# XuyangBai/PointDSC

Hardware: AMD Instinct MI355X
Metric: point-cloud pairs/sec @ N=5000 corr (higher is better)
Workload: dtype f32 (attention products as fp16x3 split (fp16 hi+lo operand pairs, three f16 MFMAs per product), f32 accumulate; fc_message / PointCN products as fp16 hi+lo split; spatial-consistency matrix stored as unorm16); 1 GPU; 3DMatch-like synthetic correspondences (BASELINE.json configs[2]): N=5000 corr, 32 pairs per step sharded over 1 GPU(s) = 32 per GPU, 12-layer PointDSC, seeded random weights; num_corr=5000, pairs_per_gpu=32, global_batch=32, compat_format=u16, layer_gemm=h3, att_leaves=canonical, latency_mode=False, range_guard=lazy (pipeline), collective=none (single process, no process group)

## Files before the change

include/pointdsc_hip.h:

```cpp
#ifndef POINTDSC_HIP_H
#define POINTDSC_HIP_H

#include <stddef.h>

#ifdef __cplusplus
extern "C" {
#endif

#define PDSC_VERSION 9
#define PDSC_CHANNELS 128
#define PDSC_MAX_K 64
#define PDSC_MAX_POWER_ITERS 32

enum pdsc_status {
    PDSC_OK = 0,
    PDSC_ERR_ARG = -1,
    PDSC_ERR_WORKSPACE = -2,
    PDSC_ERR_LAUNCH = -3
};

typedef struct pdsc_config {
    int in_dim;
    int num_layers;
    int num_channels;
// ... 79 lines not shown

int pdsc_layer0(const float* corr_pos, int in_dim, const float* W0, const float* b0, float* feat,
                int M, void* stream);

enum pdsc_layer_kernel {
    PDSC_LAYER_KERNEL_AUTO = 0,
    PDSC_LAYER_KERNEL_BLOCK,
    PDSC_LAYER_KERNEL_WAVE,
    PDSC_LAYER_KERNEL_H3,
    PDSC_LAYER_KERNEL_X3
};
typedef struct pdsc_layer_call {
    const float* msg;
    const float* part_o;
    const float* part_ml;
    int nsplit, Npad;
    const float* res;
    const float* feat_in;
    float* feat_out;
    float* featB_out;
    float* qkv_out;
    void* q_split;
    void* kv_tiles;
    const void* w1; const float* b1;
    const void* w2; const float* b2;
    const void* w3; const float* b3;
    const void* wp; const float* bp;
    const void* wq; const float* bq;
    const void* wq_split;
    const void* wfrag_tail;
    const void* wfrag_head;
    int gemm_format;
    int io_flags;
    int bs, N;
    int kernel;
} pdsc_layer_call;
int pdsc_layer_run(const pdsc_layer_call* call, void* stream);

size_t    pdsc_wsplit_bytes(const pdsc_config* cfg);
long long pdsc_wsplit_offset(const pdsc_config* cfg, int section, int layer);
int       pdsc_wsplit_build(const pdsc_config* cfg, const float* wpack, void* wsplit, void* stream);
#define PDSC_WS_FRAG_TAIL 100
#define PDSC_WS_FRAG_HEAD 101
#define PDSC_WS_FRAG_TAIL_H3 102
#define PDSC_WS_FRAG_HEAD_H3 103
#define PDSC_WS_FOLD_TAIL_H3 104
#define PDSC_WS_FOLD_HEAD_H3 105
#define PDSC_WS_FOLD_W 106
size_t pdsc_wfrag_fold_tail_bytes(void);
size_t pdsc_wfrag_fold_head_bytes(void);
int pdsc_layer_prefers_block(int bs, int N);
int pdsc_layer_h3_uses_coop(int bs, int N);
size_t pdsc_wfrag_tail_bytes(void);
size_t pdsc_wfrag_head_bytes(void);
int pdsc_wfrag_build_tail(const float* w1, const float* b1, const float* w2, const float* b2, const float* w3,
                          const float* b3, void* out, int gemm_format, void* stream);
int pdsc_wfrag_build_head(const float* wp, const float* bp, const float* wq, const float* bq, void* out,
                          int gemm_format, void* stream);

size_t pdsc_attention_scratch_bytes(int bs, int N, int nsplit);
int    pdsc_attention_default_split(int bs, int N);
int    pdsc_sc_attention(const float* qkv, const float* compat, long long ld, float* msg,
                         void* scratch, size_t scratch_bytes, int bs, int N, int nsplit, void* stream);

size_t pdsc_split_q_bytes(int bs, int N);
size_t pdsc_split_kv_bytes(int bs, int N);
int    pdsc_pack_qkv_split(const float* qkv, void* q_split, void* kv_tiles, int bs, int N, void* stream);
size_t pdsc_attention_split_scratch_bytes(int bs, int N, int nsplit);
int    pdsc_attention_split_default_split(int bs, int N);
int    pdsc_attention_leaf_count(int N);
int    pdsc_attention_leaf_plan(int bs, int N, int leaves_mode, int* nsplit, int* nleaf);
size_t pdsc_attention_leaf_scratch_bytes(int bs, int N, int leaves_mode);
int    pdsc_sc_attention_split(const void* q_split, const void* kv_tiles, const float* compat, long long ld,
                               float* msg, void* scratch, size_t scratch_bytes, int bs, int N, int nsplit,
                               void* stream);
int    pdsc_sc_attention_split_u16(const void* q_split, const void* kv_tiles, const unsigned short* compat_u16, long long ld,
                                   float* msg, void* scratch, size_t scratch_bytes, int bs, int N, int nsplit,
                                   void* stream);

int pdsc_attention_trace(long long* device_buffer);

int pdsc_attention_leaf_split_override(int d);

int pdsc_layer_trace(long long* device_buffer);

int pdsc_classifier_hidden(const float* feat, const float* W1, const float* b1, const float* W2, const float* b2, float* h2,
                           int M, void* stream);

int pdsc_normalize_confidence(const float* feat, const float* h2, const float* w3, const float* b3,
                              float* normed, float* conf, int M, void* stream);

int pdsc_nms_keys(const float* src_keypts, const float* conf, float radius, float* keys,
                  int bs, int N, void* stream);
size_t pdsc_nms_workspace_bytes(int bs, int N);
int pdsc_nms_keys_grid(const float* src_keypts, const float* conf, float radius, float* keys, void* workspace,
                       size_t workspace_bytes, int bs, int N, void* stream);
int pdsc_rank_select(const float* keys, int* seeds, int bs, int N, int num_seeds, void* stream);

int pdsc_knn_seeds(const float* normed, const int* seeds, float* dist_scratch, int* knn_idx,
                   int bs, int N, int S, int k, void* stream);
int pdsc_knn_seeds_form(const float* normed, const float* normed_pf, const int* seeds, float* dist_scratch, int* knn_idx,
                        int bs, int N, int S, int k, int form, void* stream);
int pdsc_normalize_confidence_pf(const float* feat, const float* h2, const float* w3, const float* b3, float* normed,
                                 float* normed_pf, float* conf, int bs, int N, void* stream);

int pdsc_seed_power_iteration(const float* normed, const float* src_keypts, const float* tgt_keypts,
                              const int* knn_idx, const float* sigma, const float* sigma_spat,
                              float* eig_iters, unsigned int* conv_mask, float* seed_M,
                              int bs, int N, int S, int k, int num_iterations, void* stream);

int pdsc_seed_transforms(const float* src_keypts, const float* tgt_keypts, const int* knn_idx,
                         const float* eig_iters, const unsigned int* conv_mask, float* seed_trans,
                         float* seed_weights ,
                         int bs, int N, int S, int k, int num_iterations, void* stream);

int pdsc_seed_solve(const float* normed, const float* src_keypts, const float* tgt_keypts, const int* knn_idx,
                    const float* sigma, const float* sigma_spat, float* eig_iters, unsigned int* conv_mask, float* seed_M,
                    float* seed_trans, float* seed_weights, int bs, int N, int S, int k, int num_iterations, void* stream);

int pdsc_rigid_transform_3d(const float* A, const float* B, const float* weights, float weight_threshold,
                            float* T, int bs, int n, void* stream);

int pdsc_score_hypotheses(const float* seed_trans, const float* src_keypts, const float* tgt_keypts,
                          float inlier_threshold, int* counts, int bs, int N, int S, void* stream);
int pdsc_select_best(const int* counts, const float* seed_trans, const float* src_keypts,
                     const float* tgt_keypts, float inlier_threshold, int* best, float* initial_trans,
                     float* labels, int bs, int N, int S, void* stream);

int pdsc_post_refinement(const float* initial_trans, const float* src_keypts, const float* tgt_keypts,
                         float threshold, int max_iters, float* final_trans, int* solves,
                         int bs, int N, void* stream);

int pdsc_forward_testing(const pdsc_config* cfg, const float* wpack, const void* wsplit ,
                         const float* corr_pos, const float* src_keypts, const float* tgt_keypts,
                         int bs, int N, int num_seeds,
                         float* final_trans, float* final_labels,
                         void* workspace, size_t workspace_bytes, void* stream);

int pdsc_forward_testing_ragged(const pdsc_config* cfg, const float* wpack, const void* wsplit,
                                const float* corr_pos, const float* src_keypts, const float* tgt_keypts,
                                int bs, int N, int num_seeds, const int* num_corr, const int* num_seeds_per_pair, int n_min,
                                float* final_trans, float* final_labels,
                                void* workspace, size_t workspace_bytes, void* stream);

int pdsc_forward_testing_streams(const pdsc_config* cfg, const float* wpack, const void* wsplit,
                                 const float* corr_pos, const float* src_keypts, const float* tgt_keypts,
                                 int bs, int N, int num_seeds, const int* num_corr ,
                                 const int* num_seeds_per_pair, int n_min,
                                 float* final_trans, float* final_labels,
                                 void* workspace, size_t workspace_bytes,
                                 void* stream, void* tail_stream, void* fork_event, void* join_event);

int pdsc_forward_validation(const pdsc_config* cfg, const float* wpack, const void* wsplit,
                            const float* corr_pos, const float* src_keypts, const float* tgt_keypts,
                            int bs, int N, int num_seeds, float* final_trans, float* logits,
                            float* M, long long ldM, void* workspace, size_t workspace_bytes, void* stream);

int pdsc_feature_compat(const float* normed, const float* sigma, float* M, long long ld, int bs, int N, void* stream);

int pdsc_conv_mask_all_pairs(unsigned int* conv_mask, int bs, void* stream);

size_t pdsc_match_scratch_bytes(int Ns, int Nt);
int pdsc_match_descriptors(const float* src_desc, const float* tgt_desc, int Ns, int Nt, int D, int* nn_idx,
                           float* nn_dist, void* scratch, size_t scratch_bytes, void* stream);
int pdsc_match_descriptors_ip(const float* src_desc, const float* tgt_desc, int Ns, int Nt, int D, int* nn_idx,
                              float* nn_dot, void* scratch, size_t scratch_bytes, void* stream);
// ... 135 lines not shown
```

pointdsc_amd/_lib.py:

```python
from __future__ import annotations

import ctypes as C
import os
from pathlib import Path

PKG = Path(__file__).resolve().parent
LIB_PATH = Path(os.environ.get("POINTDSC_HIP_LIB", PKG / "libpointdsc_hip.so"))


class PointDSCLibraryError(RuntimeError):
    pass


class PdscConfig(C.Structure):
    _fields_ = [
        ("in_dim", C.c_int), ("num_layers", C.c_int), ("num_channels", C.c_int),
        ("num_iterations", C.c_int), ("k", C.c_int), ("refine_iters", C.c_int),
        ("inlier_threshold", C.c_float), ("nms_radius", C.c_float), ("refine_threshold", C.c_float),
        ("attention_precision", C.c_int), ("compat_format", C.c_int), ("layer_gemm", C.c_int),
        ("att_leaves", C.c_int), ("value_fold", C.c_int),
    ]


W_SECTIONS = [
    "LAYER0_W", "LAYER0_B", "PCN_W", "PCN_B", "QKV_W", "QKV_B", "FC1_W", "FC1_B", "FC2_W", "FC2_B",
    "FC3_W", "FC3_B", "CLS1_W", "CLS1_B", "CLS2_W", "CLS2_B", "CLS3_W", "CLS3_B", "SIGMA", "SIGMA_SPAT",
]
W = {name: i for i, name in enumerate(W_SECTIONS)}

_vp, _i, _f, _ll, _sz = C.c_void_p, C.c_int, C.c_float, C.c_longlong, C.c_size_t
_cfgp = C.POINTER(PdscConfig)


class PdscLayerCall(C.Structure):
    _fields_ = (
        [(n, _vp) for n in ("msg", "part_o", "part_ml")] + [("nsplit", _i), ("Npad", _i)] +
        [(n, _vp) for n in ("res", "feat_in", "feat_out", "featB_out", "qkv_out", "q_split", "kv_tiles",
                            "w1", "b1", "w2", "b2", "w3", "b3", "wp", "bp", "wq", "bq", "wq_split", "wfrag_tail", "wfrag_head")] +
        [(n, _i) for n in ("gemm_format", "io_flags", "bs", "N", "kernel")])

SIGNATURES = {
    "pdsc_version": (_i, []),
    "pdsc_set_range_report": (_i, [_vp]),
    "pdsc_last_error": (C.c_char_p, []),
    "pdsc_experiments_enabled": (_i, []),
    "pdsc_wpack_floats": (_ll, [_cfgp]),
    "pdsc_wpack_offset": (_ll, [_cfgp, _i, _i]),
    "pdsc_compat_ld": (_ll, [_i]),
    "pdsc_workspace_bytes": (_sz, [_cfgp, _i, _i, _i]),
    "pdsc_workspace_offset": (_ll, [_cfgp, _i, _i, _i, C.c_char_p]),
    "pdsc_spatial_compat": (_i, [_vp, _vp, _vp, _vp, _vp, _ll, _i, _i, _vp]),
    "pdsc_spatial_compat_u16": (_i, [_vp, _vp, _vp, _vp, _ll, _i, _i, _vp]),
    "pdsc_selftest_exact_math": (_i, [_vp, _f, _vp, _vp, _ll, _vp]),
    "pdsc_selftest_mfma_valu_neighbour": (_i, [_vp, _i, _i, _vp]),
    "pdsc_classifier_hidden": (_i, [_vp, _vp, _vp, _vp, _vp, _vp, _i, _vp]),
    "pdsc_linear": (_i, [_vp, _ll, _vp, _vp, _vp, _ll, _vp, _ll, _i, _i, _i, _i, _vp]),
    "pdsc_layer0": (_i, [_vp, _i, _vp, _vp, _vp, _i, _vp]),
    "pdsc_layer_run": (_i, [C.POINTER(PdscLayerCall), _vp]),
    "pdsc_wsplit_bytes": (_sz, [_cfgp]),
    "pdsc_wsplit_offset": (_ll, [_cfgp, _i, _i]),
    "pdsc_wsplit_build": (_i, [_cfgp, _vp, _vp, _vp]),
    "pdsc_layer_prefers_block": (_i, [_i, _i]),
    "pdsc_layer_h3_uses_coop": (_i, [_i, _i]),
    "pdsc_wfrag_tail_bytes": (_sz, []),
    "pdsc_wfrag_head_bytes": (_sz, []),
    "pdsc_wfrag_fold_tail_bytes": (_sz, []),
    "pdsc_wfrag_fold_head_bytes": (_sz, []),
    "pdsc_wfrag_build_tail": (_i, [_vp] * 7 + [_i, _vp]),
    "pdsc_wfrag_build_head": (_i, [_vp] * 5 + [_i, _vp]),
    "pdsc_sc_attention_split_partials": (_i, [_vp, _vp, _vp, _i, _ll, _vp, _sz, _i, _i, _i, _i, _vp]),
    "pdsc_split_q_bytes": (_sz, [_i, _i]),
    "pdsc_split_kv_bytes": (_sz, [_i, _i]),
    "pdsc_pack_qkv_split": (_i, [_vp, _vp, _vp, _i, _i, _vp]),
    "pdsc_attention_split_scratch_bytes": (_sz, [_i, _i, _i]),
    "pdsc_attention_split_default_split": (_i, [_i, _i]),
    "pdsc_attention_leaf_count": (_i, [_i]),
    "pdsc_attention_leaf_plan": (_i, [_i, _i, _i, C.POINTER(C.c_int), C.POINTER(C.c_int)]),
    "pdsc_attention_leaf_scratch_bytes": (_sz, [_i, _i, _i]),
    "pdsc_attention_trace": (_i, [_vp]),
    "pdsc_attention_leaf_split_override": (_i, [_i]),
    "pdsc_layer_trace": (_i, [_vp]),
    "pdsc_sc_attention_split": (_i, [_vp, _vp, _vp, _ll, _vp, _vp, _sz, _i, _i, _i, _vp]),
    "pdsc_sc_attention_split_u16": (_i, [_vp, _vp, _vp, _ll, _vp, _vp, _sz, _i, _i, _i, _vp]),
    "pdsc_attention_scratch_bytes": (_sz, [_i, _i, _i]),
    "pdsc_attention_default_split": (_i, [_i, _i]),
    "pdsc_sc_attention": (_i, [_vp, _vp, _ll, _vp, _vp, _sz, _i, _i, _i, _vp]),
    "pdsc_normalize_confidence": (_i, [_vp, _vp, _vp, _vp, _vp, _vp, _i, _vp]),
    "pdsc_nms_keys": (_i, [_vp, _vp, _f, _vp, _i, _i, _vp]),
    "pdsc_nms_workspace_bytes": (_sz, [_i, _i]),
    "pdsc_nms_keys_grid": (_i, [_vp, _vp, _f, _vp, _vp, _sz, _i, _i, _vp]),
    "pdsc_rank_select": (_i, [_vp, _vp, _i, _i, _i, _vp]),
    "pdsc_knn_seeds": (_i, [_vp, _vp, _vp, _vp, _i, _i, _i, _i, _vp]),
    "pdsc_knn_seeds_form": (_i, [_vp, _vp, _vp, _vp, _vp, _i, _i, _i, _i, _i, _vp]),
    "pdsc_normalize_confidence_pf": (_i, [_vp, _vp, _vp, _vp, _vp, _vp, _vp, _i, _i, _vp]),
    "pdsc_seed_power_iteration": (_i, [_vp, _vp, _vp, _vp, _vp, _vp, _vp, _vp, _vp, _i, _i, _i, _i, _i, _vp]),
    "pdsc_seed_solve": (_i, [_vp] * 11 + [_i, _i, _i, _i, _i, _vp]),
    "pdsc_seed_transforms": (_i, [_vp, _vp, _vp, _vp, _vp, _vp, _vp, _i, _i, _i, _i, _i, _vp]),
    "pdsc_rigid_transform_3d": (_i, [_vp, _vp, _vp, _f, _vp, _i, _i, _vp]),
    "pdsc_score_hypotheses": (_i, [_vp, _vp, _vp, _f, _vp, _i, _i, _i, _vp]),
    "pdsc_select_best": (_i, [_vp, _vp, _vp, _vp, _f, _vp, _vp, _vp, _i, _i, _i, _vp]),
    "pdsc_post_refinement": (_i, [_vp, _vp, _vp, _f, _i, _vp, _vp, _i, _i, _vp]),
    "pdsc_profile_enable": (_i, [_i]),
    "pdsc_profile_reset": (_i, []),
    "pdsc_profile_set_stride": (_i, [_i, _i]),
    "pdsc_profile_read": (_i, [_i, C.POINTER(C.c_double), C.POINTER(C.c_int)]),
    "pdsc_match_scratch_bytes": (_sz, [_i, _i]),
    "pdsc_match_descriptors": (_i, [_vp, _vp, _i, _i, _i, _vp, _vp, _vp, _sz, _vp]),
    "pdsc_match_descriptors_ip": (_i, [_vp, _vp, _i, _i, _i, _vp, _vp, _vp, _sz, _vp]),
    "pdsc_select_correspondences": (_i, [_vp, _vp, _i, _vp, _vp, _vp]),
    "pdsc_build_corr_pos": (_i, [_vp, _vp, _vp, _vp, _vp, _vp, _vp, _vp]),
    "pdsc_sm_workspace_bytes": (_sz, [_i, _i]),
    "pdsc_sm_baseline": (_i, [_vp, _vp, _vp, _f, _i, _i, _vp, _vp, _vp, _vp, _sz, _i, _i, _vp]),
    "pdsc_sm_baseline_form": (_i, [_vp, _vp, _vp, _f, _i, _i, _vp, _vp, _vp, _vp, _sz, _i, _i, _i, _vp]),
    "pdsc_pmc_adjacency": (_i, [_vp, _f, _vp, _ll, _i, _i, _vp]),
    "pdsc_pmc_workspace_bytes": (_sz, [_i, _i]),
    "pdsc_pmc_baseline": (_i, [_vp, _vp, _vp, _f, _i, _vp, _vp, _vp, _vp, _vp, _sz, _i, _i, _vp]),
    "pdsc_pmc_baseline_ex": (_i, [_vp, _vp, _vp, _f, _i, _vp, _vp, _vp, _vp, _vp, _sz, _i, _i, _i, C.POINTER(C.c_float), _vp]),
    "pdsc_cal_confidence_workspace_bytes": (_sz, [_i, _i]),
    "pdsc_cal_confidence": (_i, [_vp, _ll, _vp, _i, _i, _vp, _vp, _sz, _i, _i, _vp]),
    "pdsc_eval_stats": (_i, [_vp, _vp, _vp, _vp, _f, _f, _vp, _i, _i, _vp]),
    "pdsc_loss_workspace_bytes": (_sz, [_i, _i]),
    "pdsc_classification_loss": (_i, [_vp, _vp, _vp, _i, _vp, _vp, _vp, _sz, _i, _i, _vp]),
    "pdsc_sm_loss_matrix": (_i, [_vp, _ll, _vp, _i, _vp, _vp, _vp, _sz, _i, _i, _vp]),
    "pdsc_sm_loss_features": (_i, [_vp, _vp, _vp, _i, _vp, _vp, _vp, _vp, _sz, _i, _i, _vp]),
    "pdsc_transformation_loss": (_i, [_vp, _vp, _vp, _vp, _vp, _f, _f, _vp, _vp, _sz, _i, _i, _vp]),
    "pdsc_sc_attention_lse": (_i, [_vp, _vp, _ll, _vp, _vp, _vp, _sz, _i, _i, _i, _vp]),
    "pdsc_attention_backward_workspace_bytes": (_sz, [_i, _i]),
    "pdsc_sc_attention_backward": (_i, [_vp, _vp, _ll, _vp, _vp, _vp, _vp, _vp, _sz, _i, _i, _vp]),
    "pdsc_attention_backward_default_split": (_i, [_i, _i]),
    "pdsc_attention_backward_split_workspace_bytes": (_sz, [_i, _i, _i]),
    "pdsc_sc_attention_backward_split": (_i, [_vp, _vp, _ll, _vp, _vp, _vp, _vp, _vp, _sz, _i, _i, _i, _vp]),
    "pdsc_feature_compat_backward_workspace_bytes": (_sz, [_i, _i]),
    "pdsc_feature_compat_backward": (_i, [_vp, _vp, _vp, _ll, _vp, _vp, _vp, _sz, _i, _i, _vp]),
    "pdsc_icp_workspace_bytes": (_sz, [_i, _i, _i]),
    "pdsc_icp_refine": (_i, [_vp, _vp, _vp, _vp, _vp, C.c_double, C.c_double, C.c_double, _i, _vp, _vp, _vp, _vp, _vp, _vp, _vp,
                             _sz, _i, _i, _i, _vp]),
    "pdsc_information_workspace_bytes": (_sz, [_i, _i, _i]),
    "pdsc_information_matrix": (_i, [_vp, _vp, _vp, _vp, _vp, C.c_double, _vp, _vp, _vp, _vp, _sz, _i, _i, _i, _vp]),
    "pdsc_voxel_keys": (_i, [_vp, _vp, C.c_double, _vp, _i, _i, _vp]),
    "pdsc_voxel_means": (_i, [_vp, _vp, _vp, _vp, _vp, _i, _i, _vp]),
    "pdsc_hybrid_neighbours_workspace_bytes": (_sz, [_i, _i]),
    "pdsc_hybrid_neighbours": (_i, [_vp, _vp, C.c_double, _i, _vp, _vp, _vp, _vp, _sz, _i, _i, _vp]),
    "pdsc_estimate_normals": (_i, [_vp, _vp, _vp, _vp, _i, C.POINTER(C.c_double), _vp, _i, _i, _vp]),
    "pdsc_spfh": (_i, [_vp, _vp, _vp, _vp, _vp, _i, _vp, _i, _i, _vp]),
    "pdsc_fpfh_from_spfh": (_i, [_vp, _vp, _vp, _vp, _vp, _i, _vp, _vp, _i, _i, _vp]),
    "pdsc_fpfh_workspace_bytes": (_sz, [_i, _i, _i, _i]),
    "pdsc_fpfh": (_i, [_vp, _vp, C.c_double, _i, C.c_double, _i, C.POINTER(C.c_double), _vp, _vp, _vp, _vp, _sz, _i, _i, _vp]),
    "pdsc_cloud_voxel_workspace_bytes": (_sz, [_i, _i]),
    "pdsc_cloud_voxel_keys": (_i, [_vp, _vp, C.c_double, _vp, _vp, _sz, _i, _i, _i, _vp]),
    "pdsc_cloud_voxel_means": (_i, [_vp, _vp, _vp, _vp, _vp, _vp, _vp, _i, _i, _vp, _sz, _i, _i, _i, _vp]),
    "pdsc_cloud_neighbours": (_i, [_vp, _vp, C.c_double, _i, _vp, _vp, _vp, _vp, _sz, _i, _i, _i, _vp]),
    "pdsc_posegraph_workspace_bytes": (_sz, [_i, _i, _i]),
    "pdsc_posegraph_nodes": (_i, [_vp] * 6 + [_i, _i, _i, _vp]),
    "pdsc_global_optimization": (_i, [_vp] * 9 + [C.c_double, C.c_double, C.c_double, _i, _vp, _vp, _vp, _vp, _vp, _vp, _sz, _i, _i, _i, _i,
                                      _i, _vp]),
    "pdsc_encoder_range_probe": (_i, [_cfgp, _vp, _vp, _vp, _vp, _vp, _i, _i, _i, _vp, _vp, _sz, _vp]),
    "pdsc_forward_validation": (_i, [_cfgp, _vp, _vp, _vp, _vp, _vp, _i, _i, _i, _vp, _vp, _vp, _ll, _vp, _sz, _vp]),
    "pdsc_feature_compat": (_i, [_vp, _vp, _vp, _ll, _i, _i, _vp]),
    "pdsc_conv_mask_all_pairs": (_i, [_vp, _i, _vp]),
    "pdsc_forward_testing": (_i, [_cfgp, _vp, _vp, _vp, _vp, _vp, _i, _i, _i, _vp, _vp, _vp, _sz, _vp]),
    "pdsc_forward_testing_ragged": (_i, [_cfgp, _vp, _vp, _vp, _vp, _vp, _i, _i, _i, _vp, _vp, _i, _vp, _vp, _vp, _sz, _vp]),
    "pdsc_forward_testing_streams": (_i, [_cfgp, _vp, _vp, _vp, _vp, _vp, _i, _i, _i, _vp, _vp, _i, _vp, _vp, _vp, _sz, _vp, _vp, _vp, _vp]),
}
# ... 37 lines not shown
```

pointdsc_amd/csrc/api.hip:

```cpp
#include <stdarg.h>
#include <stdlib.h>
#include <string.h>
#include <mutex>
#include "pdsc_common.h"
#include "ragged.h"
#include "attention_common.h"
#include "layer_args.h"

namespace pdsc {

static thread_local char g_err[512] = "";

static unsigned int*& range_report_slot() {
    static thread_local unsigned int* slot = nullptr;
    return slot;
}

void set_error(const char* fmt, ...) {
    va_list ap;
    va_start(ap, fmt);
    vsnprintf(g_err, sizeof(g_err), fmt, ap);
    va_end(ap);
}

int check_launch(const char* what) {
    const hipError_t e = hipGetLastError();
    if (e != hipSuccess) {
        set_error("%s: %s", what, hipGetErrorString(e));
        return PDSC_ERR_LAUNCH;
    }
    return PDSC_OK;
}

int ensure_dynamic_lds(const void* fn, size_t bytes, const char* what) {
    struct Entry { const void* fn; size_t granted[64]; };
    static Entry table[64];
    static int used = 0;
    static std::mutex mu;
    int dev = 0;
    if (hipGetDevice(&dev) != hipSuccess) return check_launch(what);
    std::lock_guard<std::mutex> lock(mu);
    Entry* e = nullptr;
    for (int i = 0; i < used; ++i)
        if (table[i].fn == fn) { e = &table[i]; break; }
    if (e && dev < 64 && e->granted[dev] >= bytes) return PDSC_OK;
    if (hipFuncSetAttribute(fn, hipFuncAttributeMaxDynamicSharedMemorySize, (int)bytes) != hipSuccess) return check_launch(what);
    if (!e && used < 64) { e = &table[used++]; e->fn = fn; memset(e->granted, 0, sizeof(e->granted)); }
    if (e && dev < 64) e->granted[dev] = bytes;
    return PDSC_OK;
}

__global__ void fill_u32_kernel(unsigned int* p, unsigned int value, size_t count) {
    const size_t i = (size_t)blockIdx.x * blockDim.x + threadIdx.x;
    if (i < count) p[i] = value;
}
__global__ void copy_u32_kernel(unsigned int* __restrict__ dst, const unsigned int* __restrict__ src, size_t count) {
    for (size_t i = (size_t)blockIdx.x * blockDim.x + threadIdx.x; i < count; i += (size_t)gridDim.x * blockDim.x) dst[i] = src[i];
}
__global__ void absmax_kernel(const float* __restrict__ x, size_t count, unsigned int* __restrict__ slot) {
    unsigned int m = 0u;
    for (size_t i = (size_t)blockIdx.x * blockDim.x + threadIdx.x; i < count; i += (size_t)gridDim.x * blockDim.x) {
        const unsigned int u = __float_as_uint(x[i]) & 0x7fffffffu;
        m = u > m ? u : m;
    }
#pragma unroll
    for (int off = 32; off > 0; off >>= 1) {
        const unsigned int o = __shfl_xor(m, off, 64);
        m = o > m ? o : m;
    }
    if ((threadIdx.x & 63) == 0 && m) atomicMax(slot, m);
}
static int launch_absmax(const float* x, size_t count, unsigned int* slot, hipStream_t st) {
    const size_t blocks = (count + 1023) / 1024;
    hipLaunchKernelGGL(absmax_kernel, dim3((unsigned)(blocks < 2048 ? blocks : 2048)), dim3(256), 0, st, x, count, slot);
    return check_launch("absmax");
}
int launch_copy_u32(unsigned int* dst, const unsigned int* src, size_t count, hipStream_t st) {
    if (count == 0) return PDSC_OK;
    const size_t blocks = (count + 255) / 256;
    hipLaunchKernelGGL(copy_u32_kernel, dim3((unsigned)(blocks < 4096 ? blocks : 4096)), dim3(256), 0, st, dst, src, count);
    return check_launch("copy");
}
int launch_fill_u32(unsigned int* p, unsigned int value, size_t count, hipStream_t st) {
    if (count == 0) return PDSC_OK;
    hipLaunchKernelGGL(fill_u32_kernel, dim3((unsigned)((count + 255) / 256)), dim3(256), 0, st, p, value, count);
    return check_launch("fill");
}

struct ProfKind { hipEvent_t* start = nullptr; hipEvent_t* stop = nullptr; int cap = 0, n = 0, stride = 1; long long calls = 0; bool open = false; };
static ProfKind g_prof[PDSC_PROF_NUM_KINDS];

void profile_mark_begin(int kind, hipStream_t st) {
    ProfKind& p = g_prof[kind];
    if (p.cap == 0 || p.n >= p.cap) return;
    if ((p.calls++ % p.stride) != 0) return;
    (void)hipEventRecord(p.start[p.n], st);
    p.open = true;
}
void profile_mark_end(int kind, hipStream_t st) {
// ... 99 lines not shown
    "compat", "featA", "featB", "featC", "qkv", "msg", "t64a", "t64b", "att_scratch", "q_split", "kv_tiles", "normed",
    "normed_pf", "h1", "h2", "conf", "keys", "nms_ws", "seeds", "knn_dist", "knn_idx", "eig_iters", "conv_mask",
    "seed_trans", "seed_w", "counts", "best", "initial_trans", "solves", "range_flag", "refine_trace",
#ifdef PDSC_EXPERIMENTS
    "score_dbg",
#endif
};
static_assert(sizeof(ws_names) / sizeof(ws_names[0]) == WS_NUM, "ws_names must name every WsId, in order");

struct WsLayout {
    size_t offset[WS_NUM], bytes[WS_NUM], total;
    template <class T> T* at(void* ws, WsId id) const { return (T*)((char*)ws + offset[id]); }
};

static WsLayout make_layout(const pdsc_config* c, int bs, int N, int S) {
    WsLayout L{};
    size_t* B = L.bytes;
    const size_t M = (size_t)bs * N, C = PDSC_CHANNELS, f = sizeof(float);
    const size_t ld = (size_t)pdsc_compat_ld(N);
    const int k = c->k < N - 1 ? c->k : N - 1;
    const int iters = c->num_iterations > 0 ? c->num_iterations : 1;
    const bool compat16 = c->attention_precision != PDSC_ATT_FP32 && c->compat_format == PDSC_COMPAT_U16;
    B[WS_COMPAT] = (size_t)bs * N * ld * (compat16 ? sizeof(unsigned short) : f);
    B[WS_FEATA] = M * C * f;
    const size_t Mpf = (size_t)bs * round_up(N, 32);
    B[WS_FEATB] = B[WS_FEATC] = Mpf * C * f;
    B[WS_QKV] = M * 3 * C * f;
    B[WS_MSG] = M * C * f;
    B[WS_T64A] = B[WS_T64B] = M * (C / 2) * f;
    {
        const size_t a32 = pdsc_attention_scratch_bytes(bs, N, 0), a16 = pdsc_attention_split_scratch_bytes(bs, N, 0);
        const size_t amg = c->att_leaves >= PDSC_LEAVES_CANONICAL ? pdsc_attention_leaf_scratch_bytes(bs, N, c->att_leaves) : 0;
        B[WS_ATT_SCRATCH] = c->attention_precision == PDSC_ATT_FP32 ? a32 : (a16 > amg ? a16 : amg);
    }
    B[WS_Q_SPLIT] = c->attention_precision != PDSC_ATT_FP32 ? pdsc_split_q_bytes(bs, N) : 0;
    B[WS_KV_TILES] = c->attention_precision != PDSC_ATT_FP32 ? pdsc_split_kv_bytes(bs, N) : 0;
    B[WS_NORMED] = M * C * f;
    B[WS_NORMED_PF] = knn_seeds_uses_fused(bs, N, S, k) ? Mpf * C * f : 0;
    B[WS_H1] = B[WS_H2] = M * 32 * f;
    B[WS_CONF] = B[WS_KEYS] = M * f;
    B[WS_NMS_WS] = pdsc_nms_workspace_bytes(bs, N);
    B[WS_SEEDS] = (size_t)bs * S * sizeof(int);
    B[WS_KNN_DIST] = (size_t)bs * S * ld * f;
    B[WS_KNN_IDX] = (size_t)bs * S * (k > 0 ? k : 1) * sizeof(int);
    B[WS_EIG_ITERS] = (size_t)bs * S * iters * PDSC_MAX_K * f;
    B[WS_CONV_MASK] = (size_t)bs * sizeof(unsigned int);
    B[WS_SEED_TRANS] = (size_t)bs * S * 16 * f;
    B[WS_SEED_W] = (size_t)bs * S * (k > 0 ? k : 1) * f;
    B[WS_COUNTS] = (size_t)bs * S * sizeof(int);
    B[WS_BEST] = (size_t)bs * sizeof(int);
    B[WS_INITIAL_TRANS] = (size_t)bs * 16 * f;
    B[WS_SOLVES] = (size_t)bs * sizeof(int);
    B[WS_RANGE_FLAG] = (size_t)bs * sizeof(unsigned int);
    B[WS_REFINE_TRACE] = (size_t)bs * PDSC_REFINE_TRACE * sizeof(int);
#ifdef PDSC_EXPERIMENTS
    B[WS_SCORE_DBG] = (size_t)bs * S * 16 * f;
#endif
    for (int i = 0; i < WS_NUM; ++i) {
        L.offset[i] = L.total;
        L.total += (size_t)round_up((long long)B[i], 256);
    }
    return L;
}

}

using namespace pdsc;

extern "C" int pdsc_version(void) { return PDSC_VERSION; }

extern "C" int pdsc_set_range_report(unsigned int* host_words) {
    if (host_words) {
        hipPointerAttribute_t at{};
        if (hipPointerGetAttributes(&at, host_words) != hipSuccess || at.type != hipMemoryTypeHost || at.devicePointer == nullptr) {
            (void)hipGetLastError();
            set_error("pdsc_set_range_report: %p is not pinned, device-mapped host memory", (void*)host_words);
            return PDSC_ERR_ARG;
        }
        host_words = (unsigned int*)at.devicePointer;
    }
    range_report_slot() = host_words;
    return PDSC_OK;
}
extern "C" int pdsc_experiments_enabled(void) {
#ifdef PDSC_EXPERIMENTS
    return 1;
#else
    return 0;
#endif
}
extern "C" const char* pdsc_last_error(void) { return g_err; }

extern "C" long long pdsc_wpack_floats(const pdsc_config* cfg) {
    if (!config_ok(cfg)) return -1;
    return wpack_offset(cfg, PDSC_W_SIGMA_SPAT, 0) + section_floats(PDSC_W_SIGMA_SPAT);
}
extern "C" long long pdsc_wpack_offset(const pdsc_config* cfg, int section, int layer) {
    if (!config_ok(cfg)) return -1;
    return wpack_offset(cfg, section, layer);
}

extern "C" size_t pdsc_workspace_bytes(const pdsc_config* cfg, int bs, int N, int num_seeds) {
    if (!config_ok(cfg) || bs <= 0 || N <= 1 || num_seeds <= 0) return 0;
    return make_layout(cfg, bs, N, num_seeds).total;
}
extern "C" long long pdsc_workspace_offset(const pdsc_config* cfg, int bs, int N, int num_seeds, const char* name) {
    if (!config_ok(cfg) || bs <= 0 || N <= 1 || num_seeds <= 0 || !name) return -1;
    const WsLayout L = make_layout(cfg, bs, N, num_seeds);
    for (int i = 0; i < WS_NUM; ++i)
        if (strcmp(ws_names[i], name) == 0) return (long long)L.offset[i];
    return -1;
}

extern "C" int pdsc_profile_enable(int max_records) {
    for (int k = 0; k < PDSC_PROF_NUM_KINDS; ++k) {
        ProfKind& p = g_prof[k];
        for (int i = 0; i < p.cap; ++i) { (void)hipEventDestroy(p.start[i]); (void)hipEventDestroy(p.stop[i]); }
        delete[] p.start; delete[] p.stop;
        const int keep_stride = p.stride;
        p = ProfKind();
        p.stride = keep_stride;
        if (max_records > 0) {
            p.start = new hipEvent_t[max_records];
            p.stop = new hipEvent_t[max_records];
            for (int i = 0; i < max_records; ++i) {
                if (hipEventCreate(&p.start[i]) != hipSuccess || hipEventCreate(&p.stop[i]) != hipSuccess)
                    return check_launch("pdsc_profile_enable");
            }
            p.cap = max_records;
        }
    }
    return PDSC_OK;
}
extern "C" int pdsc_profile_reset(void) {
    for (int k = 0; k < PDSC_PROF_NUM_KINDS; ++k) { g_prof[k].n = 0; g_prof[k].open = false; g_prof[k].calls = 0; }
    return PDSC_OK;
}
extern "C" int pdsc_profile_set_stride(int kind, int stride) {
    PDSC_REQUIRE(kind >= 0 && kind < PDSC_PROF_NUM_KINDS && stride >= 1, "pdsc_profile_set_stride: kind=%d stride=%d", kind, stride);
    g_prof[kind].stride = stride;
    g_prof[kind].calls = 0;
    return PDSC_OK;
}
extern "C" int pdsc_profile_read(int kind, double* total_ms, int* launches) {
    PDSC_REQUIRE(kind >= 0 && kind < PDSC_PROF_NUM_KINDS && total_ms && launches, "pdsc_profile_read: bad argument");
    ProfKind& p = g_prof[kind];
    double tot = 0.0;
    for (int i = 0; i < p.n; ++i) {
        if (hipEventSynchronize(p.stop[i]) != hipSuccess) return check_launch("pdsc_profile_read");
        float ms = 0.f;
        if (hipEventElapsedTime(&ms, p.start[i], p.stop[i]) != hipSuccess) return check_launch("pdsc_profile_read");
        tot += ms;
    }
    *total_ms = tot;
    *launches = p.n;
    return PDSC_OK;
}

#define PDSC_TRY(call)                 \
    do {                               \
        const int rc__ = (call);       \
        if (rc__ != PDSC_OK) return rc__; \
    } while (0)

struct EncoderPlan {
    bool fused;
    bool split;
    LayerKernel kernel;
    bool x3, frag;
    bool fuse_merge;
    bool pf, leaves, fold;
    int gemm;
    int ns, Npad;
    int nleaf, value_width;
    int leaf_ns;
    int ws_tail, ws_head;
};

static int plan_encoder(const pdsc_config* cfg, int bs, int N, const int* nvalid, int n_min, EncoderPlan* plan) {
    EncoderPlan& p = *plan = EncoderPlan{};
    p.split = cfg->attention_precision != PDSC_ATT_FP32;
    p.x3 = cfg->attention_precision == PDSC_ATT_FP16X3_ALL;
    p.fused = env_int("PDSC_FUSED_LAYERS", 1) != 0 && cfg->num_layers > 0;
    const bool canonical = cfg->att_leaves >= PDSC_LEAVES_CANONICAL;
    const int min_tiles = (n_min + 31) / 32;
    p.ns = p.split ? pdsc_attention_split_default_split(bs, N) : 0;
#define PDSC_REQUIRE_SHORTEST_PAIR(cond)                                                                                             \
    PDSC_REQUIRE(cond, "pdsc_forward_testing_ragged: the shortest pair (%d correspondences) has fewer 32-key tiles than the key split " \
                 "planned for bs=%d, N=%d (%d): batch pairs of more similar size", n_min, bs, N, p.ns)
    if (nvalid && p.split && !canonical) PDSC_REQUIRE_SHORTEST_PAIR(min_tiles >= p.ns);
    const char* var = env_str("PDSC_LAYER_VARIANT");
    const bool force_block = var && var[0] == 'b', force_wave = var && var[0] == 'w';
    auto by_size = [&](int pairs, int rows) {
        return force_block || (!force_wave && pdsc_layer_prefers_block(pairs, rows)) ? LayerKernel::Block : LayerKernel::Wave;
    };
    if (!p.fused || !p.split) {
        p.kernel = by_size(1, bs * N);
        return PDSC_OK;
    }
    p.Npad = (int)round_up(N, 256);
    p.gemm = env_int("PDSC_LAYER_GEMM", cfg->layer_gemm) == PDSC_LAYER_GEMM_H3 ? PDSC_LAYER_GEMM_H3 : PDSC_LAYER_GEMM_F32;
    const bool h3 = p.gemm == PDSC_LAYER_GEMM_H3;
    const LayerKernel natural = by_size(bs, N);
    p.frag = env_int("PDSC_LAYER_FRAG", 1) && !p.x3 && !force_block && (natural == LayerKernel::Wave || h3);
    p.kernel = p.x3     ? LayerKernel::X3
               : !p.frag ? natural
                         : h3 && env_int("PDSC_LAYER_H3_VARIANT", 1) != 0 ? LayerKernel::H3 : LayerKernel::Wave;
    p.fuse_merge = env_int("PDSC_FUSE_MERGE", 1) && p.ns > 1 && p.ns <= layer_merge_limit(p.kernel);
    const bool pf_ok = p.kernel == LayerKernel::H3 && env_int("PDSC_LAYER_PF", 1) != 0;
    int lf_ns = 0, lf_nw = 0;
    if (canonical) PDSC_TRY(leaf_plan(bs, N, cfg->att_leaves, &lf_nw, &lf_ns, &p.nleaf));
    p.leaf_ns = lf_ns;
    p.leaves = pf_ok && canonical && (!nvalid || min_tiles >= 2 * p.nleaf);
    if (nvalid && !p.leaves) PDSC_REQUIRE_SHORTEST_PAIR(min_tiles >= p.ns);
#undef PDSC_REQUIRE_SHORTEST_PAIR
    p.pf = p.leaves || (pf_ok && p.fuse_merge);
    p.fold = cfg->value_fold == PDSC_VALUE_FOLD_ON && p.pf && N <= PDSC_VALUE_FOLD_MAX_N;
    p.value_width = p.fold ? PDSC_CHANNELS / 2 : PDSC_CHANNELS;
    p.ws_tail = p.fold ? PDSC_WS_FOLD_TAIL_H3 : h3 ? PDSC_WS_FRAG_TAIL_H3 : PDSC_WS_FRAG_TAIL;
    p.ws_head = p.fold ? PDSC_WS_FOLD_HEAD_H3 : h3 ? PDSC_WS_FRAG_HEAD_H3 : PDSC_WS_FRAG_HEAD;
    return PDSC_OK;
}

enum class ForwardMode { Testing, Validation, Probe };

struct ForwardCall {
    ForwardMode mode;
    const pdsc_config* cfg;
    const float* wpack;
    const void* wsplit;
    const float *corr_pos, *src, *tgt;
    int bs, N, num_seeds;
    float *final_trans, *final_labels, *Mout;
    long long ldM;
    void* workspace;
    size_t workspace_bytes;
    void* stream;
    const int *nvalid, *svalid;
    int n_min;
    void *tail_stream, *ev_fork, *ev_join;
    unsigned int* probe;
};

struct ForwardCtx {
    const ForwardCall& c;
    EncoderPlan plan;
    WsLayout L;
    hipStream_t st;
    int M, S, k, cfmt;
    long long ld;
    bool split;
    float *compat, *featA, *featB, *featC, *qkv, *msg, *normed, *normed_pf, *conf, *keys, *seed_trans;
    int *seeds, *knn_idx, *counts;
    unsigned int *conv_mask, *range_flag;
    void *att_scratch, *q_split, *kv_tiles;
    const float* W(int section, int layer) const { return c.wpack + wpack_offset(c.cfg, section, layer); }
    const void* WS(int section, int layer) const { return (const unsigned short*)c.wsplit + pdsc_wsplit_offset(c.cfg, section, layer); }
};

static int validate_call(const ForwardCall& c) {
    if (!config_ok(c.cfg)) return PDSC_ERR_ARG;
    PDSC_REQUIRE(!c.tail_stream || (c.ev_fork && c.ev_join && c.tail_stream != c.stream),
                 "pdsc_forward_testing_streams: a tail stream (different from the main stream) needs the fork and join events");
    const int N = c.N, n_min = c.n_min, k = c.cfg->k < N - 1 ? c.cfg->k : N - 1;
    if (c.nvalid) {
        PDSC_REQUIRE(c.mode == ForwardMode::Testing && c.svalid, "pdsc_forward_testing_ragged: testing forward only, both count arrays needed");
        PDSC_REQUIRE(n_min >= 2 && n_min <= N, "pdsc_forward_testing_ragged: n_min=%d (N=%d)", n_min, N);
        PDSC_REQUIRE(n_min > k, "pdsc_forward_testing_ragged: the shortest pair (%d correspondences) has no "
                     "more than k=%d: the reference clamps k per pair (k = min(k, num_corr - 1)); run such a pair in its own call", n_min, k);
    }
    const bool outputs = c.mode == ForwardMode::Probe || (c.final_trans && c.final_labels);
    PDSC_REQUIRE(c.wpack && c.corr_pos && c.src && c.tgt && outputs && c.workspace, "pdsc_forward_testing: null pointer");
    PDSC_REQUIRE(c.bs > 0 && N > 1, "pdsc_forward_testing: bs=%d N=%d", c.bs, N);
    PDSC_REQUIRE(c.num_seeds >= 1 && c.num_seeds <= N,
                 "pdsc_forward_testing: num_seeds=%d (int(N*ratio) must be >= 1; the reference fails on an empty seed set)", c.num_seeds);
    return PDSC_OK;
}

static int bind_workspace(ForwardCtx& x) {
    const ForwardCall& c = x.c;
    const WsLayout& L = x.L = make_layout(c.cfg, c.bs, c.N, c.num_seeds);
    if (c.workspace_bytes < L.total) {
        set_error("pdsc_forward_testing: workspace %zu < %zu bytes", c.workspace_bytes, L.total);
        return PDSC_ERR_WORKSPACE;
    }
    void* ws = c.workspace;
    x.st = (hipStream_t)c.stream;
    x.M = c.bs * c.N; x.S = c.num_seeds; x.k = c.cfg->k < c.N - 1 ? c.cfg->k : c.N - 1;
    x.ld = pdsc_compat_ld(c.N);
    x.compat = L.at<float>(ws, WS_COMPAT); x.featA = L.at<float>(ws, WS_FEATA); x.featB = L.at<float>(ws, WS_FEATB);
    x.featC = L.at<float>(ws, WS_FEATC); x.qkv = L.at<float>(ws, WS_QKV); x.msg = L.at<float>(ws, WS_MSG);
    x.normed = L.at<float>(ws, WS_NORMED); x.conf = L.at<float>(ws, WS_CONF); x.keys = L.at<float>(ws, WS_KEYS);
    x.seed_trans = L.at<float>(ws, WS_SEED_TRANS); x.seeds = L.at<int>(ws, WS_SEEDS); x.knn_idx = L.at<int>(ws, WS_KNN_IDX);
    x.counts = L.at<int>(ws, WS_COUNTS); x.conv_mask = L.at<unsigned int>(ws, WS_CONV_MASK); x.att_scratch = L.at<void>(ws, WS_ATT_SCRATCH);
    const bool split = x.split = x.plan.split;
    PDSC_REQUIRE(!split || c.wsplit, "pdsc_forward_testing: the split-precision modes need the split-weight buffer (pdsc_wsplit_build)");
    x.q_split = split ? L.at<void>(ws, WS_Q_SPLIT) : nullptr;
    x.kv_tiles = split ? L.at<void>(ws, WS_KV_TILES) : nullptr;
    x.range_flag = split && c.mode != ForwardMode::Probe ? L.at<unsigned int>(ws, WS_RANGE_FLAG) : nullptr;
    x.cfmt = split && c.cfg->compat_format == PDSC_COMPAT_U16 ? PDSC_COMPAT_U16 : PDSC_COMPAT_F32;
    const bool knn_fused = c.mode == ForwardMode::Testing && knn_seeds_uses_fused(c.bs, c.N, x.S, x.k);
    x.normed_pf = knn_fused ? L.at<float>(ws, WS_NORMED_PF) : nullptr;
    return PDSC_OK;
}

static int probe_absmax(const ForwardCtx& x, int kind, const float* v, size_t count) {
    return x.c.probe ? launch_absmax(v, count, x.c.probe + kind, x.st) : PDSC_OK;
}

static int run_compat_layer0(const ForwardCtx& x) {
    const ForwardCall& c = x.c;
    if (x.cfmt == PDSC_COMPAT_U16)
        PDSC_TRY(pdsc_spatial_compat_u16(c.src, c.tgt, x.W(PDSC_W_SIGMA_SPAT, 0), (unsigned short*)x.compat, x.ld, c.bs, c.N, x.st));
    else
        PDSC_TRY(pdsc_spatial_compat(c.src, c.tgt, x.W(PDSC_W_SIGMA_SPAT, 0), x.compat, nullptr, x.ld, c.bs, c.N, x.st));
    PDSC_TRY(launch_layer0(c.corr_pos, c.cfg->in_dim, x.W(PDSC_W_LAYER0_W, 0), x.W(PDSC_W_LAYER0_B, 0), x.featA, x.M, x.range_flag, c.bs, x.st));
    return probe_absmax(x, PDSC_RANGE_LAYER0, x.featA, (size_t)x.M * PDSC_CHANNELS);
}

static int attention_split(const ForwardCtx& x, float* msg_out, int nsplit) {
    return launch_attention_split_ex(x.q_split, x.kv_tiles, x.compat, x.cfmt, x.ld, msg_out, x.att_scratch, x.L.bytes[WS_ATT_SCRATCH], x.c.bs,
                                     x.c.N, nsplit, PDSC_PARTIALS_ROWS, x.c.nvalid, x.st);
}

static int run_fused_layer(const ForwardCtx& x, int i, bool last, const float* cur, float* nxt) {
    const EncoderPlan& plan = x.plan;
    const bool tail = i >= 0, head = !last, split = x.split;
    const bool parts = plan.pf || plan.fuse_merge;
    const int slots = plan.leaves ? plan.nleaf : plan.ns;
    const int nparts = plan.leaves && plan.leaf_ns == 1 ? 1 : slots;
    const float* part_o = parts ? (const float*)x.att_scratch : nullptr;
    const float* part_ml = parts ? part_o + (size_t)x.c.bs * slots * plan.Npad * plan.value_width : nullptr;
    pdsc_layer_call c{};
    c.bs = split ? x.c.bs : 1; c.N = split ? x.c.N : x.M;
    if (tail) {
        c.msg = parts ? nullptr : x.msg;
        c.part_o = part_o; c.part_ml = part_ml; c.nsplit = nparts; c.Npad = plan.Npad;
        c.res = cur;
    } else
        c.feat_in = x.featA;
    if (last) c.feat_out = x.featA;
    if (head) {
        c.featB_out = nxt; c.qkv_out = split ? nullptr : x.qkv;
        c.q_split = x.q_split; c.kv_tiles = x.kv_tiles;
    }
    if (plan.frag) {
        if (tail) c.wfrag_tail = x.WS(plan.ws_tail, i);
        if (head) c.wfrag_head = x.WS(plan.ws_head, i + 1);
        c.gemm_format = plan.gemm;
    } else {
        auto mat = [&](int section, int l) { return plan.x3 ? x.WS(section, l) : (const void*)x.W(section, l); };
        if (tail) {
            c.w1 = mat(PDSC_W_FC1_W, i); c.b1 = x.W(PDSC_W_FC1_B, i); c.w2 = mat(PDSC_W_FC2_W, i); c.b2 = x.W(PDSC_W_FC2_B, i);
            c.w3 = mat(PDSC_W_FC3_W, i); c.b3 = x.W(PDSC_W_FC3_B, i);
        }
        if (head) {
            c.wp = mat(PDSC_W_PCN_W, i + 1); c.bp = x.W(PDSC_W_PCN_B, i + 1); c.wq = mat(PDSC_W_QKV_W, i + 1); c.bq = x.W(PDSC_W_QKV_B, i + 1);
            if (split) c.wq_split = x.WS(PDSC_W_QKV_W, i + 1);
        }
    }
    if (plan.pf) c.io_flags = (tail ? PDSC_IO_PARTIALS_PF | PDSC_IO_RES_PF : 0) | (head ? PDSC_IO_FEATB_PF : 0);
    LayerArgs a = layer_args_from_call(c);
    a.nvalid = split ? x.c.nvalid : nullptr;
    if (tail) a.part_slots = slots;
    if (plan.pf) {
        a.value_fold = plan.fold;
        a.range_flag = x.range_flag;
    } else
        a.trace = pdsc_layer_trace_buffer();
    PDSC_TRY(validate_layer_args(a, plan.kernel, "pdsc_forward_testing(layer)"));
    return dispatch_layer(a, plan.kernel, x.st);
}

static int run_encoder_fused(const ForwardCtx& x) {
    const ForwardCall& c = x.c;
    const EncoderPlan& plan = x.plan;
    const size_t att_bytes = x.L.bytes[WS_ATT_SCRATCH];
    PDSC_TRY(run_fused_layer(x, -1, false, nullptr, x.featB));
    float *cur = x.featB, *nxt = x.featC;
    for (int i = 0; i < c.cfg->num_layers; ++i) {
        if (!x.split)
            PDSC_TRY(launch_attention_fp32(x.qkv, x.compat, x.ld, x.msg, x.att_scratch, att_bytes, c.bs, c.N, 0, c.nvalid, x.st));
        else if (plan.leaves)
            PDSC_TRY(launch_attention_leaves(x.q_split, x.kv_tiles, x.compat, x.cfmt, x.ld, x.att_scratch, att_bytes, c.bs, c.N,
                                             c.cfg->att_leaves, c.nvalid, c.n_min, x.st, plan.value_width));
        else if (plan.pf)
            PDSC_TRY(launch_attention_split_ex(x.q_split, x.kv_tiles, x.compat, x.cfmt, x.ld, nullptr, x.att_scratch, att_bytes, c.bs, c.N,
                                               plan.ns, PDSC_PARTIALS_PF, c.nvalid, x.st, plan.value_width));
        else
            PDSC_TRY(attention_split(x, plan.fuse_merge ? nullptr : x.msg, plan.ns));
        PDSC_TRY(run_fused_layer(x, i, i + 1 == c.cfg->num_layers, cur, nxt));
        float* tmp = cur; cur = nxt; nxt = tmp;
    }
    return PDSC_OK;
}

static int run_encoder_per_conv(const ForwardCtx& x) {
    const int C = PDSC_CHANNELS, H = C / 2, M = x.M;
    float *t64a = x.L.at<float>(x.c.workspace, WS_T64A), *t64b = x.L.at<float>(x.c.workspace, WS_T64B);
    for (int i = 0; i < x.c.cfg->num_layers; ++i) {
        PDSC_TRY(pdsc_linear(x.featA, C, x.W(PDSC_W_PCN_W, i), x.W(PDSC_W_PCN_B, i), nullptr, 0, x.featB, C, M, C, C, 1, x.st));
        PDSC_TRY(probe_absmax(x, PDSC_RANGE_POINTCN, x.featB, (size_t)M * C));
        PDSC_TRY(pdsc_linear(x.featB, C, x.W(PDSC_W_QKV_W, i), x.W(PDSC_W_QKV_B, i), nullptr, 0, x.qkv, 3 * C, M, C, 3 * C, 0, x.st));
        PDSC_TRY(probe_absmax(x, PDSC_RANGE_QKV, x.qkv, (size_t)M * 3 * C));
        if (x.split) {
            PDSC_TRY(pdsc_pack_qkv_split(x.qkv, x.q_split, x.kv_tiles, x.c.bs, x.c.N, x.st));
            PDSC_TRY(attention_split(x, x.msg, 0));
        } else
            PDSC_TRY(pdsc_sc_attention(x.qkv, x.compat, x.ld, x.msg, x.att_scratch, x.L.bytes[WS_ATT_SCRATCH], x.c.bs, x.c.N, 0, x.st));
        PDSC_TRY(probe_absmax(x, PDSC_RANGE_MESSAGE, x.msg, (size_t)M * C));
        PDSC_TRY(pdsc_linear(x.msg, C, x.W(PDSC_W_FC1_W, i), x.W(PDSC_W_FC1_B, i), nullptr, 0, t64a, H, M, C, H, 1, x.st));
        PDSC_TRY(probe_absmax(x, PDSC_RANGE_FC1, t64a, (size_t)M * H));
        PDSC_TRY(pdsc_linear(t64a, H, x.W(PDSC_W_FC2_W, i), x.W(PDSC_W_FC2_B, i), nullptr, 0, t64b, H, M, H, H, 1, x.st));
        PDSC_TRY(probe_absmax(x, PDSC_RANGE_FC2, t64b, (size_t)M * H));
        PDSC_TRY(pdsc_linear(t64b, H, x.W(PDSC_W_FC3_W, i), x.W(PDSC_W_FC3_B, i), x.featB, C, x.featA, C, M, H, C, 0, x.st));
        PDSC_TRY(probe_absmax(x, PDSC_RANGE_FEATURE, x.featA, (size_t)M * C));
    }
    return PDSC_OK;
}

static int fork_tail(ForwardCtx& x) {
    if (!x.c.tail_stream) return PDSC_OK;
    if (hipEventRecord((hipEvent_t)x.c.ev_fork, (hipStream_t)x.c.stream) != hipSuccess ||
        hipStreamWaitEvent((hipStream_t)x.c.tail_stream, (hipEvent_t)x.c.ev_fork, 0) != hipSuccess)
        return check_launch("pdsc_forward_testing_streams(fork)");
    x.st = (hipStream_t)x.c.tail_stream;
    return PDSC_OK;
}
static int join_tail(const ForwardCtx& x) {
    if (!x.c.tail_stream) return PDSC_OK;
    if (hipEventRecord((hipEvent_t)x.c.ev_join, (hipStream_t)x.c.tail_stream) != hipSuccess ||
        hipStreamWaitEvent((hipStream_t)x.c.stream, (hipEvent_t)x.c.ev_join, 0) != hipSuccess)
        return check_launch("pdsc_forward_testing_streams(join)");
    return PDSC_OK;
}

static int run_seed_selection(const ForwardCtx& x) {
    const ForwardCall& c = x.c;
    const int C = PDSC_CHANNELS, M = x.M;
    float *h1 = x.L.at<float>(c.workspace, WS_H1), *h2 = x.L.at<float>(c.workspace, WS_H2);
    if (env_int("PDSC_CLS_FUSED", 1))
        PDSC_TRY(launch_classifier_hidden(x.featA, x.W(PDSC_W_CLS1_W, 0), x.W(PDSC_W_CLS1_B, 0), x.W(PDSC_W_CLS2_W, 0), x.W(PDSC_W_CLS2_B, 0), h2, M, x.st));
    else {
        PDSC_TRY(pdsc_linear(x.featA, C, x.W(PDSC_W_CLS1_W, 0), x.W(PDSC_W_CLS1_B, 0), nullptr, 0, h1, 32, M, C, 32, 1, x.st));
        PDSC_TRY(pdsc_linear(h1, 32, x.W(PDSC_W_CLS2_W, 0), x.W(PDSC_W_CLS2_B, 0), nullptr, 0, h2, 32, M, 32, 32, 1, x.st));
    }
    if (x.normed_pf)
        PDSC_TRY(launch_normalize_conf_pf(x.featA, h2, x.W(PDSC_W_CLS3_W, 0), x.W(PDSC_W_CLS3_B, 0), x.normed, x.normed_pf, x.conf, c.bs, c.N, x.st));
    else
        PDSC_TRY(pdsc_normalize_confidence(x.featA, h2, x.W(PDSC_W_CLS3_W, 0), x.W(PDSC_W_CLS3_B, 0), x.normed, x.conf, M, x.st));
    if (c.mode == ForwardMode::Testing) {
        PDSC_TRY(launch_nms_keys_grid(c.src, x.conf, c.cfg->nms_radius, x.keys, x.L.at<void>(c.workspace, WS_NMS_WS),
                                      pdsc_nms_workspace_bytes(c.bs, c.N), c.bs, c.N, c.nvalid, x.st));
        return launch_rank_select(x.keys, x.seeds, c.bs, c.N, x.S, c.nvalid, c.svalid, x.st, x.conv_mask);
    }
    PDSC_TRY(pdsc_feature_compat(x.normed, x.W(PDSC_W_SIGMA, 0), c.Mout, c.ldM, c.bs, c.N, x.st));
    return pdsc_rank_select(x.conf, x.seeds, c.bs, c.N, x.S, x.st);
}

static int run_hypotheses(const ForwardCtx& x) {
    const ForwardCall& c = x.c;
    const bool testing = c.mode == ForwardMode::Testing;
    const int iters = c.cfg->num_iterations;
    void* ws = c.workspace;
    float *knn_dist = x.L.at<float>(ws, WS_KNN_DIST), *eig = x.L.at<float>(ws, WS_EIG_ITERS), *seed_w = x.L.at<float>(ws, WS_SEED_W);
    PDSC_TRY(launch_knn_seeds_form(x.normed, x.normed_pf, x.seeds, knn_dist, x.knn_idx, c.bs, c.N, x.S, x.k, c.nvalid, x.normed_pf ? 2 : 1, x.st));
    if (!testing && c.bs > 1) {
        PDSC_TRY(pdsc_seed_power_iteration(x.normed, c.src, c.tgt, x.knn_idx, x.W(PDSC_W_SIGMA, 0), x.W(PDSC_W_SIGMA_SPAT, 0), eig, x.conv_mask,
                                           nullptr, c.bs, c.N, x.S, x.k, iters, x.st));
        PDSC_TRY(pdsc_conv_mask_all_pairs(x.conv_mask, c.bs, x.st));
        PDSC_TRY(pdsc_seed_transforms(c.src, c.tgt, x.knn_idx, eig, x.conv_mask, x.seed_trans, seed_w, c.bs, c.N, x.S, x.k, iters, x.st));
    } else
        PDSC_TRY(launch_seed_solve_forward(x.normed, c.src, c.tgt, x.knn_idx, x.W(PDSC_W_SIGMA, 0), x.W(PDSC_W_SIGMA_SPAT, 0), eig, x.conv_mask,
                                           x.seed_trans, seed_w, c.bs, c.N, x.S, x.k, iters, testing, x.st));
#ifdef PDSC_EXPERIMENTS
    score_debug_slot() = env_int("PDSC_SCORE_DEBUG", 0) ? x.L.at<float>(ws, WS_SCORE_DBG) : nullptr;
#endif
    PDSC_TRY(launch_score_hypotheses(x.seed_trans, c.src, c.tgt, c.cfg->inlier_threshold, x.counts, c.bs, c.N, x.S, c.nvalid, x.st));
#ifdef PDSC_EXPERIMENTS
    score_debug_slot() = nullptr;
#endif
    return PDSC_OK;
}

static int finish_testing(const ForwardCtx& x) {
    const ForwardCall& c = x.c;
    const WsLayout& L = x.L;
    void* ws = c.workspace;
    return launch_select_and_refine(x.counts, x.seed_trans, c.src, c.tgt, c.cfg->inlier_threshold, c.cfg->refine_threshold, c.cfg->refine_iters,
                                    L.at<int>(ws, WS_BEST), L.at<float>(ws, WS_INITIAL_TRANS), c.final_labels, c.final_trans,
                                    L.at<int>(ws, WS_SOLVES), c.bs, c.N, x.S, c.nvalid, x.st, L.at<int>(ws, WS_REFINE_TRACE), x.range_flag,
                                    range_report_slot());
}
static int finish_validation(const ForwardCtx& x) {
    const ForwardCall& c = x.c;
    PDSC_TRY(pdsc_select_best(x.counts, x.seed_trans, c.src, c.tgt, c.cfg->inlier_threshold, x.L.at<int>(c.workspace, WS_BEST), c.final_trans,
                              x.keys , c.bs, c.N, x.S, x.st));
    return launch_copy_u32((unsigned int*)c.final_labels, (const unsigned int*)x.conf, (size_t)x.M, x.st);
}

static int run_forward(const ForwardCall& call) {
    const bool probe = call.mode == ForwardMode::Probe, testing = call.mode == ForwardMode::Testing;
    ForwardCtx x{call};
    PDSC_TRY(validate_call(call));
    PDSC_TRY(plan_encoder(call.cfg, call.bs, call.N, call.nvalid, call.n_min, &x.plan));
    PDSC_TRY(bind_workspace(x));
    PDSC_TRY(run_compat_layer0(x));
    PDSC_TRY(x.plan.fused && !probe ? run_encoder_fused(x) : run_encoder_per_conv(x));
    if (probe) return PDSC_OK;
    PDSC_TRY(fork_tail(x));
    PDSC_TRY(run_seed_selection(x));
    PDSC_TRY(run_hypotheses(x));
    PDSC_TRY(testing ? finish_testing(x) : finish_validation(x));
    return join_tail(x);
}

extern "C" int pdsc_forward_testing(const pdsc_config* cfg, const float* wpack, const void* wsplit, const float* corr_pos,
                                    const float* src, const float* tgt, int bs, int N, int num_seeds,
                                    float* final_trans, float* final_labels, void* workspace, size_t workspace_bytes,
                                    void* stream) {
    return run_forward({.mode = ForwardMode::Testing, .cfg = cfg, .wpack = wpack, .wsplit = wsplit, .corr_pos = corr_pos, .src = src,
                        .tgt = tgt, .bs = bs, .N = N, .num_seeds = num_seeds, .final_trans = final_trans, .final_labels = final_labels,
                        .workspace = workspace, .workspace_bytes = workspace_bytes, .stream = stream});
}

extern "C" int pdsc_forward_testing_ragged(const pdsc_config* cfg, const float* wpack, const void* wsplit, const float* corr_pos,
                                           const float* src, const float* tgt, int bs, int N, int num_seeds, const int* num_corr,
                                           const int* num_seeds_per_pair, int n_min, float* final_trans, float* final_labels,
                                           void* workspace, size_t workspace_bytes, void* stream) {
    PDSC_REQUIRE(num_corr && num_seeds_per_pair, "pdsc_forward_testing_ragged: the per-pair count arrays (device, [bs] int32) are required");
    return run_forward({.mode = ForwardMode::Testing, .cfg = cfg, .wpack = wpack, .wsplit = wsplit, .corr_pos = corr_pos, .src = src,
                        .tgt = tgt, .bs = bs, .N = N, .num_seeds = num_seeds, .final_trans = final_trans, .final_labels = final_labels,
                        .workspace = workspace, .workspace_bytes = workspace_bytes, .stream = stream, .nvalid = num_corr,
                        .svalid = num_seeds_per_pair, .n_min = n_min});
}

extern "C" int pdsc_forward_testing_streams(const pdsc_config* cfg, const float* wpack, const void* wsplit, const float* corr_pos,
                                            const float* src, const float* tgt, int bs, int N, int num_seeds, const int* num_corr,
                                            const int* num_seeds_per_pair, int n_min, float* final_trans, float* final_labels,
                                            void* workspace, size_t workspace_bytes, void* stream, void* tail_stream, void* fork_event,
                                            void* join_event) {
    PDSC_REQUIRE((num_corr == nullptr) == (num_seeds_per_pair == nullptr), "pdsc_forward_testing_streams: both count arrays or neither");
    PDSC_REQUIRE(tail_stream && fork_event && join_event, "pdsc_forward_testing_streams: tail stream and both events are required");
    return run_forward({.mode = ForwardMode::Testing, .cfg = cfg, .wpack = wpack, .wsplit = wsplit, .corr_pos = corr_pos, .src = src,
                        .tgt = tgt, .bs = bs, .N = N, .num_seeds = num_seeds, .final_trans = final_trans, .final_labels = final_labels,
                        .workspace = workspace, .workspace_bytes = workspace_bytes, .stream = stream, .nvalid = num_corr,
                        .svalid = num_seeds_per_pair, .n_min = n_min, .tail_stream = tail_stream, .ev_fork = fork_event, .ev_join = join_event});
}

extern "C" int pdsc_encoder_range_probe(const pdsc_config* cfg, const float* wpack, const void* wsplit, const float* corr_pos,
                                        const float* src, const float* tgt, int bs, int N, int num_seeds, float* absmax,
                                        void* workspace, size_t workspace_bytes, void* stream) {
    PDSC_REQUIRE(absmax, "pdsc_encoder_range_probe: absmax [PDSC_RANGE_NUM_KINDS] (device) required");
    PDSC_TRY(launch_fill_u32((unsigned int*)absmax, 0u, PDSC_RANGE_NUM_KINDS, (hipStream_t)stream));
    return run_forward({.mode = ForwardMode::Probe, .cfg = cfg, .wpack = wpack, .wsplit = wsplit, .corr_pos = corr_pos, .src = src, .tgt = tgt,
                        .bs = bs, .N = N, .num_seeds = num_seeds, .workspace = workspace, .workspace_bytes = workspace_bytes, .stream = stream,
                        .probe = (unsigned int*)absmax});
}

extern "C" int pdsc_forward_validation(const pdsc_config* cfg, const float* wpack, const void* wsplit, const float* corr_pos,
                                       const float* src, const float* tgt, int bs, int N, int num_seeds,
                                       float* final_trans, float* logits, float* Mout, long long ldM, void* workspace,
                                       size_t workspace_bytes, void* stream) {
    PDSC_REQUIRE(Mout && ldM >= N, "pdsc_forward_validation: M matrix [bs][N][ldM >= N] required");
    return run_forward({.mode = ForwardMode::Validation, .cfg = cfg, .wpack = wpack, .wsplit = wsplit, .corr_pos = corr_pos, .src = src,
                        .tgt = tgt, .bs = bs, .N = N, .num_seeds = num_seeds, .final_trans = final_trans, .final_labels = logits, .Mout = Mout,
                        .ldM = ldM, .workspace = workspace, .workspace_bytes = workspace_bytes, .stream = stream});
}
```

pointdsc_amd/csrc/compat.hip:

```cpp
#include <stdlib.h>
#include "pdsc_common.h"

#define PDSC_COMPAT_DEFAULT_VARIANT 3

namespace pdsc {

struct InvariantDivisor {
    float b, y;
    __device__ __forceinline__ explicit InvariantDivisor(float b_) : b(b_) {
        const float y0 = __builtin_amdgcn_rcpf(b_);
        const float e = fmaf(-b_, y0, 1.0f);
        y = fmaf(e, y0, y0);
    }
    __device__ __forceinline__ float div(float a) const {
        const float q0 = a * y;
        const float r0 = fmaf(-b, q0, a);
        const float q1 = fmaf(r0, y, q0);
        const float r1 = fmaf(-b, q1, a);
        return fmaf(r1, y, q1);
    }
};

template <bool FASTMATH>
__device__ __forceinline__ float dist3(float x, float y, float z) {
    const float ss = fmaf(z, z, fmaf(y, y, x * x));
    return FASTMATH ? sqrt_rn(ss) : sqrtf(ss);
}
template <bool FASTMATH>
__device__ __forceinline__ float compat_from_dists(float ds, float dt, float s2, const InvariantDivisor& inv) {
    const float df = ds - dt;
    const float q = FASTMATH ? inv.div(df * df) : (df * df) / s2;
    return fmaxf(1.0f - q, 0.0f);
}

constexpr int CT_ROWS = 64;
constexpr int CT_COLS = 256;

template <bool WRITE_DIST, bool FASTMATH>
__global__ __launch_bounds__(256) void compat_kernel(const float* __restrict__ src, const float* __restrict__ tgt,
                                                     const float* __restrict__ sigma_spat,
                                                     float* __restrict__ compat, float* __restrict__ src_dist,
                                                     long long ld, int N) {
    __shared__ __attribute__((aligned(16))) float rows_s[CT_ROWS][8];
    const int b = blockIdx.z;
    const int i0 = blockIdx.y * CT_ROWS;
    const int j0 = blockIdx.x * CT_COLS;
    const float* srcb = src + (size_t)b * N * 3;
    const float* tgtb = tgt + (size_t)b * N * 3;
    const int t = threadIdx.x;
    if (t < CT_ROWS) {
        const int i = min(i0 + t, N - 1);
        rows_s[t][0] = srcb[i * 3 + 0]; rows_s[t][1] = srcb[i * 3 + 1]; rows_s[t][2] = srcb[i * 3 + 2];
        rows_s[t][4] = tgtb[i * 3 + 0]; rows_s[t][5] = tgtb[i * 3 + 1]; rows_s[t][6] = tgtb[i * 3 + 2];
    }
    const int lane = t & 63, wave = t >> 6;
    const int jc = j0 + lane * 4;
    float sx[4], sy[4], sz[4], tx[4], ty[4], tz[4];
#pragma unroll
    for (int c = 0; c < 4; ++c) {
        const int j = min(jc + c, N - 1);
        sx[c] = srcb[j * 3 + 0]; sy[c] = srcb[j * 3 + 1]; sz[c] = srcb[j * 3 + 2];
        tx[c] = tgtb[j * 3 + 0]; ty[c] = tgtb[j * 3 + 1]; tz[c] = tgtb[j * 3 + 2];
    }
    const float sg = sigma_spat[0];
    const float s2 = sg * sg;
    const InvariantDivisor inv(s2);
    __syncthreads();
    if (jc >= ld) return;
    float* outb = compat + (size_t)b * N * ld;
    float* distb = WRITE_DIST ? src_dist + (size_t)b * N * ld : nullptr;
#pragma unroll 4
    for (int r = 0; r < 16; ++r) {
        const int il = wave * 16 + r;
        const int i = i0 + il;
        if (i >= N) break;
        const f32x4 ps = *reinterpret_cast<const f32x4*>(&rows_s[il][0]);
        const f32x4 pt = *reinterpret_cast<const f32x4*>(&rows_s[il][4]);
        f32x4 o, dd;
#pragma unroll
        for (int c = 0; c < 4; ++c) {
            const float ds = dist3<FASTMATH>(ps[0] - sx[c], ps[1] - sy[c], ps[2] - sz[c]);
            const float dt = dist3<FASTMATH>(pt[0] - tx[c], pt[1] - ty[c], pt[2] - tz[c]);
            const float v = compat_from_dists<FASTMATH>(ds, dt, s2, inv);
            const bool valid = (jc + c) < N;
            o[c] = valid ? v : 0.0f;
            dd[c] = valid ? ds : 0.0f;
        }
        *reinterpret_cast<f32x4*>(outb + (size_t)i * ld + jc) = o;
        if (WRITE_DIST) *reinterpret_cast<f32x4*>(distb + (size_t)i * ld + jc) = dd;
    }
}

constexpr int CS_T = 128;
constexpr int CS_STRIP = 32;
constexpr int CS_LD = CS_T + 4;

template <bool FASTMATH>
__global__ __launch_bounds__(256) void compat_sym_kernel(const float* __restrict__ src, const float* __restrict__ tgt,
                                                         const float* __restrict__ sigma_spat, float* __restrict__ compat,
                                                         long long ld, int N) {
    const int I = blockIdx.y, J = blockIdx.x, b = blockIdx.z;
    if (I > J) return;
    __shared__ __attribute__((aligned(16))) float Ts[CS_STRIP * CS_LD];
    __shared__ __attribute__((aligned(16))) float rows_s[CS_T * 8];
    const int i0 = I * CS_T, j0 = J * CS_T;
    const float* srcb = src + (size_t)b * N * 3;
    const float* tgtb = tgt + (size_t)b * N * 3;
    const int t = threadIdx.x;
    if (t < CS_T) {
        const int i = min(i0 + t, N - 1);
        rows_s[t * 8 + 0] = srcb[i * 3 + 0]; rows_s[t * 8 + 1] = srcb[i * 3 + 1]; rows_s[t * 8 + 2] = srcb[i * 3 + 2];
        rows_s[t * 8 + 4] = tgtb[i * 3 + 0]; rows_s[t * 8 + 5] = tgtb[i * 3 + 1]; rows_s[t * 8 + 6] = tgtb[i * 3 + 2];
    }
    const int l32 = t & 31, rg = t >> 5;
    const int jc = j0 + l32 * 4;
    float sx[4], sy[4], sz[4], tx[4], ty[4], tz[4];
#pragma unroll
    for (int c = 0; c < 4; ++c) {
        const int j = min(jc + c, N - 1);
        sx[c] = srcb[j * 3 + 0]; sy[c] = srcb[j * 3 + 1]; sz[c] = srcb[j * 3 + 2];
        tx[c] = tgtb[j * 3 + 0]; ty[c] = tgtb[j * 3 + 1]; tz[c] = tgtb[j * 3 + 2];
    }
    const float sg = sigma_spat[0];
    const float s2 = sg * sg;
    const InvariantDivisor inv(s2);
    float* outb = compat + (size_t)b * N * ld;
    const bool offdiag = I != J;
    __syncthreads();
    for (int strip = 0; strip < CS_T / CS_STRIP; ++strip) {
#pragma unroll
        for (int r = 0; r < 4; ++r) {
            const int sl = rg + 8 * r;
            const int il = strip * CS_STRIP + sl;
            const int i = i0 + il;
            const f32x4 ps = *reinterpret_cast<const f32x4*>(rows_s + il * 8);
            const f32x4 pt = *reinterpret_cast<const f32x4*>(rows_s + il * 8 + 4);
            f32x4 o;
#pragma unroll
            for (int c = 0; c < 4; ++c) {
                const float ds = dist3<FASTMATH>(ps[0] - sx[c], ps[1] - sy[c], ps[2] - sz[c]);
                const float dt = dist3<FASTMATH>(pt[0] - tx[c], pt[1] - ty[c], pt[2] - tz[c]);
                const float v = compat_from_dists<FASTMATH>(ds, dt, s2, inv);
                o[c] = (jc + c) < N ? v : 0.0f;
            }
            if (i < N && jc < ld) *reinterpret_cast<f32x4*>(outb + (size_t)i * ld + jc) = o;
            if (offdiag) *reinterpret_cast<f32x4*>(Ts + sl * CS_LD + 4 * l32) = o;
        }
        if (offdiag) {
            __syncthreads();
            const int sl = t & 31, jq0 = t >> 5;
            const int i = i0 + strip * CS_STRIP + sl;
#pragma unroll
            for (int p = 0; p < 4; ++p) {
                const int jq = jq0 + 8 * p;
                const f32x4 v = *reinterpret_cast<const f32x4*>(Ts + sl * CS_LD + 4 * jq);
#pragma unroll
                for (int c = 0; c < 4; ++c) {
                    const int j = j0 + 4 * jq + c;
                    if (j < N && i < N) outb[(size_t)j * ld + i] = v[c];
                }
            }
            __syncthreads();
        }
    }
}

typedef unsigned short u16x2 __attribute__((ext_vector_type(2)));
typedef float f32x2 __attribute__((ext_vector_type(2)));
__host__ __device__ __forceinline__ int c16_pos(int r) { return 16 * ((r >> 2) & 1) + 4 * (r >> 3) + (r & 3); }
__host__ __device__ __forceinline__ int c16_chunk_base(int q) { return 16 * (q & 1) + 4 * (q >> 1); }

constexpr int CF_T = 128;
__device__ __forceinline__ int cf_point_slot(int r) { return (r + (r >> 4)) * 8; }

template <bool EDGE, bool CLAMP>
__device__ __forceinline__ void compat_fast_tile(const float* __restrict__ pts, unsigned short* __restrict__ outb, long long ld,
                                                 int N, int i0, int j0, bool offdiag, float ninv) {
    const int t = threadIdx.x, lane = t & 63, w = t >> 6;
    const int ri = (w >> 1) * 8 + (lane >> 3), cj = (w & 1) * 8 + (lane & 7);
    const int rbase = 32 * (ri >> 2) + c16_chunk_base(ri & 3);
    const int cbase = 32 * (cj >> 2) + c16_chunk_base(cj & 3);
    f32x2 sx[4], sy[4], sz[4], tx[4], ty[4], tz[4];
#pragma unroll
    for (int cp = 0; cp < 4; ++cp) {
        const int m0 = 2 * cp, c0 = cbase + (m0 & 3) + 8 * (m0 >> 2);
        const f32x4 a0 = *reinterpret_cast<const f32x4*>(pts + cf_point_slot(CF_T + c0));
        const f32x4 b0 = *reinterpret_cast<const f32x4*>(pts + cf_point_slot(CF_T + c0) + 4);
        const f32x4 a1 = *reinterpret_cast<const f32x4*>(pts + cf_point_slot(CF_T + c0 + 1));
        const f32x4 b1 = *reinterpret_cast<const f32x4*>(pts + cf_point_slot(CF_T + c0 + 1) + 4);
        sx[cp] = f32x2{a0[0], a1[0]}; sy[cp] = f32x2{a0[1], a1[1]}; sz[cp] = f32x2{a0[2], a1[2]};
        tx[cp] = f32x2{b0[0], b1[0]}; ty[cp] = f32x2{b0[1], b1[1]}; tz[cp] = f32x2{b0[2], b1[2]};
    }
    unsigned tr[8][4];
    f32x2 one2 = {1.0f, 1.0f}, ninv2 = {ninv, ninv}, zero2 = {0.f, 0.f};
    asm volatile("" : "+v"(one2), "+v"(ninv2), "+v"(zero2));
    const int colpos = j0 + 32 * (cj >> 2) + 8 * (cj & 3);
    const int rowpos = i0 + 32 * (ri >> 2) + 8 * (ri & 3);
#pragma unroll
    for (int rp = 0; rp < 4; ++rp) {
        const int m0 = 2 * rp, r0 = rbase + (m0 & 3) + 8 * (m0 >> 2);
        const f32x4 ps0 = *reinterpret_cast<const f32x4*>(pts + cf_point_slot(r0));
        const f32x4 pt0 = *reinterpret_cast<const f32x4*>(pts + cf_point_slot(r0) + 4);
        const f32x4 ps1 = *reinterpret_cast<const f32x4*>(pts + cf_point_slot(r0 + 1));
        const f32x4 pt1 = *reinterpret_cast<const f32x4*>(pts + cf_point_slot(r0 + 1) + 4);
        unsigned d0[4], d1[4];
        f32x2 bs[2][3], bt[2][3];
#pragma unroll
        for (int rr = 0; rr < 2; ++rr)
#pragma unroll
            for (int e = 0; e < 3; ++e) {
                bs[rr][e] = f32x2{(rr ? ps1 : ps0)[e], (rr ? ps1 : ps0)[e]};
                bt[rr][e] = f32x2{(rr ? pt1 : pt0)[e], (rr ? pt1 : pt0)[e]};
                asm volatile("" : "+v"(bs[rr][e]), "+v"(bt[rr][e]));
            }
#pragma unroll
        for (int cp = 0; cp < 4; ++cp) {
            f32x2 o[2];
#pragma unroll
            for (int rr = 0; rr < 2; ++rr) {
                const f32x2 dx = bs[rr][0] - sx[cp], dy = bs[rr][1] - sy[cp], dz = bs[rr][2] - sz[cp];
                const f32x2 ex = bt[rr][0] - tx[cp], ey = bt[rr][1] - ty[cp], ez = bt[rr][2] - tz[cp];
                const f32x2 a = __builtin_elementwise_fma(dz, dz, __builtin_elementwise_fma(dy, dy, dx * dx));
                const f32x2 b = __builtin_elementwise_fma(ez, ez, __builtin_elementwise_fma(ey, ey, ex * ex));
                const f32x2 ds = {__builtin_amdgcn_sqrtf(a[0]), __builtin_amdgcn_sqrtf(a[1])};
                const f32x2 dt = {__builtin_amdgcn_sqrtf(b[0]), __builtin_amdgcn_sqrtf(b[1])};
                const f32x2 df = ds - dt;
                f32x2 v = __builtin_elementwise_fma(df * df, ninv2, one2);
                if (CLAMP) v = __builtin_elementwise_max(v, zero2);
                o[rr] = v;
            }
            if (EDGE) {
                const int mc = 2 * cp, jc = j0 + cbase + (mc & 3) + 8 * (mc >> 2);
                const int ir = i0 + r0;
                const bool vj0 = jc < N, vj1 = jc + 1 < N, vi0 = ir < N, vi1 = ir + 1 < N;
                o[0][0] = (vi0 && vj0) ? o[0][0] : 0.f; o[0][1] = (vi0 && vj1) ? o[0][1] : 0.f;
                o[1][0] = (vi1 && vj0) ? o[1][0] : 0.f; o[1][1] = (vi1 && vj1) ? o[1][1] : 0.f;
            }
            d0[cp] = __builtin_bit_cast(unsigned, __builtin_amdgcn_cvt_pknorm_u16(o[0][0], o[0][1]));
            d1[cp] = __builtin_bit_cast(unsigned, __builtin_amdgcn_cvt_pknorm_u16(o[1][0], o[1][1]));
            tr[2 * cp][rp] = __builtin_bit_cast(unsigned, __builtin_amdgcn_cvt_pknorm_u16(o[0][0], o[1][0]));
            tr[2 * cp + 1][rp] = __builtin_bit_cast(unsigned, __builtin_amdgcn_cvt_pknorm_u16(o[0][1], o[1][1]));
        }
        const int i = i0 + r0;
        if (!EDGE || (i < N && colpos < ld)) *reinterpret_cast<u32x4*>(outb + (size_t)i * ld + colpos) = u32x4{d0[0], d0[1], d0[2], d0[3]};
        if (!EDGE || (i + 1 < N && colpos < ld)) *reinterpret_cast<u32x4*>(outb + (size_t)(i + 1) * ld + colpos) = u32x4{d1[0], d1[1], d1[2], d1[3]};
    }
    if (offdiag) {
#pragma unroll
        for (int m = 0; m < 8; ++m) {
            const int j = j0 + cbase + (m & 3) + 8 * (m >> 2);
            if (!EDGE || (j < N && rowpos < ld)) *reinterpret_cast<u32x4*>(outb + (size_t)j * ld + rowpos) = u32x4{tr[m][0], tr[m][1], tr[m][2], tr[m][3]};
        }
    }
}

template <bool CLAMP>
__global__ __launch_bounds__(256) void compat_sym_u16_kernel(const float* __restrict__ src, const float* __restrict__ tgt,
                                                             const float* __restrict__ sigma_spat,
                                                             unsigned short* __restrict__ compat, long long ld, int N, int nt) {
    const int idx = blockIdx.x, b = blockIdx.y;
    int I = (int)(((float)(2 * nt + 1) - __builtin_sqrtf((float)((2 * nt + 1) * (2 * nt + 1) - 8 * idx))) * 0.5f);
    I = max(0, min(I, nt - 1));
    while (I > 0 && I * nt - I * (I - 1) / 2 > idx) --I;
    while ((I + 1) * nt - (I + 1) * I / 2 <= idx) ++I;
    const int J = I + idx - (I * nt - I * (I - 1) / 2);
    __shared__ __attribute__((aligned(16))) float pts[(2 * CF_T + 2 * CF_T / 16) * 8];
    const int i0 = I * CF_T, j0 = J * CF_T;
    const float* srcb = src + (size_t)b * N * 3;
    const float* tgtb = tgt + (size_t)b * N * 3;
    const int t = threadIdx.x;
    {
        const int p = min((t < CF_T ? i0 : j0 - CF_T) + t, N - 1);
        float* d = pts + cf_point_slot(t);
        *reinterpret_cast<f32x4*>(d) = f32x4{srcb[p * 3 + 0], srcb[p * 3 + 1], srcb[p * 3 + 2], 0.f};
        *reinterpret_cast<f32x4*>(d + 4) = f32x4{tgtb[p * 3 + 0], tgtb[p * 3 + 1], tgtb[p * 3 + 2], 0.f};
    }
    const float sg = sigma_spat[0];
    const float s2 = sg * sg;
    const float y0 = __builtin_amdgcn_rcpf(s2);
    const float ninv = -fmaf(fmaf(-s2, y0, 1.0f), y0, y0);
    unsigned short* outb = compat + (size_t)b * N * ld;
    __syncthreads();
    if (i0 + CF_T > N || j0 + CF_T > N)
        compat_fast_tile<true, CLAMP>(pts, outb, ld, N, i0, j0, I != J, ninv);
    else
        compat_fast_tile<false, CLAMP>(pts, outb, ld, N, i0, j0, I != J, ninv);
}

#ifdef PDSC_EXPERIMENTS
constexpr int C16_PITCH = 2 * CS_T + 8;

__global__ __launch_bounds__(256) void compat_sym_u16_exact_kernel(const float* __restrict__ src, const float* __restrict__ tgt,
                                                                   const float* __restrict__ sigma_spat,
                                                                   unsigned short* __restrict__ compat, long long ld, int N) {
    const int I = blockIdx.y, J = blockIdx.x, b = blockIdx.z;
    if (I > J) return;
    __shared__ __attribute__((aligned(16))) unsigned char Ts[CS_STRIP * C16_PITCH];
    __shared__ __attribute__((aligned(16))) float rows_s[CS_T * 8];
    const int i0 = I * CS_T, j0 = J * CS_T;
    const float* srcb = src + (size_t)b * N * 3;
    const float* tgtb = tgt + (size_t)b * N * 3;
    const int t = threadIdx.x;
    if (t < CS_T) {
        const int i = min(i0 + t, N - 1);
        rows_s[t * 8 + 0] = srcb[i * 3 + 0]; rows_s[t * 8 + 1] = srcb[i * 3 + 1]; rows_s[t * 8 + 2] = srcb[i * 3 + 2];
        rows_s[t * 8 + 4] = tgtb[i * 3 + 0]; rows_s[t * 8 + 5] = tgtb[i * 3 + 1]; rows_s[t * 8 + 6] = tgtb[i * 3 + 2];
    }
    const int l32 = t & 31, rg = t >> 5;
    const int jc = j0 + l32 * 4;
    float sx[4], sy[4], sz[4], tx[4], ty[4], tz[4];
#pragma unroll
    for (int c = 0; c < 4; ++c) {
        const int j = min(jc + c, N - 1);
        sx[c] = srcb[j * 3 + 0]; sy[c] = srcb[j * 3 + 1]; sz[c] = srcb[j * 3 + 2];
        tx[c] = tgtb[j * 3 + 0]; ty[c] = tgtb[j * 3 + 1]; tz[c] = tgtb[j * 3 + 2];
    }
    const float sg = sigma_spat[0];
    const float s2 = sg * sg;
    const InvariantDivisor inv(s2);
    unsigned short* outb = compat + (size_t)b * N * ld;
    const bool offdiag = I != J;
    const int jpos = (jc & ~31) + c16_pos(jc & 31);
    __syncthreads();
    for (int strip = 0; strip < CS_T / CS_STRIP; ++strip) {
#pragma unroll
        for (int r = 0; r < 4; ++r) {
            const int sl = rg + 8 * r;
            const int il = strip * CS_STRIP + sl;
            const int i = i0 + il;
            const f32x4 ps = *reinterpret_cast<const f32x4*>(rows_s + il * 8);
            const f32x4 pt = *reinterpret_cast<const f32x4*>(rows_s + il * 8 + 4);
            float o[4];
#pragma unroll
            for (int c = 0; c < 4; ++c) {
                const float ds = dist3<true>(ps[0] - sx[c], ps[1] - sy[c], ps[2] - sz[c]);
                const float dt = dist3<true>(pt[0] - tx[c], pt[1] - ty[c], pt[2] - tz[c]);
                const float v = compat_from_dists<true>(ds, dt, s2, inv);
                o[c] = ((jc + c) < N && i < N) ? v : 0.0f;
            }
            uint2 q;
            q.x = __builtin_bit_cast(unsigned, __builtin_amdgcn_cvt_pknorm_u16(o[0], o[1]));
            q.y = __builtin_bit_cast(unsigned, __builtin_amdgcn_cvt_pknorm_u16(o[2], o[3]));
            if (i < N && jc < ld) *reinterpret_cast<uint2*>(outb + (size_t)i * ld + jpos) = q;
            if (offdiag) *reinterpret_cast<uint2*>(Ts + sl * C16_PITCH + 8 * l32) = q;
        }
        if (offdiag) {
            __syncthreads();
#pragma unroll
            for (int p2 = 0; p2 < 2; ++p2) {
                const int idx = t + 256 * p2, jl = idx >> 2, q = idx & 3;
                unsigned w[4];
#pragma unroll
                for (int m = 0; m < 8; ++m) {
                    const int p = 8 * q + m;
                    const int sl = 8 * ((p >> 2) & 3) + 4 * (p >> 4) + (p & 3);
                    const unsigned v = *reinterpret_cast<const unsigned short*>(Ts + sl * C16_PITCH + 2 * jl);
                    if (m & 1) w[m >> 1] |= v << 16; else w[m >> 1] = v;
                }
                const int j = j0 + jl;
                if (j < N) *reinterpret_cast<u32x4*>(outb + (size_t)j * ld + i0 + strip * CS_STRIP + 8 * q) = u32x4{w[0], w[1], w[2], w[3]};
            }
            __syncthreads();
        }
    }
}
#endif

__global__ void exact_math_selftest_kernel(const float* __restrict__ x, float b, float* __restrict__ sq, float* __restrict__ dv,
                                           long long n) {
    const long long i = (long long)blockIdx.x * 256 + threadIdx.x;
    if (i >= n) return;
    const InvariantDivisor inv(b);
    sq[i] = sqrt_rn(x[i]);
    dv[i] = inv.div(x[i]);
}

}

extern "C" int pdsc_selftest_exact_math(const float* x, float divisor, float* sqrt_out, float* div_out, long long n,
                                        void* stream) {
    PDSC_REQUIRE(x && sqrt_out && div_out && n > 0, "pdsc_selftest_exact_math: bad argument");
    hipLaunchKernelGGL(pdsc::exact_math_selftest_kernel, dim3((unsigned)((n + 255) / 256)), dim3(256), 0, (hipStream_t)stream,
                       x, divisor, sqrt_out, div_out, n);
    return pdsc::check_launch("pdsc_selftest_exact_math");
}

extern "C" long long pdsc_compat_ld(int N) { return N <= 0 ? -1 : pdsc::round_up(N, 64); }

extern "C" int pdsc_spatial_compat(const float* src, const float* tgt, const float* sigma_spat, float* compat,
                                   float* src_dist, long long ld, int bs, int N, void* stream) {
    PDSC_REQUIRE(src && tgt && sigma_spat && compat, "pdsc_spatial_compat: null pointer");
    PDSC_REQUIRE(bs > 0 && N > 0, "pdsc_spatial_compat: bs=%d N=%d", bs, N);
    PDSC_REQUIRE(ld >= N && ld % 4 == 0, "pdsc_spatial_compat: ld=%lld must be >= N and a multiple of 4", ld);
    hipStream_t st = (hipStream_t)stream;
    const dim3 full_grid(pdsc::ceil_div((int)ld, pdsc::CT_COLS), pdsc::ceil_div(N, pdsc::CT_ROWS), bs);
    const int nt = pdsc::ceil_div(N, pdsc::CS_T);
    const dim3 sym_grid(nt, nt, bs);
    pdsc::profile_mark_begin(PDSC_PROF_COMPAT, st);
    if (src_dist)
        hipLaunchKernelGGL((pdsc::compat_kernel<true, true>), full_grid, dim3(256), 0, st, src, tgt, sigma_spat, compat, src_dist, ld, N);
    else {
#ifdef PDSC_EXPERIMENTS
        const int variant = pdsc::env_int("PDSC_COMPAT_VARIANT", PDSC_COMPAT_DEFAULT_VARIANT);
        if (variant == 0)
            hipLaunchKernelGGL((pdsc::compat_kernel<false, false>), full_grid, dim3(256), 0, st, src, tgt, sigma_spat, compat, nullptr, ld, N);
        else if (variant == 1)
            hipLaunchKernelGGL((pdsc::compat_kernel<false, true>), full_grid, dim3(256), 0, st, src, tgt, sigma_spat, compat, nullptr, ld, N);
        else if (variant == 2)
            hipLaunchKernelGGL((pdsc::compat_sym_kernel<false>), sym_grid, dim3(256), 0, st, src, tgt, sigma_spat, compat, ld, N);
        else
#endif
        hipLaunchKernelGGL((pdsc::compat_sym_kernel<true>), sym_grid, dim3(256), 0, st, src, tgt, sigma_spat, compat, ld, N);
    }
    pdsc::profile_mark_end(PDSC_PROF_COMPAT, st);
    return pdsc::check_launch("pdsc_spatial_compat");
}

extern "C" int pdsc_spatial_compat_u16(const float* src, const float* tgt, const float* sigma_spat, unsigned short* compat_u16,
                                       long long ld, int bs, int N, void* stream) {
    PDSC_REQUIRE(src && tgt && sigma_spat && compat_u16, "pdsc_spatial_compat_u16: null pointer");
    PDSC_REQUIRE(bs > 0 && N > 0, "pdsc_spatial_compat_u16: bs=%d N=%d", bs, N);
    PDSC_REQUIRE(ld >= pdsc::round_up(N, 32) && ld % 32 == 0, "pdsc_spatial_compat_u16: ld=%lld must be a multiple of 32 and >= N", ld);
    hipStream_t st = (hipStream_t)stream;
    const int nt = pdsc::ceil_div(N, pdsc::CF_T);
    PDSC_REQUIRE(nt <= 1024, "pdsc_spatial_compat_u16: N=%d too large", N);
    const dim3 grid((unsigned)(nt * (nt + 1) / 2), bs);
    pdsc::profile_mark_begin(PDSC_PROF_COMPAT, st);
#ifdef PDSC_EXPERIMENTS
    const int variant = pdsc::env_int("PDSC_COMPAT16_VARIANT", 2);
    if (variant == 0)
        hipLaunchKernelGGL(pdsc::compat_sym_u16_exact_kernel, dim3(nt, nt, bs), dim3(256), 0, st, src, tgt, sigma_spat, compat_u16, ld, N);
    else if (variant == 1)
        hipLaunchKernelGGL(pdsc::compat_sym_u16_kernel<true>, grid, dim3(256), 0, st, src, tgt, sigma_spat, compat_u16, ld, N, nt);
    else
#endif
    hipLaunchKernelGGL(pdsc::compat_sym_u16_kernel<false>, grid, dim3(256), 0, st, src, tgt, sigma_spat, compat_u16, ld, N, nt);
    pdsc::profile_mark_end(PDSC_PROF_COMPAT, st);
    return pdsc::check_launch("pdsc_spatial_compat_u16");
}
```

pointdsc_amd/csrc/layer.hip:

```cpp
#include <stdlib.h>
#include <type_traits>
#include "pdsc_common.h"
#include "split_layout.h"
#include "merge_partials.h"
#include "layer_args.h"
#include "layer_block.h"

namespace pdsc {

constexpr int LF_ROWS = 32;
constexpr int LF_LD = PDSC_CHANNELS + 4;
constexpr int LF_TILE = LF_ROWS * LF_LD;


#define LF_STAMP(k)                                                                                   \
    if (a.trace && lane == 0) a.trace[(((size_t)blockIdx.y * gridDim.x + blockIdx.x) * 4 + wave) * 16 + (k)] = __builtin_readcyclecounter();

template <int K>
__device__ __forceinline__ void load_w(const float* __restrict__ W, int n0, int l31, int h, f32x4 (&w)[K / 8]) {
    const float* p = W + (size_t)(n0 + l31) * K + 4 * h;
#pragma unroll
    for (int q = 0; q < K / 8; ++q) w[q] = *reinterpret_cast<const f32x4*>(p + 8 * q);
}

// ... 213 lines not shown
            const int n0 = 128 * c + 32 * wave;
            const f32x16 zero = {0.f, 0.f, 0.f, 0.f, 0.f, 0.f, 0.f, 0.f, 0.f, 0.f, 0.f, 0.f, 0.f, 0.f, 0.f, 0.f};
            f32x16 acc = zero;
#pragma unroll
            for (int kk = 0; kk < 8; ++kk) {
                const sp16x8 xh = *reinterpret_cast<const sp16x8*>(Xh + xo + 16 * kk);
                const sp16x8 xl = *reinterpret_cast<const sp16x8*>(Xl + xo + 16 * kk);
                acc = PDSC_MFMA_X3(wl[kk], xh, acc, 0, 0, 0);
                acc = PDSC_MFMA_X3(wh[kk], xl, acc, 0, 0, 0);
                acc = PDSC_MFMA_X3(wh[kk], xh, acc, 0, 0, 0);
            }
            if (c < 2) {
                const sp16* p = a.wq_split + (size_t)(n0 + 128 + l31) * PDSC_CHANNELS + 8 * h;
#pragma unroll
                for (int kk = 0; kk < 8; ++kk) {
                    wh[kk] = *reinterpret_cast<const sp16x8*>(p + 16 * kk);
                    wl[kk] = *reinterpret_cast<const sp16x8*>(p + (size_t)3 * PDSC_CHANNELS * PDSC_CHANNELS + 16 * kk);
                }
            }
            if (c == 0) { LF_STAMP(10) }
            __syncthreads();
            store_tile<false, false>(acc, a.bq, n0, Xa, 32 * wave, l31, h, nullptr);
            __syncthreads();
            if (c == 0) { LF_STAMP(11) }
            if (a.qkv_out) tile_to_global<LF_LD>(Xa, a.qkv_out + 128 * c, 3 * PDSC_CHANNELS, m0, M, t);
            if (a.qs) {
                if (c == 0) tile_to_split<0, LF_LD>(Xa, a.qs + (size_t)m0 * SPL_Q_LD, img, valid, t);
                else if (c == 1) tile_to_split<1, LF_LD>(Xa, nullptr, img, valid, t);
                else tile_to_split<2, LF_LD>(Xa, nullptr, img, valid, t);
            }
            if (c == 0) { LF_STAMP(12) }
        }
        LF_STAMP(13)
    }
}

template <bool T, bool H>
static int launch_layer(const LayerArgs& a, hipStream_t st) {
    if (H && a.wq_split)
        hipLaunchKernelGGL((layer_fused_kernel<T, H, H>), dim3(ceil_div(a.N, LF_ROWS), a.bs), dim3(256), 0, st, a);
    else
        hipLaunchKernelGGL((layer_fused_kernel<T, H, false>), dim3(ceil_div(a.N, LF_ROWS), a.bs), dim3(256), 0, st, a);
    return check_launch("pdsc_layer_run(block)");
}

}

static long long* g_layer_trace = nullptr;
long long* pdsc_layer_trace_buffer(void) { return g_layer_trace; }
extern "C" int pdsc_layer_trace(long long* device_buffer) {
    g_layer_trace = device_buffer;
    return PDSC_OK;
}

extern "C" int pdsc_layer_prefers_block(int bs, int N) {
    return (long long)bs * pdsc::ceil_div(N, pdsc::LF_ROWS) <= 288;
}

namespace pdsc {

int validate_layer_args(const LayerArgs& a, LayerKernel kernel, const char* who) {
    const bool tail = a.msg != nullptr || a.part_o != nullptr, head = a.featB_out != nullptr;
    const bool h3 = kernel == LayerKernel::H3;
    const bool frag = h3 || (kernel == LayerKernel::Wave && (a.wf_tail || a.wf_head));
    const int io = a.io_flags;
    PDSC_REQUIRE(tail || head, "%s: neither tail (msg / partials) nor head (featB_out) requested", who);
    PDSC_REQUIRE(a.bs > 0 && a.N > 0, "%s: bs=%d N=%d", who, a.bs, a.N);
    PDSC_REQUIRE(a.gemm_format == PDSC_LAYER_GEMM_F32 || a.gemm_format == PDSC_LAYER_GEMM_H3, "%s: gemm_format=%d", who, a.gemm_format);
    PDSC_REQUIRE((io & ~(PDSC_IO_PARTIALS_PF | PDSC_IO_RES_PF | PDSC_IO_FEATB_PF)) == 0, "%s: io_flags=%d", who, io);
    PDSC_REQUIRE(h3 || (io == 0 && !a.value_fold), "%s: point-fragment hand-offs and the folded layer exist in the H3 kernel only", who);
    PDSC_REQUIRE(!h3 || a.gemm_format == PDSC_LAYER_GEMM_H3, "%s: point-fragment hand-offs need gemm_format = PDSC_LAYER_GEMM_H3", who);
    PDSC_REQUIRE(!a.value_fold || (io & PDSC_IO_PARTIALS_PF) || !tail, "%s: the folded layer merges point-fragment partials", who);
    if (tail) {
        PDSC_REQUIRE(a.res && (frag ? a.wf_tail != nullptr : a.w1 && a.b1 && a.w2 && a.b2 && a.w3 && a.b3),
                     "%s: tail needs res and fc1..fc3 (natural layout or the tail stream)", who);
        if (!a.msg) PDSC_REQUIRE(a.part_ml && a.nsplit >= 1 && a.nsplit <= layer_merge_limit(kernel) && a.Npad >= a.N,
                                 "%s: partials need part_ml, 1 <= nsplit <= %d (what this launch's kernel merges), Npad >= N", who,
                                 layer_merge_limit(kernel));
        if (!a.msg) PDSC_REQUIRE(a.part_slots == a.nsplit || (h3 && a.part_slots > a.nsplit),
                                 "%s: part_slots=%d (partials per pair in the layout) must be nsplit=%d, or more in the H3 kernels", who,
                                 a.part_slots, a.nsplit);
        PDSC_REQUIRE(!(io & PDSC_IO_PARTIALS_PF) || (!a.msg && a.Npad % 32 == 0), "%s: PF partials come un-merged (msg NULL), Npad a multiple of 32", who);
    } else {
        PDSC_REQUIRE(a.feat_in, "%s: head-only needs feat_in", who);
        PDSC_REQUIRE(!(io & (PDSC_IO_PARTIALS_PF | PDSC_IO_RES_PF)), "%s: head-only takes feat_in in row order", who);
    }
    if (head) PDSC_REQUIRE((a.qkv_out || a.qs) && (frag ? a.wf_head != nullptr : a.wp && a.bp && a.wq && a.bq),
                           "%s: head needs qkv_out or the split streams, and pcn, qkv weights (natural layout or the head stream)", who);
    else PDSC_REQUIRE(a.feat_out && !(io & PDSC_IO_FEATB_PF), "%s: tail-only needs feat_out (row order)", who);
    PDSC_REQUIRE((a.qs == nullptr) == (a.kv == nullptr), "%s: q_split and kv_tiles go together", who);
    PDSC_REQUIRE(!h3 || launch_layer_h3_fits(a, tail, head), "%s: output set not served by the H3 kernel (head: the split streams "
                 "only; tail + head: no feat_out; tail only: feat_out)", who);
    return PDSC_OK;
}

int dispatch_layer(const LayerArgs& a, LayerKernel kernel, hipStream_t st) {
    const bool tail = a.msg != nullptr || a.part_o != nullptr, head = a.featB_out != nullptr;
    if (kernel == LayerKernel::H3) {
        LayerArgs h = a;
        h.stagger_cycles = env_int("PDSC_LAYER_STAGGER", 0);
        h.stagger_mode = env_int("PDSC_LAYER_STAGGER_MODE", 1);
        return launch_layer_h3(h, tail, head, st);
    }
    if (kernel == LayerKernel::Wave) return launch_layer_wave(a, tail, head, st);
    if (kernel == LayerKernel::X3) return launch_layer_x3(a, tail, head, st);
    if (tail && head) {
        profile_mark_begin(PDSC_PROF_LAYER, st);
        const int rc = launch_layer<true, true>(a, st);
        profile_mark_end(PDSC_PROF_LAYER, st);
        return rc;
    }
    if (tail) return launch_layer<true, false>(a, st);
    return launch_layer<false, true>(a, st);
}

}

static bool choose_layer_kernel(const pdsc_layer_call& c, const pdsc::LayerArgs& a, pdsc::LayerKernel* kernel) {
    using pdsc::LayerKernel;
    switch (c.kernel) {
        case PDSC_LAYER_KERNEL_BLOCK: *kernel = LayerKernel::Block; return true;
        case PDSC_LAYER_KERNEL_WAVE: *kernel = LayerKernel::Wave; return true;
        case PDSC_LAYER_KERNEL_H3: *kernel = LayerKernel::H3; return true;
        case PDSC_LAYER_KERNEL_X3: *kernel = LayerKernel::X3; return true;
        case PDSC_LAYER_KERNEL_AUTO: break;
        default: return false;
    }
    if (!a.wf_tail && !a.wf_head) {
        const char* ev = pdsc::env_str("PDSC_LAYER_VARIANT");
        const bool block = ev && (ev[0] == 'b' || ev[0] == 'w') ? ev[0] == 'b' : pdsc_layer_prefers_block(c.bs, c.N) != 0;
        *kernel = block ? LayerKernel::Block : LayerKernel::Wave;
    } else if (c.io_flags != 0) {
        *kernel = LayerKernel::H3;
    } else {
        const bool h3 = c.gemm_format == PDSC_LAYER_GEMM_H3 && pdsc::env_int("PDSC_LAYER_H3_VARIANT", 1) != 0 &&
                        pdsc::launch_layer_h3_fits(a, a.msg != nullptr || a.part_o != nullptr, a.featB_out != nullptr);
        *kernel = h3 ? LayerKernel::H3 : LayerKernel::Wave;
    }
    return true;
}

extern "C" int pdsc_layer_run(const pdsc_layer_call* call, void* stream) {
    PDSC_REQUIRE(call, "pdsc_layer_run: null call");
    const pdsc_layer_call& c = *call;
    const bool natural = c.w1 || c.b1 || c.w2 || c.b2 || c.w3 || c.b3 || c.wp || c.bp || c.wq || c.bq || c.wq_split;
    PDSC_REQUIRE(!natural || (!c.wfrag_tail && !c.wfrag_head), "pdsc_layer_run: weights given in natural layout AND as fragment streams");
    if (c.featB_out && !c.q_split && !c.kv_tiles) PDSC_REQUIRE(c.qkv_out, "pdsc_layer_run: head needs qkv_out when no split streams are given");
    pdsc::LayerArgs a = pdsc::layer_args_from_call(c);
    a.trace = c.io_flags ? nullptr : g_layer_trace;
    pdsc::LayerKernel kernel;
    PDSC_REQUIRE(choose_layer_kernel(c, a, &kernel), "pdsc_layer_run: kernel=%d", c.kernel);
    const int rc = pdsc::validate_layer_args(a, kernel, "pdsc_layer_run");
    return rc != PDSC_OK ? rc : pdsc::dispatch_layer(a, kernel, (hipStream_t)stream);
}
```

pointdsc_amd/csrc/layer_args.h:

```cpp
#pragma once
#include "pdsc_common.h"
#include "merge_partials.h"

namespace pdsc {

struct LayerArgs {
    const float* msg;
    const float* part_o;
    const float* part_ml;
    int nsplit, Npad;
    int part_slots;
    const float* res;
    const float* feat_in;
    float* feat_out;
    float* featB_out;
    float* qkv_out;
    const float *w1, *b1, *w2, *b2, *w3, *b3;
    const float *wp, *bp, *wq, *bq;
    const sp16* wq_split;
    sp16* qs;
    unsigned char* kv;
    int N, bs;
    const unsigned char* wf_tail;
    const unsigned char* wf_head;
    int gemm_format;
    int io_flags;
    int stagger_cycles, stagger_mode;
    long long* trace;
    unsigned int* range_flag;
    int value_fold;
    const int* nvalid;
};

enum class LayerKernel { Block, Wave, H3, X3 };
constexpr int layer_merge_limit(LayerKernel k) {
    return k == LayerKernel::Block ? MERGE_MAX_SPLIT_BLOCK : k == LayerKernel::H3 ? MERGE_MAX_SPLIT_H3 : MERGE_MAX_SPLIT;
}

inline LayerArgs layer_args_from_call(const pdsc_layer_call& c) {
    LayerArgs a{};
    a.msg = c.msg; a.part_o = c.part_o; a.part_ml = c.part_ml; a.nsplit = c.nsplit; a.part_slots = c.nsplit; a.Npad = c.Npad;
    a.res = c.res; a.feat_in = c.feat_in; a.feat_out = c.feat_out; a.featB_out = c.featB_out; a.qkv_out = c.qkv_out;
    a.qs = (sp16*)c.q_split; a.kv = (unsigned char*)c.kv_tiles;
    a.w1 = (const float*)c.w1; a.b1 = c.b1; a.w2 = (const float*)c.w2; a.b2 = c.b2; a.w3 = (const float*)c.w3; a.b3 = c.b3;
    a.wp = (const float*)c.wp; a.bp = c.bp; a.wq = (const float*)c.wq; a.bq = c.bq; a.wq_split = (const sp16*)c.wq_split;
    a.wf_tail = (const unsigned char*)c.wfrag_tail; a.wf_head = (const unsigned char*)c.wfrag_head;
    a.gemm_format = c.gemm_format; a.io_flags = c.io_flags;
    a.N = c.N; a.bs = c.bs;
    return a;
}

int validate_layer_args(const LayerArgs& a, LayerKernel kernel, const char* who);
int dispatch_layer(const LayerArgs& a, LayerKernel kernel, hipStream_t st);

int launch_layer_wave(const LayerArgs& a, bool tail, bool head, hipStream_t st);
int launch_layer_h3(const LayerArgs& a, bool tail, bool head, hipStream_t st);
int launch_layer_h3_coop(const LayerArgs& a, bool tail, bool head, hipStream_t st);
int launch_layer_x3(const LayerArgs& a, bool tail, bool head, hipStream_t st);
bool launch_layer_h3_fits(const LayerArgs& a, bool tail, bool head);
enum class H3Form { TailHeadPF, HeadPF, TailHead, Tail, Head, FoldTailHeadPF, FoldHeadPF, FoldTail, Unserved };
H3Form layer_h3_form(const LayerArgs& a, bool tail, bool head);
int build_value_fold(const float* w1, const float* b1, const float* wqkv, const float* bqkv, const float* w2, const float* b2,
                     const float* w3, const float* b3, const float* wp, const float* bp, float* wfold, void* tail_out, void* head_out,
                     hipStream_t st);

}

long long* pdsc_layer_trace_buffer(void);
```

pointdsc_amd/csrc/layer_coop.hip:

```cpp
#include <type_traits>
#include "pdsc_common.h"
#include "split_layout.h"
#include "merge_partials.h"
#include "layer_args.h"
#include "layer_wave.h"
#include "ragged.h"

namespace pdsc {

constexpr int LC_WAVES = 4;

struct CoopOps { u32x4 v[2][8][2][64]; };

template <bool QKV>
__device__ __forceinline__ void coop_finish(const f32x16& acc, const f32x16& cross, f32x4 (&v)[4]) {
#pragma unroll
    for (int g = 0; g < 4; ++g)
#pragma unroll
        for (int e = 0; e < 4; ++e) v[g][e] = QKV ? acc[4 * g + e] : fmaf(cross[4 * g + e], H3_INV, acc[4 * g + e]);
}

template <bool T, bool H, bool FB_PF, int NB, bool F = false>
__global__ __launch_bounds__(64 * LC_WAVES, NB <= 4 ? 2 : 1) void layer_h3_coop_kernel(LayerArgs a) {
    __shared__ __attribute__((aligned(16))) CoopOps ops;
    __shared__ __attribute__((aligned(16))) float Vs_all[LC_WAVES][32 * LW_VLD];
    const int lane = threadIdx.x & 63;
    const int w = __builtin_amdgcn_readfirstlane(threadIdx.x >> 6);
    const int l31 = lane & 31, h = lane >> 5;
    const int gw = blockIdx.x;
    const TileDesc td = tile_desc(a, gw, l31);
    if (td.valid <= 0) return;
    const int b = td.b, m0 = td.m0, valid = td.valid;
    const bool live = td.live;
    const size_t row = td.row;
    float* Vs = Vs_all[w];
    unsigned char* patch = reinterpret_cast<unsigned char*>(Vs);
    float rmax = 0.f;

    constexpr int K0 = T ? (F ? 2 : 0) : 4, K1 = H ? 12 : 4;
    constexpr int TC = tail_chunks<F>(), HC = head_chunks<F>(), TO = F ? 2 : 0;
    constexpr int VW = F ? LW_FOLD_VW : PDSC_CHANNELS;
    WChunk W[NB];
    const bool low = w < 2;
    auto issue = [&](auto kc) {
        constexpr int k = decltype(kc)::value;
        if constexpr (k >= K0 && k < K1) {
            WChunk& dst = W[k % NB];
            if constexpr (k < 2) { if (low) load_chunk_frag(dst, a.wf_tail, 2 * w + k, TC, k == 0 ? w : -1, lane); }
            else if constexpr (k == 2) { if (low) load_chunk_frag(dst, a.wf_tail, 4 - 2 * TO + w, TC, 2 - TO + w, lane); }
            else if constexpr (k == 3) load_chunk_frag(dst, a.wf_tail, 6 - 2 * TO + w, TC, 4 - TO + w, lane);
            else if constexpr (k < 6) load_chunk_frag(dst, a.wf_head, 2 * w + (k - 4), HC, k == 4 ? w : -1, lane);
            else {
                const int t = w + 4 * ((k - 6) >> 1);
                if (!F || k < 10 || low) load_chunk_frag(dst, a.wf_head, 8 + 2 * t + (k & 1), HC, (k & 1) ? -1 : 4 + t, lane);
            }
        }
    };
    static_for<K0, K0 + NB>([&](auto kc) { issue(kc); });
    f32x16 acc, cross;
    auto run_chunk = [&](auto kc, int set, int c, bool first, auto qkv_c) {
        constexpr int k = decltype(kc)::value;
        u32x4 oh[4], ol[4];
#pragma unroll
        for (int g = 0; g < 4; ++g) { oh[g] = ops.v[set][4 * c + g][0][lane]; ol[g] = ops.v[set][4 * c + g][1][lane]; }
        if (first) acc = bias_step(W[k % NB]);
        if constexpr (decltype(qkv_c)::value) mma_x3(acc, W[k % NB], oh, ol);
        else mma_h3(acc, cross, W[k % NB], oh, ol, first);
        issue(std::integral_constant<int, k + NB>{});
    };
    using std::false_type; using std::true_type;
    auto put = [&](int set, int kk, const u32x4& oh, const u32x4& ol) { ops.v[set][kk][0][lane] = oh; ops.v[set][kk][1][lane] = ol; };
    f32x4 y3[4];
    f32x4 v[4];

    if constexpr (T) {
        f32x4 x0[4];
        if (F && !low) {
        } else if (a.msg) {
#pragma unroll
            for (int q = 0; q < 4; ++q) x0[q] = *reinterpret_cast<const f32x4*>(a.msg + row * VW + 8 * (4 * w + q) + 4 * h);
        } else {
            with_split_count<MERGE_MAX_SPLIT_H3>(a.nsplit, [&](auto ns_tag) {
                constexpr int NS = decltype(ns_tag)::value;
                const size_t slot0 = (size_t)b * a.part_slots * a.Npad + (row - (size_t)b * a.N);
                const MergeWeights<NS> mw = merge_row_weights<NS>(a.part_ml, slot0, (size_t)a.Npad);
                const bool pf = a.io_flags & PDSC_IO_PARTIALS_PF;
                const size_t e0 = pf ? ((size_t)b * a.part_slots * a.Npad + (size_t)td.tile * 32) * VW + lane * 4 : slot0 * VW + 4 * h;
                const int eq = pf ? 256 : 8;
                constexpr int GQ = NB > 4 ? 4 : NS <= 2 ? 4 : NS <= 4 ? 2 : 1;
#pragma unroll
                for (int q0 = 0; q0 < 4; q0 += GQ) {
                    f32x4 pv[GQ][NS];
#pragma unroll
                    for (int q = 0; q < GQ; ++q)
#pragma unroll
                        for (int sp = 0; sp < NS; ++sp) pv[q][sp] = *reinterpret_cast<const f32x4*>(a.part_o + e0 + (size_t)sp * a.Npad * VW + (size_t)eq * (4 * w + q0 + q));
#pragma unroll
                    for (int q = 0; q < GQ; ++q) {
#pragma unroll
                        for (int e = 0; e < 4; ++e) {
                            x0[q0 + q][e] = merge_apply<NS>(pv[q], mw, e);
                            if constexpr (GQ < 4) asm volatile("" : "+v"(x0[q0 + q][e]));
                        }
                    }
                    if constexpr (GQ < 4) __builtin_amdgcn_sched_barrier(0);
                }
            });
        }
        if constexpr (F) {
            if (low) {
                const float* bpr = reinterpret_cast<const float*>(a.wf_tail + LW_FOLD_BPRIME_BYTES);
#pragma unroll
                for (int q = 0; q < 4; ++q) {
                    const f32x4 bv = *reinterpret_cast<const f32x4*>(bpr + 8 * (4 * w + q) + 4 * h);
#pragma unroll
                    for (int e = 0; e < 4; ++e) x0[q][e] = fmaxf(x0[q][e] + bv[e], 0.f);
                }
                u32x4 ph, pl;
                make_kstep<true>(x0[0], x0[1], ph, pl, rmax); put(1, 2 * w, ph, pl);
                make_kstep<true>(x0[2], x0[3], ph, pl, rmax); put(1, 2 * w + 1, ph, pl);
            }
        } else {
            u32x4 ph, pl;
            make_kstep<true>(x0[0], x0[1], ph, pl, rmax); put(0, 2 * w, ph, pl);
            make_kstep<true>(x0[2], x0[3], ph, pl, rmax); put(0, 2 * w + 1, ph, pl);
        }
        {
            const bool pf = a.io_flags & PDSC_IO_RES_PF;
            const float* r0 = a.res + (pf ? (size_t)gw * PF_TILE_FLOATS + lane * 4 : row * PDSC_CHANNELS + 4 * h);
            const int eq = pf ? 256 : 8;
#pragma unroll
            for (int s = 0; s < 4; ++s) y3[s] = *reinterpret_cast<const f32x4*>(r0 + eq * (4 * w + s));
        }
        __syncthreads();

        if constexpr (F) {
        } else if (low) {
            run_chunk(std::integral_constant<int, 0>{}, 0, 0, true, false_type{});
            run_chunk(std::integral_constant<int, 1>{}, 0, 1, false, false_type{});
            coop_finish<false>(acc, cross, v);
#pragma unroll
            for (int s = 0; s < 4; ++s)
#pragma unroll
                for (int e = 0; e < 4; ++e) v[s][e] = fmaxf(v[s][e], 0.f);
            u32x4 ph, pl;
            make_kstep<true>(v[0], v[1], ph, pl, rmax); put(1, 2 * w, ph, pl);
            make_kstep<true>(v[2], v[3], ph, pl, rmax); put(1, 2 * w + 1, ph, pl);
        } else {
            issue(std::integral_constant<int, NB>{});
            issue(std::integral_constant<int, NB + 1>{});
        }
        if constexpr (!F) __syncthreads();

        if (low) {
            run_chunk(std::integral_constant<int, 2>{}, 1, 0, true, false_type{});
            coop_finish<false>(acc, cross, v);
#pragma unroll
            for (int s = 0; s < 4; ++s)
#pragma unroll
                for (int e = 0; e < 4; ++e) v[s][e] = fmaxf(v[s][e], 0.f);
            u32x4 ph, pl;
            make_kstep<true>(v[0], v[1], ph, pl, rmax); put(0, 2 * w, ph, pl);
            make_kstep<true>(v[2], v[3], ph, pl, rmax); put(0, 2 * w + 1, ph, pl);
        } else {
            issue(std::integral_constant<int, NB + 2>{});
        }
        __syncthreads();

        run_chunk(std::integral_constant<int, 3>{}, 0, 0, true, false_type{});
        coop_finish<false>(acc, cross, v);
#pragma unroll
        for (int s = 0; s < 4; ++s) {
#pragma unroll
            for (int e = 0; e < 4; ++e) y3[s][e] = y3[s][e] + v[s][e];
            if constexpr (!H) *reinterpret_cast<f32x4*>(a.feat_out + row * PDSC_CHANNELS + 32 * w + 8 * s + 4 * h) = y3[s];
        }
    } else {
#pragma unroll
        for (int s = 0; s < 4; ++s) y3[s] = *reinterpret_cast<const f32x4*>(a.feat_in + row * PDSC_CHANNELS + 32 * w + 8 * s + 4 * h);
    }

    if constexpr (H) {
        {
            u32x4 ph, pl;
            make_kstep<true>(y3[0], y3[1], ph, pl, rmax); put(1, 2 * w, ph, pl);
            make_kstep<true>(y3[2], y3[3], ph, pl, rmax); put(1, 2 * w + 1, ph, pl);
        }
        __syncthreads();

        run_chunk(std::integral_constant<int, 4>{}, 1, 0, true, false_type{});
        run_chunk(std::integral_constant<int, 5>{}, 1, 1, false, false_type{});
        coop_finish<false>(acc, cross, v);
#pragma unroll
        for (int s = 0; s < 4; ++s) {
#pragma unroll
            for (int e = 0; e < 4; ++e) v[s][e] = fmaxf(v[s][e], 0.f);
            if constexpr (FB_PF) *reinterpret_cast<f32x4*>(a.featB_out + (size_t)gw * PF_TILE_FLOATS + pf_offset_floats(4 * w + s) + lane * 4) = v[s];
            else *reinterpret_cast<f32x4*>(patch + l31 * LW_PROW + 32 * s + 16 * h) = v[s];
        }
        if constexpr (!FB_PF) {
            wave_lds_sync();
#pragma unroll
            for (int it = 0; it < 4; ++it) {
                const int pt = 8 * it + (lane >> 3), piece = lane & 7;
                const u32x4 ev = *reinterpret_cast<const u32x4*>(patch + pt * LW_PROW + 16 * piece);
                *reinterpret_cast<u32x4*>(a.featB_out + ((size_t)m0 + min(pt, valid - 1)) * PDSC_CHANNELS + 32 * w + 4 * piece) = ev;
            }
            wave_lds_sync();
        }
        {
            u32x4 ph, pl;
            make_kstep<false>(v[0], v[1], ph, pl, rmax); put(0, 2 * w, ph, pl);
            make_kstep<false>(v[2], v[3], ph, pl, rmax); put(0, 2 * w + 1, ph, pl);
        }
        __syncthreads();

        unsigned char* img = a.kv + (size_t)gw * SPL_TILE_STRIDE;
        const int n0 = 32 * w;

        run_chunk(std::integral_constant<int, 6>{}, 0, 0, true, true_type{});
        run_chunk(std::integral_constant<int, 7>{}, 0, 1, false, true_type{});
        coop_finish<true>(acc, cross, v);
#pragma unroll
        for (int s = 0; s < 4; ++s) range_note(rmax, v[s]);
#pragma unroll
        for (int s = 0; s < 4; ++s) {
            unsigned hi[2], lo[2];
            split4(v[s], hi, lo);
            *reinterpret_cast<u32x4*>(patch + l31 * LW_PROW + 64 * h + 16 * s) = chunk_for_store(hi, lo);
        }
        wave_lds_sync();
#pragma unroll
        for (int it = 0; it < 4; ++it) {
            const int pt = 8 * it + (lane >> 3), piece = lane & 7;
            const u32x4 ev = *reinterpret_cast<const u32x4*>(patch + pt * LW_PROW + 16 * piece);
            sp16* dst = a.qs + ((size_t)m0 + min(pt, valid - 1)) * SPL_Q_LD + (piece >> 2) * PDSC_CHANNELS + n0 + 8 * (piece & 3);
            *reinterpret_cast<u32x4*>(dst) = ev;
        }

        run_chunk(std::integral_constant<int, 8>{}, 0, 0, true, true_type{});
        run_chunk(std::integral_constant<int, 9>{}, 0, 1, false, true_type{});
        coop_finish<true>(acc, cross, v);
#pragma unroll
        for (int s = 0; s < 4; ++s) range_note(rmax, v[s]);
#pragma unroll
        for (int s = 0; s < 4; ++s) {
            f32x4 z = v[s];
#pragma unroll
            for (int e = 0; e < 4; ++e) z[e] = live ? z[e] : 0.f;
            unsigned hi[2], lo[2];
            split4(z, hi, lo);
            *reinterpret_cast<u32x4*>(img + (h ? SPL_KL : SPL_KH) + spl_k_offset(l31, 4 * w + s)) = chunk_for_store(hi, lo);
        }

        if (F && !low) { range_report(a.range_flag, b, rmax); return; }
        run_chunk(std::integral_constant<int, 10>{}, 0, 0, true, true_type{});
        run_chunk(std::integral_constant<int, 11>{}, 0, 1, false, true_type{});
        coop_finish<true>(acc, cross, v);
#pragma unroll
        for (int s = 0; s < 4; ++s) range_note(rmax, v[s]);
        wave_lds_sync();
#pragma unroll
        for (int s = 0; s < 4; ++s) {
            f32x4 z = v[s];
#pragma unroll
            for (int e = 0; e < 4; ++e) z[e] = live ? z[e] : 0.f;
            *reinterpret_cast<f32x4*>(Vs + l31 * LW_VLD + 8 * s + 4 * h) = z;
        }
        wave_lds_sync();
#pragma unroll
        for (int it = 0; it < 2; ++it) {
            const int cl = 16 * it + (lane >> 2), jh = lane & 3;
            float vt[8];
#pragma unroll
            for (int e = 0; e < 8; ++e) vt[e] = Vs[spl_v_key(jh, e) * LW_VLD + cl];
            unsigned chi[4], clo[4];
#pragma unroll
            for (int e = 0; e < 8; e += 2) split2(vt[e], vt[e + 1], chi[e / 2], clo[e / 2]);
            const int off = spl_v_offset_w<VW>(n0 + cl, jh);
            *reinterpret_cast<u32x4*>(img + SPL_VH + off) = u32x4{chi[0], chi[1], chi[2], chi[3]};
            *reinterpret_cast<u32x4*>(img + (F ? spl_v_lo<LW_FOLD_VW>() : SPL_VL) + off) = u32x4{clo[0], clo[1], clo[2], clo[3]};
        }
    }
    range_report(a.range_flag, b, rmax);
}

int launch_layer_h3_coop(const LayerArgs& a, bool tail, bool head, hipStream_t st) {
    const dim3 grid(a.bs * ceil_div(a.N, 32)), block(64 * LC_WAVES);
    switch (layer_h3_form(a, tail, head)) {
        case H3Form::FoldTailHeadPF: hipLaunchKernelGGL((layer_h3_coop_kernel<true, true, true, 4, true>), grid, block, 0, st, a); break;
        case H3Form::FoldHeadPF: hipLaunchKernelGGL((layer_h3_coop_kernel<false, true, true, 4, true>), grid, block, 0, st, a); break;
        case H3Form::FoldTail: hipLaunchKernelGGL((layer_h3_coop_kernel<true, false, false, 4, true>), grid, block, 0, st, a); break;
        case H3Form::TailHeadPF: hipLaunchKernelGGL((layer_h3_coop_kernel<true, true, true, 4>), grid, block, 0, st, a); break;
        case H3Form::HeadPF: hipLaunchKernelGGL((layer_h3_coop_kernel<false, true, true, 4>), grid, block, 0, st, a); break;
        case H3Form::TailHead: hipLaunchKernelGGL((layer_h3_coop_kernel<true, true, false, 4>), grid, block, 0, st, a); break;
        case H3Form::Tail: hipLaunchKernelGGL((layer_h3_coop_kernel<true, false, false, 4>), grid, block, 0, st, a); break;
        case H3Form::Head: hipLaunchKernelGGL((layer_h3_coop_kernel<false, true, false, 4>), grid, block, 0, st, a); break;
        case H3Form::Unserved: return PDSC_ERR_ARG;
    }
    return check_launch("pdsc_layer_run(h3, four wavefronts per tile)");
}

}
```

pointdsc_amd/csrc/layer_h3.hip:

```cpp
#include <stdlib.h>
#include <type_traits>
#include "pdsc_common.h"
#include "split_layout.h"
#include "merge_partials.h"
#include "layer_args.h"
#include "layer_wave.h"

namespace pdsc {

constexpr int PDSC_H3_COOP_TILES = 2560;

#define LH_STAMP(k) \
    if (TRACE && lane == 0) a.trace[(size_t)gw * 64 + (k)] = __builtin_readcyclecounter();

template <bool F = false>
constexpr int stage_tiles(int stage) { return stage == ST_FC1 || stage == ST_FC2 ? 2 : stage == ST_FC3 || stage == ST_PCN ? 4 : F ? 10 : 12; }

template <bool T, bool H, bool TRACE = false, int PIPE = 6, int EXP = 0, bool FB_PF = false, int NWV = LW_WAVES, int NBUF = 2, bool F = false>
__global__ __launch_bounds__(64 * NWV, NBUF > 2 ? 1 : 2) void layer_h3_kernel(LayerArgs a) {
    __shared__ __attribute__((aligned(16))) float Vs_all[NWV][32 * LW_VLD];
    const int lane = threadIdx.x & 63;
    const int wave = __builtin_amdgcn_readfirstlane(threadIdx.x >> 6);
    const int l31 = lane & 31, h = lane >> 5;
    const int tpp = ceil_div_dev(a.N, 32);
    const int gw = blockIdx.x * NWV + wave;
    if (gw >= a.bs * tpp) return;
    const int b = gw / tpp, tile = gw - b * tpp;
    const int m0 = b * a.N + tile * 32;
    const int valid = min(32, (a.nvalid ? a.nvalid[b] : a.N) - tile * 32);
    if (valid <= 0) return;
    const bool live = l31 < valid;
    const size_t row = (size_t)m0 + min(l31, valid - 1);
    float* Vs = Vs_all[wave];
    unsigned char* patch = reinterpret_cast<unsigned char*>(Vs);

    if (a.stagger_cycles > 0 && blockIdx.x < 512) {
        unsigned hwid;
        asm volatile("s_getreg_b32 %0, hwreg(HW_REG_HW_ID)" : "=s"(hwid));
        const bool late = a.stagger_mode == 1 ? (hwid & 1u) : a.stagger_mode == 2 ? (blockIdx.x & 1) : ((blockIdx.x >> 8) & 1);
        if (late) {
            const long long t0 = __builtin_readcyclecounter();
            while (__builtin_readcyclecounter() - t0 < a.stagger_cycles) __builtin_amdgcn_s_sleep(32);
        }
    }
    LH_STAMP(0)
    float rmax = 0.f;
    constexpr int NCH = num_chunks<T, H, F>();
    constexpr int VW = F ? LW_FOLD_VW : PDSC_CHANNELS;
    constexpr int NQ = VW / 8;
    WChunk w[NBUF];
    static_for<0, NBUF - 1>([&](auto jc) {
        constexpr int j = decltype(jc)::value;
        if constexpr (j < NCH) load_chunk<T, true, true, F>(w[j], a, j, lane);
    });

    u32x4 a0h[8], a0l[8], a1h[4], a1l[4], a2h[4], a2l[4], ayh[8], ayl[8], xqh[8], xql[8];
    f32x4 y3[16];
    if (T) {
        f32x4 x0[16];
        auto first_operand = [&](int kk) __attribute__((always_inline)) {
            if constexpr (F) {
                const float* bpr = reinterpret_cast<const float*>(a.wf_tail + LW_FOLD_BPRIME_BYTES);
#pragma unroll
                for (int u = 0; u < 2; ++u) {
                    const f32x4 bv = *reinterpret_cast<const f32x4*>(bpr + 8 * (2 * kk + u) + 4 * h);
#pragma unroll
                    for (int e = 0; e < 4; ++e) x0[2 * kk + u][e] = fmaxf(x0[2 * kk + u][e] + bv[e], 0.f);
                }
                make_kstep<true>(x0[2 * kk], x0[2 * kk + 1], a1h[kk], a1l[kk], rmax);
            } else {
                make_kstep<true>(x0[2 * kk], x0[2 * kk + 1], a0h[kk], a0l[kk], rmax);
            }
        };
        if (a.msg) {
#pragma unroll
            for (int q = 0; q < NQ; ++q) x0[q] = *reinterpret_cast<const f32x4*>(a.msg + row * VW + 8 * q + 4 * h);
#pragma unroll
            for (int kk = 0; kk < NQ / 2; ++kk) first_operand(kk);
        } else {
            with_split_count<MERGE_MAX_SPLIT_H3>(a.nsplit, [&](auto ns_tag) {
                constexpr int NS = decltype(ns_tag)::value;
                constexpr int GQ = (NS <= 2 ? 16 : NS <= 4 ? 8 : 4) < NQ ? (NS <= 2 ? 16 : NS <= 4 ? 8 : 4) : NQ;
                const size_t slot0 = (size_t)b * a.part_slots * a.Npad + (row - (size_t)b * a.N);
                const bool pf = a.io_flags & PDSC_IO_PARTIALS_PF;
                const size_t e0 = pf ? ((size_t)b * a.part_slots * a.Npad + (size_t)tile * 32) * VW + lane * 4 : slot0 * VW + 4 * h;
                const int eq = pf ? 256 : 8;
                const MergeWeights<NS> mw = merge_row_weights<NS>(a.part_ml, slot0, (size_t)a.Npad);
#pragma unroll
                for (int q0 = 0; q0 < NQ; q0 += GQ) {
                    f32x4 pv[GQ][NS];
#pragma unroll
                    for (int q = 0; q < GQ; ++q)
#pragma unroll
                        for (int sp = 0; sp < NS; ++sp)
                            pv[q][sp] = (EXP & 4) ? f32x4{1.f, 2.f, 3.f, (float)lane}
                                                  : *reinterpret_cast<const f32x4*>(a.part_o + e0 + (size_t)sp * a.Npad * VW + eq * (q0 + q));
#pragma unroll
                    for (int q = 0; q < GQ; ++q) {
#pragma unroll
                        for (int e = 0; e < 4; ++e) {
                            x0[q0 + q][e] = merge_apply<NS>(pv[q], mw, e);
                            asm volatile("" : "+v"(x0[q0 + q][e]));
                        }
                    }
#pragma unroll
                    for (int kk = q0 / 2; kk < (q0 + GQ) / 2; ++kk) first_operand(kk);
                    __builtin_amdgcn_sched_barrier(0);
                }
            });
        }
    } else {
#pragma unroll
        for (int q = 0; q < 16; ++q) y3[q] = *reinterpret_cast<const f32x4*>(a.feat_in + row * PDSC_CHANNELS + 8 * q + 4 * h);
#pragma unroll
        for (int kk = 0; kk < 8; ++kk) make_kstep<true>(y3[2 * kk], y3[2 * kk + 1], ayh[kk], ayl[kk], rmax);
    }
    LH_STAMP(1)

    unsigned char* img = H ? a.kv + (size_t)gw * SPL_TILE_STRIDE : nullptr;
    f32x16 acc, cross;
    f32x4 vp[4];
    u32x4 ev = {0u, 0u, 0u, 0u};
    float vt[8];

    auto epi = [&](auto stage_c, auto tile_c, auto sc, f32x4 (&v)[4]) {
        constexpr ChunkDesc d = {decltype(stage_c)::value, decltype(tile_c)::value, 0, 0};
        constexpr int s = decltype(sc)::value;
        constexpr int n0 = 32 * d.tile;
        if constexpr (d.stage == ST_FC1 || d.stage == ST_FC2) {
            if constexpr (s < 4) {
#pragma unroll
                for (int e = 0; e < 4; ++e) v[s][e] = fmaxf(v[s][e], 0.f);
                if constexpr (s & 1)
                    make_kstep<true>(v[s - 1], v[s], (d.stage == ST_FC1 ? a1h : a2h)[2 * d.tile + (s >> 1)],
                                     (d.stage == ST_FC1 ? a1l : a2l)[2 * d.tile + (s >> 1)], rmax);
            }
        } else if constexpr (d.stage == ST_FC3) {
            if constexpr (s < 4) {
#pragma unroll
                for (int e = 0; e < 4; ++e) y3[4 * d.tile + s][e] = y3[4 * d.tile + s][e] + v[s][e];
                if constexpr (!H && !(EXP & 2)) *reinterpret_cast<f32x4*>(a.feat_out + row * PDSC_CHANNELS + n0 + 8 * s + 4 * h) = y3[4 * d.tile + s];
                if constexpr (H && (s & 1))
                    make_kstep<true>(y3[4 * d.tile + s - 1], y3[4 * d.tile + s], ayh[2 * d.tile + (s >> 1)], ayl[2 * d.tile + (s >> 1)], rmax);
            }
        } else if constexpr (d.stage == ST_PCN) {
            if constexpr (s < 4) {
#pragma unroll
                for (int e = 0; e < 4; ++e) v[s][e] = fmaxf(v[s][e], 0.f);
                if constexpr (FB_PF) {
                    if constexpr (!(EXP & (2 | 64))) *reinterpret_cast<f32x4*>(a.featB_out + (size_t)gw * PF_TILE_FLOATS + pf_offset_floats(4 * d.tile + s) + lane * 4) = v[s];
                } else
                    patch_put_featB(patch, lane, s, v[s]);
            }
            if constexpr (!FB_PF) {
                if constexpr (s == 3) wave_lds_sync();
                if constexpr (s >= 4) {
                    const int pt = min(patch_line_row(lane, s - 4), valid - 1);
                    if constexpr (!(EXP & 2)) *reinterpret_cast<u32x4*>(featB_line(a.featB_out, (size_t)m0 + pt, n0, lane)) = ev;
                    else asm volatile("" :: "v"(ev));
                }
                if constexpr (s >= 3 && s < 7) ev = patch_line(patch, lane, s - 3);
            }
            if constexpr (s == 4 || s == 5)
                make_kstep<false>(v[2 * (s - 4)], v[2 * (s - 4) + 1], xqh[2 * d.tile + (s - 4)], xql[2 * d.tile + (s - 4)], rmax);
        } else {
            if constexpr (s < 4) range_note(rmax, v[s]);
            {
                if constexpr (d.tile >= 4 && d.tile < 8) {
                    if constexpr (s < 4) {
                        const u32x4 ck = k_chunk(v[s], live);
                        if constexpr (!(EXP & (2 | 16))) k_chunk_store(img, lane, 4 * (d.tile - 4) + s, ck);
                        else asm volatile("" :: "v"(ck));
                    }
                } else if constexpr (d.tile < 4) {
                    if constexpr (s < 4) {
                        unsigned hi[2], lo[2];
                        split4(v[s], hi, lo);
                        *reinterpret_cast<u32x4*>(patch + l31 * LW_PROW + 64 * h + 16 * s) = chunk_for_store(hi, lo);
                    }
                    if constexpr (s == 3) wave_lds_sync();
                    if constexpr (s >= 4) {
                        const int pt = 8 * (s - 4) + (lane >> 3), piece = lane & 7;
                        sp16* dst = a.qs + ((size_t)m0 + min(pt, valid - 1)) * SPL_Q_LD + (piece >> 2) * PDSC_CHANNELS + n0 + 8 * (piece & 3);
                        if constexpr (!(EXP & (2 | 8))) *reinterpret_cast<u32x4*>(dst) = ev;
                        else asm volatile("" :: "v"(ev), "v"(dst));
                    }
                    if constexpr (s >= 3 && s < 7) ev = patch_line(patch, lane, s - 3);
                } else {
                    if constexpr (s < 4) vt_put(Vs, lane, s, zero_unless(live, v[s]));
                    if constexpr (s == 3) wave_lds_sync();
                    if constexpr (s == 4 || s == 6) vt_gather(Vs, lane, (s - 4) >> 1, vt);
                    if constexpr (s == 5 || s == 7) {
                        u32x4 ch, cl;
                        vt_split(vt, ch, cl);
                        const int off = vt_offset<VW>(lane, (s - 5) >> 1, 32 * (d.tile - 8));
                        if constexpr (!(EXP & (2 | 32))) vt_store<VW>(img, off, ch, cl);
                        else asm volatile("" :: "v"(ch), "v"(cl), "v"(off));
                    }
                }
            }
        }
    };

    static_for<0, NCH>([&](auto ic) {
        constexpr int i = decltype(ic)::value;
        constexpr ChunkDesc d = chunk_desc<T, F>(i);
        if constexpr (i + NBUF - 1 < NCH && !((EXP & 1) && i >= 1)) load_chunk<T, true, true, F>(w[(i + NBUF - 1) % NBUF], a, i + NBUF - 1, lane);
        if constexpr (T && d.stage == ST_FC2 && d.tile == 0 && !(EXP & 4)) {
            const bool pf = a.io_flags & PDSC_IO_RES_PF;
            const float* r0 = a.res + (pf ? (size_t)gw * PF_TILE_FLOATS + lane * 4 : row * PDSC_CHANNELS + 4 * h);
            const int eq = pf ? 256 : 8;
#pragma unroll
            for (int q = 0; q < 16; ++q) y3[q] = *reinterpret_cast<const f32x4*>(r0 + eq * q);
        }
        const WChunk& wc = w[i % NBUF];
        if constexpr (d.chunk == 0) acc = bias_step(wc);
        constexpr bool pending = d.tile > 0;
        using StageC = std::integral_constant<int, d.stage>;
        using PrevC = std::integral_constant<int, d.tile - 1>;
        static_for<0, 4>([&](auto gc) {
            constexpr int g = decltype(gc)::value;
            if constexpr (d.stage == ST_QKV) {
                const sp16x8 wh = __builtin_bit_cast(sp16x8, wc.v[2 * g]), wl = __builtin_bit_cast(sp16x8, wc.v[2 * g + 1]);
                const sp16x8 bh = __builtin_bit_cast(sp16x8, xqh[4 * d.chunk + g]), bl = __builtin_bit_cast(sp16x8, xql[4 * d.chunk + g]);
                acc = PDSC_MFMA_X3(wl, bh, acc, 0, 0, 0);
                acc = PDSC_MFMA_X3(wh, bl, acc, 0, 0, 0);
                acc = PDSC_MFMA_X3(wh, bh, acc, 0, 0, 0);
            } else {
                const u32x4* oh = d.stage == ST_FC1 ? a0h : d.stage == ST_FC2 ? a1h : d.stage == ST_FC3 ? a2h : ayh;
                const u32x4* ol = d.stage == ST_FC1 ? a0l : d.stage == ST_FC2 ? a1l : d.stage == ST_FC3 ? a2l : ayl;
                const f32x16 zero = {0.f, 0.f, 0.f, 0.f, 0.f, 0.f, 0.f, 0.f, 0.f, 0.f, 0.f, 0.f, 0.f, 0.f, 0.f, 0.f};
                const f16x8 wh = __builtin_bit_cast(f16x8, wc.v[2 * g]), wl = __builtin_bit_cast(f16x8, wc.v[2 * g + 1]);
                const f16x8 bh = __builtin_bit_cast(f16x8, oh[4 * d.chunk + g]), bl = __builtin_bit_cast(f16x8, ol[4 * d.chunk + g]);
                cross = __builtin_amdgcn_mfma_f32_32x32x16_f16(wl, bh, (d.chunk == 0 && g == 0) ? zero : cross, 0, 0, 0);
                acc = __builtin_amdgcn_mfma_f32_32x32x16_f16(wh, bh, acc, 0, 0, 0);
                cross = __builtin_amdgcn_mfma_f32_32x32x16_f16(wh, bl, cross, 0, 0, 0);
            }
            if constexpr (pending) {
                if constexpr (d.nchunks == 2) {
                    epi(StageC{}, PrevC{}, std::integral_constant<int, 4 * d.chunk + g>{}, vp);
                } else {
                    epi(StageC{}, PrevC{}, std::integral_constant<int, 2 * g>{}, vp);
                    epi(StageC{}, PrevC{}, std::integral_constant<int, 2 * g + 1>{}, vp);
                }
            }
        });
        if constexpr (d.chunk == d.nchunks - 1) {
#pragma unroll
            for (int g = 0; g < 4; ++g)
#pragma unroll
                for (int e = 0; e < 4; ++e) vp[g][e] = d.stage != ST_QKV ? fmaf(cross[4 * g + e], H3_INV, acc[4 * g + e]) : acc[4 * g + e];
            if constexpr (d.tile == stage_tiles<F>(d.stage) - 1) {
                static_for<0, 8>([&](auto sc) { epi(StageC{}, std::integral_constant<int, d.tile>{}, sc, vp); });
            }
        }
        if constexpr (PIPE > 0) {
#pragma unroll
            for (int k = 0; k < 13; ++k) {
                __builtin_amdgcn_sched_group_barrier(0x008, 1, 0);
                __builtin_amdgcn_sched_group_barrier(0x002, PIPE, 0);
            }
        }
        LH_STAMP(2 + i)
        __builtin_amdgcn_sched_barrier(0);
    });

    LH_STAMP(63)
    range_report(a.range_flag, b, rmax);
}

bool launch_layer_h3_fits(const LayerArgs& a, bool tail, bool head) {
    if (a.gemm_format != PDSC_LAYER_GEMM_H3) return false;
    if (head && (!a.qs || !a.kv || a.qkv_out)) return false;
    if (tail && head && a.feat_out) return false;
    if (tail && !head && !a.feat_out) return false;
    return a.wf_tail || !tail;
}

H3Form layer_h3_form(const LayerArgs& a, bool tail, bool head) {
    const bool fb_pf = a.io_flags & PDSC_IO_FEATB_PF;
    if (a.value_fold) {
        if (tail && head && fb_pf) return H3Form::FoldTailHeadPF;
        if (head && !tail && fb_pf) return H3Form::FoldHeadPF;
        if (tail && !head) return H3Form::FoldTail;
        set_error("pdsc_layer_run(h3): the folded layer exists with point-fragment featB only");
        return H3Form::Unserved;
    }
    if (head && fb_pf) return tail ? H3Form::TailHeadPF : H3Form::HeadPF;
    return tail && head ? H3Form::TailHead : tail ? H3Form::Tail : H3Form::Head;
}

static void h3_launch_shape(int tiles, int* nwv, int* nbuf) {
    *nwv = LW_WAVES; *nbuf = 2;
    (void)tiles;
#ifdef PDSC_EXPERIMENTS
    const int force = env_int("PDSC_LAYER_H3_SHAPE", 0);
    if (force == 42 || force == 23 || force == 13 || force == 24 || force == 14 || force == 22) { *nwv = force / 10; *nbuf = force % 10; }
#endif
}

int launch_layer_h3(const LayerArgs& a, bool tail, bool head, hipStream_t st) {
    const int waves = a.bs * ceil_div(a.N, 32);
    int nwv, nbuf;
    h3_launch_shape(waves, &nwv, &nbuf);
    if (a.value_fold) { nwv = LW_WAVES; nbuf = 2; }
    const dim3 grid(ceil_div(waves, nwv)), block(64 * nwv);
    const H3Form form = layer_h3_form(a, tail, head);
    if (form == H3Form::Unserved) return PDSC_ERR_ARG;
    const bool timed = tail && head;
    int coop_tiles = PDSC_H3_COOP_TILES;
#ifdef PDSC_EXPERIMENTS
    coop_tiles = env_int("PDSC_LAYER_H3_COOP", coop_tiles);
#endif
    if (waves <= coop_tiles && !a.trace) {
        if (timed) profile_mark_begin(PDSC_PROF_LAYER, st);
        const int rc = launch_layer_h3_coop(a, tail, head, st);
        if (timed) profile_mark_end(PDSC_PROF_LAYER, st);
        return rc;
    }
    if (timed) profile_mark_begin(PDSC_PROF_LAYER, st);
#ifdef PDSC_EXPERIMENTS
#define PDSC_H3_LAUNCH_EXTRA(TT, HH, PF)                                                                                            \
        if (nwv == 1 && nbuf == 4) hipLaunchKernelGGL((layer_h3_kernel<TT, HH, false, 6, 0, PF, 1, 4>), grid, block, 0, st, a);      \
        else if (nwv == 2 && nbuf == 3) hipLaunchKernelGGL((layer_h3_kernel<TT, HH, false, 6, 0, PF, 2, 3>), grid, block, 0, st, a); \
        else if (nwv == 1 && nbuf == 3) hipLaunchKernelGGL((layer_h3_kernel<TT, HH, false, 6, 0, PF, 1, 3>), grid, block, 0, st, a); \
        else if (nwv == 2 && nbuf == 4) hipLaunchKernelGGL((layer_h3_kernel<TT, HH, false, 6, 0, PF, 2, 4>), grid, block, 0, st, a); \
        else if (nwv == 2 && nbuf == 2) hipLaunchKernelGGL((layer_h3_kernel<TT, HH, false, 6, 0, PF, 2, 2>), grid, block, 0, st, a); \
        else
#else
#define PDSC_H3_LAUNCH_EXTRA(TT, HH, PF)
#endif
#define PDSC_H3_LAUNCH(TT, HH, PF)                                                                                                  \
    do {                                                                                                                            \
        PDSC_H3_LAUNCH_EXTRA(TT, HH, PF)                                                                                            \
        hipLaunchKernelGGL((layer_h3_kernel<TT, HH, false, 6, 0, PF>), grid, block, 0, st, a);                                       \
    } while (0)
    switch (form) {
        case H3Form::FoldTailHeadPF: hipLaunchKernelGGL((layer_h3_kernel<true, true, false, 6, 0, true, LW_WAVES, 2, true>), grid, block, 0, st, a); break;
        case H3Form::FoldHeadPF: hipLaunchKernelGGL((layer_h3_kernel<false, true, false, 6, 0, true, LW_WAVES, 2, true>), grid, block, 0, st, a); break;
        case H3Form::FoldTail: hipLaunchKernelGGL((layer_h3_kernel<true, false, false, 6, 0, false, LW_WAVES, 2, true>), grid, block, 0, st, a); break;
        case H3Form::TailHeadPF: {
#ifdef PDSC_LAYER_DIAG
            const int ex = env_int("PDSC_LAYER_H3_EXP", 0);
            if (ex == 1) hipLaunchKernelGGL((layer_h3_kernel<true, true, false, 6, 1, true>), grid, block, 0, st, a);
            else if (ex == 2) hipLaunchKernelGGL((layer_h3_kernel<true, true, false, 6, 2, true>), grid, block, 0, st, a);
            else if (ex == 4) hipLaunchKernelGGL((layer_h3_kernel<true, true, false, 6, 4, true>), grid, block, 0, st, a);
            else if (ex == 7) hipLaunchKernelGGL((layer_h3_kernel<true, true, false, 6, 7, true>), grid, block, 0, st, a);
            else if (ex == 8) hipLaunchKernelGGL((layer_h3_kernel<true, true, false, 6, 8, true>), grid, block, 0, st, a);
            else if (ex == 16) hipLaunchKernelGGL((layer_h3_kernel<true, true, false, 6, 16, true>), grid, block, 0, st, a);
            else if (ex == 32) hipLaunchKernelGGL((layer_h3_kernel<true, true, false, 6, 32, true>), grid, block, 0, st, a);
            else if (ex == 64) hipLaunchKernelGGL((layer_h3_kernel<true, true, false, 6, 64, true>), grid, block, 0, st, a);
            else
#endif
            PDSC_H3_LAUNCH(true, true, true);
            break;
        }
        case H3Form::HeadPF: PDSC_H3_LAUNCH(false, true, true); break;
        case H3Form::TailHead:
#ifdef PDSC_EXPERIMENTS
            if (a.trace) hipLaunchKernelGGL((layer_h3_kernel<true, true, true>), dim3(ceil_div(waves, LW_WAVES)), dim3(64 * LW_WAVES), 0, st, a);
            else
#endif
            PDSC_H3_LAUNCH(true, true, false);
            break;
        case H3Form::Tail: PDSC_H3_LAUNCH(true, false, false); break;
        case H3Form::Head: PDSC_H3_LAUNCH(false, true, false); break;
        case H3Form::Unserved: break;
    }
#undef PDSC_H3_LAUNCH
#undef PDSC_H3_LAUNCH_EXTRA
    if (timed) profile_mark_end(PDSC_PROF_LAYER, st);
    return check_launch("pdsc_layer_run(h3)");
}

}

using namespace pdsc;

extern "C" int pdsc_layer_h3_uses_coop(int bs, int N) {
    if (bs <= 0 || N <= 0) return 0;
    int coop_tiles = PDSC_H3_COOP_TILES;
#ifdef PDSC_EXPERIMENTS
    coop_tiles = env_int("PDSC_LAYER_H3_COOP", coop_tiles);
#endif
    return (long long)bs * ceil_div(N, 32) <= coop_tiles ? 1 : 0;
}
```

pointdsc_amd/csrc/linear.hip:

```cpp
#include "pdsc_common.h"
#include "gram_tile.h"
#include "ragged.h"

namespace pdsc {

constexpr int LIN_BM = 64;

struct LinearArgs {
    const float* X; long long ldx; long long x_batch;
    const int* row_idx; long long idx_batch;
    const float* W; long long w_batch;
    const float* bias;
    const float* R; long long ldr;
    float* Y; long long ldy; long long y_batch;
    int M, K, Nout, relu;
    const float* sigma;
};

template <int NT, int MODE>
__global__ __launch_bounds__(256) void linear_kernel(LinearArgs a) {
    extern __shared__ __attribute__((aligned(16))) float lds[];
    const int K = a.K, KP = K + 4, K4 = K >> 2;
    float* Xs = lds;
    float* Ws = lds + LIN_BM * KP;
    const int t = threadIdx.x, lane = t & 63, wave = t >> 6;
    const int b = blockIdx.z;
    const int m0 = blockIdx.y * LIN_BM;
    const int n0 = blockIdx.x * (64 * NT);
    const float* X = a.X + (size_t)b * a.x_batch;
    const float* W = a.W + (size_t)b * a.w_batch;
    const int* ridx = a.row_idx ? a.row_idx + (size_t)b * a.idx_batch : nullptr;

    for (int idx = t; idx < LIN_BM * K4; idx += 256) {
        const int row = idx / K4, c = idx - row * K4;
        int m = m0 + row;
        f32x4 v = {0.f, 0.f, 0.f, 0.f};
        if (m < a.M) {
            if (ridx) m = ridx[m];
            v = *reinterpret_cast<const f32x4*>(X + (size_t)m * a.ldx + c * 4);
        }
        *reinterpret_cast<f32x4*>(Xs + row * KP + c * 4) = v;
    }
    for (int idx = t; idx < 64 * NT * K4; idx += 256) {
        const int row = idx / K4, c = idx - row * K4;
        const int n = n0 + row;
        f32x4 v = {0.f, 0.f, 0.f, 0.f};
        if (n < a.Nout) v = *reinterpret_cast<const f32x4*>(W + (size_t)n * K + c * 4);
        *reinterpret_cast<f32x4*>(Ws + row * KP + c * 4) = v;
    }
    __syncthreads();

    const int wm = wave & 1, wn = wave >> 1;
    const int l31 = lane & 31, h = lane >> 5;
    f32x16 acc[NT];
#pragma unroll
    for (int nt = 0; nt < NT; ++nt)
#pragma unroll
        for (int r = 0; r < 16; ++r) acc[nt][r] = 0.f;

    const float* xa = Xs + (wm * 32 + l31) * KP + 4 * h;
    const float* wb = Ws + ((wn * NT) * 32 + l31) * KP + 4 * h;
    const int nq = K >> 3;
    for (int q = 0; q < nq; ++q) {
        const f32x4 av = *reinterpret_cast<const f32x4*>(xa + 8 * q);
        f32x4 bv[NT];
#pragma unroll
        for (int nt = 0; nt < NT; ++nt) bv[nt] = *reinterpret_cast<const f32x4*>(wb + nt * 32 * KP + 8 * q);
#pragma unroll
        for (int e = 0; e < 4; ++e)
#pragma unroll
            for (int nt = 0; nt < NT; ++nt)
                acc[nt] = __builtin_amdgcn_mfma_f32_32x32x2f32(av[e], bv[nt][e], acc[nt], 0, 0, 0);
    }

    float* Y = a.Y + (size_t)b * a.y_batch;
#pragma unroll
    for (int nt = 0; nt < NT; ++nt) {
        const int n = n0 + (wn * NT + nt) * 32 + l31;
        if (n >= a.Nout) continue;
        const float bval = (MODE == 0 && a.bias) ? a.bias[n] : 0.f;
        float sig2 = 1.f;
        if (MODE == 2) { const float sg = a.sigma[0]; sig2 = sg * sg; }
#pragma unroll
        for (int r = 0; r < 16; ++r) {
            const int i = (r & 3) + 8 * (r >> 2) + 4 * h;
            const int m = m0 + wm * 32 + i;
            if (m >= a.M) continue;
            float v = acc[nt][r];
            if (MODE == 0) {
                v = v + bval;
                if (a.relu) v = fmaxf(v, 0.f);
                if (a.R) v = a.R[(size_t)m * a.ldr + n] + v;
            } else if (MODE == 1) {
                v = 2.0f - 2.0f * v;
            } else {
                v = fminf(fmaxf(1.0f - (1.0f - v) / sig2, 0.0f), 1.0f);
                if (m == n) v = 0.0f;
            }
            Y[(size_t)m * a.ldy + n] = v;
        }
    }
}

constexpr int L0_MAX_BLOCKS = 2048;
constexpr int L0_LD = 16;
template <int KD>
__global__ __launch_bounds__(256) void layer0_kernel(const float* __restrict__ corr, int in_dim,
                                                     const float* __restrict__ W0, const float* __restrict__ b0,
                                                     float* __restrict__ feat, int M, unsigned int* __restrict__ range_flag, int bs) {
    if (range_flag && blockIdx.x == 0)
        for (int i = threadIdx.x; i < bs; i += 256) range_flag[i] = 0u;
    const int c4 = (threadIdx.x & 31) * 4, rl = threadIdx.x >> 5;
    float w[4][KD], bias[4];
#pragma unroll
    for (int c = 0; c < 4; ++c) {
#pragma unroll
        for (int d4 = 0; d4 < KD; d4 += 4) {
            const f32x4 v = *reinterpret_cast<const f32x4*>(W0 + (c4 + c) * L0_LD + d4);
#pragma unroll
            for (int d = 0; d < 4; ++d) w[c][d4 + d] = v[d];
        }
        bias[c] = b0[c4 + c];
    }
    for (long long row = (long long)blockIdx.x * 8 + rl; row < M; row += (long long)gridDim.x * 8) {
        float x[KD];
#pragma unroll
        for (int d = 0; d < KD; ++d) x[d] = d < in_dim ? corr[row * in_dim + d] : 0.f;
        f32x4 o;
#pragma unroll
        for (int c = 0; c < 4; ++c) {
            float s = 0.f;
#pragma unroll
            for (int d = 0; d < KD; ++d) s = fmaf(x[d], w[c][d], s);
            o[c] = s + bias[c];
        }
        *reinterpret_cast<f32x4*>(feat + row * PDSC_CHANNELS + c4) = o;
    }
}

constexpr int CH_ROWS = 128, CH_K = PDSC_CHANNELS, CH_H = 32;
constexpr int CH_XLD = CH_K + 4, CH_W2LD = CH_H + 4;
struct ClassifierLds {
    float W1[CH_H * CH_XLD];
    float W2[CH_H * CH_W2LD];
    float b1[CH_H], b2[CH_H];
    float X[CH_ROWS * CH_XLD];
};

__global__ __launch_bounds__(256) void classifier_hidden_kernel(const float* __restrict__ X, const float* __restrict__ W1,
                                                               const float* __restrict__ b1, const float* __restrict__ W2,
                                                               const float* __restrict__ b2, float* __restrict__ H2, int M) {
    extern __shared__ __attribute__((aligned(16))) unsigned char lds_raw[];
    ClassifierLds& sh = *reinterpret_cast<ClassifierLds*>(lds_raw);
    const int t = threadIdx.x, lane = t & 63, wave = t >> 6, l31 = lane & 31, h = lane >> 5;
    const int num_tiles = ceil_div_dev(M, CH_ROWS);
    for (int idx = t; idx < CH_H * (CH_K / 4); idx += 256) {
        const int row = idx / (CH_K / 4), c = idx - row * (CH_K / 4);
        *reinterpret_cast<f32x4*>(sh.W1 + row * CH_XLD + 4 * c) = *reinterpret_cast<const f32x4*>(W1 + (size_t)row * CH_K + 4 * c);
    }
    for (int idx = t; idx < CH_H * (CH_H / 4); idx += 256) {
        const int row = idx / (CH_H / 4), c = idx - row * (CH_H / 4);
        *reinterpret_cast<f32x4*>(sh.W2 + row * CH_W2LD + 4 * c) = *reinterpret_cast<const f32x4*>(W2 + (size_t)row * CH_H + 4 * c);
    }
    if (t < CH_H) { sh.b1[t] = b1[t]; sh.b2[t] = b2[t]; }
    f32x4 stage[16];
    auto load_tile = [&](int tile) {
#pragma unroll
        for (int i = 0; i < 16; ++i) {
            const int m = tile * CH_ROWS + (t >> 5) + 8 * i;
            stage[i] = m < M ? *reinterpret_cast<const f32x4*>(X + (size_t)m * CH_K + 4 * (t & 31)) : f32x4{0.f, 0.f, 0.f, 0.f};
        }
    };
    int tile = blockIdx.x;
    if (tile < num_tiles) load_tile(tile);
    for (; tile < num_tiles; tile += gridDim.x) {
        __syncthreads();
#pragma unroll
        for (int i = 0; i < 16; ++i) *reinterpret_cast<f32x4*>(sh.X + ((t >> 5) + 8 * i) * CH_XLD + 4 * (t & 31)) = stage[i];
        __syncthreads();
        if (tile + gridDim.x < num_tiles) load_tile(tile + gridDim.x);
        f32x16 acc;
#pragma unroll
        for (int r = 0; r < 16; ++r) acc[r] = 0.f;
        const float* wa = sh.W1 + l31 * CH_XLD + 4 * h;
        const float* xb = sh.X + (wave * 32 + l31) * CH_XLD + 4 * h;
#pragma unroll
        for (int q = 0; q < CH_K / 8; ++q) {
            const f32x4 av = *reinterpret_cast<const f32x4*>(wa + 8 * q);
            const f32x4 bv = *reinterpret_cast<const f32x4*>(xb + 8 * q);
#pragma unroll
            for (int e = 0; e < 4; ++e) acc = __builtin_amdgcn_mfma_f32_32x32x2f32(av[e], bv[e], acc, 0, 0, 0);
        }
        f32x4 h1[4];
#pragma unroll
        for (int q = 0; q < 4; ++q)
#pragma unroll
            for (int e = 0; e < 4; ++e) h1[q][e] = fmaxf(acc[4 * q + e] + sh.b1[e + 8 * q + 4 * h], 0.f);
        f32x16 acc2;
#pragma unroll
        for (int r = 0; r < 16; ++r) acc2[r] = 0.f;
        const float* wa2 = sh.W2 + l31 * CH_W2LD + 4 * h;
#pragma unroll
        for (int q = 0; q < CH_H / 8; ++q) {
            const f32x4 av = *reinterpret_cast<const f32x4*>(wa2 + 8 * q);
#pragma unroll
            for (int e = 0; e < 4; ++e) acc2 = __builtin_amdgcn_mfma_f32_32x32x2f32(av[e], h1[q][e], acc2, 0, 0, 0);
        }
        const int m = tile * CH_ROWS + wave * 32 + l31;
        if (m < M) {
#pragma unroll
            for (int g = 0; g < 4; ++g) {
                f32x4 o;
#pragma unroll
                for (int e = 0; e < 4; ++e) o[e] = fmaxf(acc2[4 * g + e] + sh.b2[e + 8 * g + 4 * h], 0.f);
                *reinterpret_cast<f32x4*>(H2 + (size_t)m * CH_H + 8 * g + 4 * h) = o;
            }
        }
    }
// ... 83 lines not shown
            const int col = tile * GR_COLS + 32 * sub + l31;
            if (col < a.N) {
#pragma unroll
                for (int r = 0; r < 16; ++r) {
                    const int row = r0 + (r & 3) + 8 * (r >> 2) + 4 * h;
                    if (row < a.R) {
                        float v;
                        if (MODE == 1) v = 2.0f - 2.0f * acc[r];
                        else {
                            v = feature_compat_clamp(feature_compat_raw(acc[r], sig2));
                            if (row == col) v = 0.0f;
                        }
                        Yb[(size_t)row * a.ldy + col] = v;
                    }
                }
            }
        }
        if (tile + 1 < t1) {
            store_tile(lds + ((tile + 1 - t0) & 1) * GR_COLS * GR_LD);
            __syncthreads();
        }
    }
}

template <int MODE, int GR_COLS>
static int launch_gram_cols(GramArgs a, int bs, hipStream_t st) {
    const size_t lds_bytes = 2 * (size_t)GR_COLS * GR_LD * sizeof(float);
    const int rc_lds = ensure_dynamic_lds(reinterpret_cast<const void*>(&gram_rows_kernel<MODE, GR_COLS>), lds_bytes, "gram_rows(dynamic LDS)");
    if (rc_lds != PDSC_OK) return rc_lds;
    const int row_blocks = ceil_div(a.R, GR_ROWS), tiles = ceil_div(a.N, GR_COLS);
    int splits = ceil_div(GR_COLS == 32 ? 1536 : 768, row_blocks * bs);
    if (splits > tiles) splits = tiles;
    if (splits < 1) splits = 1;
    a.tiles_per_split = ceil_div(tiles, splits);
    splits = ceil_div(tiles, a.tiles_per_split);
    hipLaunchKernelGGL((gram_rows_kernel<MODE, GR_COLS>), dim3(splits, row_blocks, bs), dim3(256), lds_bytes, st, a);
    return check_launch("gram_rows_kernel");
}
template <int MODE>
static int launch_gram(GramArgs a, int bs, hipStream_t st) {
    return env_int("PDSC_GRAM_COLS", 64) == 32 ? launch_gram_cols<MODE, 32>(a, bs, st) : launch_gram_cols<MODE, 64>(a, bs, st);
}

int knn_dist_rows(const float* normed, const int* seeds, float* dist, long long ldd, int bs, int N, int S,
                  hipStream_t st) {
    GramArgs a{};
    a.X = normed; a.row_idx = seeds; a.Y = dist; a.ldy = ldd; a.R = S; a.N = N;
    return launch_gram<1>(a, bs, st);
}

}

extern "C" int pdsc_feature_compat(const float* normed, const float* sigma, float* Mout, long long ld, int bs, int N,
                                   void* stream) {
    PDSC_REQUIRE(normed && sigma && Mout, "pdsc_feature_compat: null pointer");
    PDSC_REQUIRE(bs > 0 && N > 0 && ld >= N, "pdsc_feature_compat: bs=%d N=%d ld=%lld", bs, N, ld);
    pdsc::GramArgs a{};
    a.X = normed; a.sigma = sigma; a.Y = Mout; a.ldy = ld; a.R = N; a.N = N;
    return pdsc::launch_gram<2>(a, bs, (hipStream_t)stream);
}

extern "C" int pdsc_linear(const float* X, long long ldx, const float* W, const float* bias, const float* residual,
                           long long ldr, float* Y, long long ldy, int M, int K, int Nout, int relu, void* stream) {
    PDSC_REQUIRE(X && W && Y, "pdsc_linear: null pointer");
    PDSC_REQUIRE(M > 0 && Nout > 0, "pdsc_linear: M=%d Nout=%d", M, Nout);
    PDSC_REQUIRE(K >= 8 && K <= 128 && K % 8 == 0, "pdsc_linear: K=%d must be a multiple of 8 in [8,128]", K);
    PDSC_REQUIRE(ldx >= K && ldx % 4 == 0, "pdsc_linear: ldx=%lld", ldx);
    PDSC_REQUIRE(ldy >= Nout, "pdsc_linear: ldy=%lld < Nout", ldy);
    PDSC_REQUIRE(!residual || ldr >= Nout, "pdsc_linear: ldr=%lld < Nout", ldr);
    pdsc::LinearArgs a{};
    a.X = X; a.ldx = ldx; a.W = W; a.bias = bias; a.R = residual; a.ldr = ldr; a.Y = Y; a.ldy = ldy;
    a.M = M; a.K = K; a.Nout = Nout; a.relu = relu;
    hipStream_t st = (hipStream_t)stream;
    if (Nout > 64) return pdsc::launch_linear<2, 0>(a, 1, st);
    return pdsc::launch_linear<1, 0>(a, 1, st);
}

namespace pdsc {
int launch_layer0(const float* corr_pos, int in_dim, const float* W0, const float* b0, float* feat, int M, unsigned int* range_flag, int bs,
                  hipStream_t st) {
    PDSC_REQUIRE(corr_pos && W0 && b0 && feat, "pdsc_layer0: null pointer");
    PDSC_REQUIRE(in_dim >= 1 && in_dim <= 16 && M > 0, "pdsc_layer0: in_dim=%d (1..16) M=%d", in_dim, M);
    const int blocks = ceil_div(M, 8) < L0_MAX_BLOCKS ? ceil_div(M, 8) : L0_MAX_BLOCKS;
    if (in_dim <= 8)
        hipLaunchKernelGGL(layer0_kernel<8>, dim3((unsigned)blocks), dim3(256), 0, st, corr_pos, in_dim, W0, b0, feat, M, range_flag, bs);
    else
        hipLaunchKernelGGL(layer0_kernel<16>, dim3((unsigned)blocks), dim3(256), 0, st, corr_pos, in_dim, W0, b0, feat, M, range_flag, bs);
    return check_launch("pdsc_layer0");
}
}

extern "C" int pdsc_layer0(const float* corr_pos, int in_dim, const float* W0, const float* b0, float* feat, int M,
                           void* stream) {
    return pdsc::launch_layer0(corr_pos, in_dim, W0, b0, feat, M, nullptr, 0, (hipStream_t)stream);
}

extern "C" int pdsc_classifier_hidden(const float* feat, const float* W1, const float* b1, const float* W2, const float* b2, float* h2,
                                      int M, void* stream) {
    PDSC_REQUIRE(feat && W1 && b1 && W2 && b2 && h2 && M > 0, "pdsc_classifier_hidden: bad argument");
    return pdsc::launch_classifier_hidden(feat, W1, b1, W2, b2, h2, M, (hipStream_t)stream);
}
```

pointdsc_amd/csrc/ragged.h:

```cpp
#pragma once
#include "pdsc_common.h"

namespace pdsc {

int launch_nms_keys_grid(const float* src, const float* conf, float radius, float* keys, void* workspace, size_t workspace_bytes,
                         int bs, int N, const int* nvalid, hipStream_t st);
int launch_rank_select(const float* keys, int* seeds, int bs, int N, int num_seeds, const int* nvalid, const int* svalid, hipStream_t st,
                       unsigned int* conv_mask_init = nullptr);
int launch_seed_solve_forward(const float* normed, const float* src, const float* tgt, const int* knn_idx, const float* sigma,
                              const float* sigma_spat, float* eig_iters, unsigned int* conv_mask, float* seed_trans, float* seed_weights,
                              int bs, int N, int S, int k, int num_iterations, bool mask_ready, hipStream_t st);
int launch_select_and_refine(const int* counts, const float* seed_trans, const float* src, const float* tgt, float inlier_threshold,
                             float refine_threshold, int max_iters, int* best, float* initial_trans, float* labels, float* final_trans,
                             int* solves, int bs, int N, int S, const int* nvalid, hipStream_t st, int* trace, const unsigned int* range_flag,
                             unsigned int* range_report = nullptr);
int launch_knn_seeds(const float* normed, const int* seeds, float* dist_scratch, int* knn_idx, int bs, int N, int S, int k,
                     const int* nvalid, hipStream_t st);
bool knn_seeds_uses_fused(int bs, int N, int S, int k);
int launch_knn_seeds_form(const float* normed, const float* normed_pf, const int* seeds, float* dist_scratch, int* knn_idx, int bs, int N,
                          int S, int k, const int* nvalid, int form, hipStream_t st);
int launch_normalize_conf_pf(const float* feat, const float* h2, const float* w3, const float* b3, float* normed, float* normed_pf,
                             float* conf, int bs, int N, hipStream_t st);
int launch_score_hypotheses_slp(const float* seed_trans, const float* src, const float* tgt, float thr2, int* counts, int bs, int N, int S,
                                const int* nvalid, hipStream_t st);
float*& score_debug_slot();
int launch_score_hypotheses(const float* seed_trans, const float* src, const float* tgt, float inlier_threshold, int* counts, int bs,
                            int N, int S, const int* nvalid, hipStream_t st);
int launch_select_best(const int* counts, const float* seed_trans, const float* src, const float* tgt, float inlier_threshold, int* best,
                       float* best_trans, float* labels, int bs, int N, int S, const int* nvalid, hipStream_t st);
int launch_post_refinement(const float* initial_trans, const float* src, const float* tgt, float threshold, int max_iters,
                           float* final_trans, int* solves, int bs, int N, const int* nvalid, hipStream_t st, int* trace = nullptr,
                           const unsigned int* range_flag = nullptr);
int launch_layer0(const float* corr_pos, int in_dim, const float* W0, const float* b0, float* feat, int M, unsigned int* range_flag, int bs,
                  hipStream_t st);
constexpr int PDSC_REFINE_TRACE = 24;
int launch_attention_split_ex(const void* q_split, const void* kv_tiles, const void* compat, int compat_format, long long ld,
                              float* msg, void* scratch, size_t scratch_bytes, int bs, int N, int nsplit, int partial_layout,
                              const int* nvalid, hipStream_t st, int value_width = PDSC_CHANNELS);

constexpr int PDSC_ATT_MAX_LEAVES = 8;
int attention_leaf_count(int N);
int leaf_plan(int bs, int N, int leaves_mode, int* nw_out, int* nsplit_out, int* nleaf_out);
int launch_attention_leaves(const void* q_split, const void* kv_tiles, const void* compat, int compat_format, long long ld,
                            void* scratch, size_t scratch_bytes, int bs, int N, int leaves_mode, const int* nvalid, int n_min,
                            hipStream_t st, int value_width = PDSC_CHANNELS);

}
```

Baseline: 2558 pairs/s.

## Fuse layer0 into first head kernel and classifier into last tail kernel

On the point-fragment fused encoder route, the first layer's head kernel now computes the layer0 linear projection from corr_pos in registers instead of reading a layer0 feature buffer. The final tail kernel also runs the classifier MLP, normalization and confidence output directly from its registers. The range-flag clearing that the layer0 kernel used to do is moved into the compat kernel's first block. This removes the separate layer0, classifier-hidden and normalize launches and their feature round-trips through memory. The cost is heavier kernel variants with possibly more register pressure, and an override knob that selects which ends are fused.

After: 2568 pairs/s (median of 6 runs). About the same (+0.4%).

```diff
diff --git a/include/pointdsc_hip.h b/include/pointdsc_hip.h
--- a/include/pointdsc_hip.h
+++ b/include/pointdsc_hip.h
@@ -185,6 +185,8 @@
 
 int pdsc_attention_leaf_split_override(int d);
 
+int pdsc_encoder_ends_override(int mode);
+
 int pdsc_layer_trace(long long* device_buffer);
 
 int pdsc_classifier_hidden(const float* feat, const float* W1, const float* b1, const float* W2, const float* b2, float* h2,
diff --git a/pointdsc_amd/_lib.py b/pointdsc_amd/_lib.py
--- a/pointdsc_amd/_lib.py
+++ b/pointdsc_amd/_lib.py
@@ -79,6 +79,7 @@
     "pdsc_attention_leaf_scratch_bytes": (_sz, [_i, _i, _i]),
     "pdsc_attention_trace": (_i, [_vp]),
     "pdsc_attention_leaf_split_override": (_i, [_i]),
+    "pdsc_encoder_ends_override": (_i, [_i]),
     "pdsc_layer_trace": (_i, [_vp]),
     "pdsc_sc_attention_split": (_i, [_vp, _vp, _vp, _ll, _vp, _vp, _sz, _i, _i, _i, _vp]),
     "pdsc_sc_attention_split_u16": (_i, [_vp, _vp, _vp, _ll, _vp, _vp, _sz, _i, _i, _i, _vp]),
diff --git a/pointdsc_amd/csrc/api.hip b/pointdsc_amd/csrc/api.hip
--- a/pointdsc_amd/csrc/api.hip
+++ b/pointdsc_amd/csrc/api.hip
@@ -15,6 +15,8 @@
     static thread_local unsigned int* slot = nullptr;
     return slot;
 }
+
+static int g_encoder_ends_override = 0;
 
 void set_error(const char* fmt, ...) {
     va_list ap;
@@ -280,6 +282,12 @@
     range_report_slot() = host_words;
     return PDSC_OK;
 }
+extern "C" int pdsc_encoder_ends_override(int mode) {
+    PDSC_REQUIRE(mode >= 0 && mode <= 4, "pdsc_encoder_ends_override: mode=%d (0 = the planner decides, 1 = separate launches, 2 = fused, "
+                 "3 / 4 = the head / the tail alone fused)", mode);
+    g_encoder_ends_override = mode;
+    return PDSC_OK;
+}
 extern "C" int pdsc_experiments_enabled(void) {
 #ifdef PDSC_EXPERIMENTS
     return 1;
@@ -373,6 +381,8 @@
     int nleaf, value_width;
     int leaf_ns;
     int ws_tail, ws_head;
+    bool head_layer0;
+    bool tail_finish;
 };
 
 static int plan_encoder(const pdsc_config* cfg, int bs, int N, const int* nvalid, int n_min, EncoderPlan* plan) {
@@ -417,6 +427,8 @@
     p.value_width = p.fold ? PDSC_CHANNELS / 2 : PDSC_CHANNELS;
     p.ws_tail = p.fold ? PDSC_WS_FOLD_TAIL_H3 : h3 ? PDSC_WS_FRAG_TAIL_H3 : PDSC_WS_FRAG_TAIL;
     p.ws_head = p.fold ? PDSC_WS_FOLD_HEAD_H3 : h3 ? PDSC_WS_FRAG_HEAD_H3 : PDSC_WS_FRAG_HEAD;
+    p.head_layer0 = p.pf && g_encoder_ends_override != 1 && g_encoder_ends_override != 4;
+    p.tail_finish = p.pf && g_encoder_ends_override != 1 && g_encoder_ends_override != 3;
     return PDSC_OK;
 }
 
@@ -506,12 +518,18 @@
     return x.c.probe ? launch_absmax(v, count, x.c.probe + kind, x.st) : PDSC_OK;
 }
 
+static bool head_computes_layer0(const ForwardCtx& x) { return x.plan.fused && x.plan.head_layer0 && x.c.mode != ForwardMode::Probe; }
+static bool tail_finishes_encoder(const ForwardCtx& x) { return x.plan.fused && x.plan.tail_finish && x.c.mode != ForwardMode::Probe; }
+
 static int run_compat_layer0(const ForwardCtx& x) {
     const ForwardCall& c = x.c;
+    const bool in_head = head_computes_layer0(x);
+    unsigned int* clear = in_head ? x.range_flag : nullptr;
     if (x.cfmt == PDSC_COMPAT_U16)
-        PDSC_TRY(pdsc_spatial_compat_u16(c.src, c.tgt, x.W(PDSC_W_SIGMA_SPAT, 0), (unsigned short*)x.compat, x.ld, c.bs, c.N, x.st));
+        PDSC_TRY(launch_spatial_compat_u16(c.src, c.tgt, x.W(PDSC_W_SIGMA_SPAT, 0), (unsigned short*)x.compat, x.ld, c.bs, c.N, clear, x.st));
     else
-        PDSC_TRY(pdsc_spatial_compat(c.src, c.tgt, x.W(PDSC_W_SIGMA_SPAT, 0), x.compat, nullptr, x.ld, c.bs, c.N, x.st));
+        PDSC_TRY(launch_spatial_compat(c.src, c.tgt, x.W(PDSC_W_SIGMA_SPAT, 0), x.compat, nullptr, x.ld, c.bs, c.N, clear, x.st));
+    if (in_head) return PDSC_OK;
     PDSC_TRY(launch_layer0(c.corr_pos, c.cfg->in_dim, x.W(PDSC_W_LAYER0_W, 0), x.W(PDSC_W_LAYER0_B, 0), x.featA, x.M, x.range_flag, c.bs, x.st));
     return probe_absmax(x, PDSC_RANGE_LAYER0, x.featA, (size_t)x.M * PDSC_CHANNELS);
 }
@@ -564,6 +582,16 @@
     if (plan.pf) {
         a.value_fold = plan.fold;
         a.range_flag = x.range_flag;
+        if (!tail && head_computes_layer0(x)) {
+            a.feat_in = nullptr;
+            a.corr_pos = x.c.corr_pos; a.in_dim = x.c.cfg->in_dim;
+            a.w0 = x.W(PDSC_W_LAYER0_W, 0); a.b0 = x.W(PDSC_W_LAYER0_B, 0);
+        }
+        if (last && tail_finishes_encoder(x)) {
+            a.cls_w1 = x.W(PDSC_W_CLS1_W, 0); a.cls_b1 = x.W(PDSC_W_CLS1_B, 0); a.cls_w2 = x.W(PDSC_W_CLS2_W, 0);
+            a.cls_b2 = x.W(PDSC_W_CLS2_B, 0); a.cls_w3 = x.W(PDSC_W_CLS3_W, 0); a.cls_b3 = x.W(PDSC_W_CLS3_B, 0);
+            a.normed = x.normed; a.normed_pf = x.normed_pf; a.conf = x.conf;
+        }
     } else
         a.trace = pdsc_layer_trace_buffer();
     PDSC_TRY(validate_layer_args(a, plan.kernel, "pdsc_forward_testing(layer)"));
@@ -637,16 +665,18 @@
     const ForwardCall& c = x.c;
     const int C = PDSC_CHANNELS, M = x.M;
     float *h1 = x.L.at<float>(c.workspace, WS_H1), *h2 = x.L.at<float>(c.workspace, WS_H2);
-    if (env_int("PDSC_CLS_FUSED", 1))
-        PDSC_TRY(launch_classifier_hidden(x.featA, x.W(PDSC_W_CLS1_W, 0), x.W(PDSC_W_CLS1_B, 0), x.W(PDSC_W_CLS2_W, 0), x.W(PDSC_W_CLS2_B, 0), h2, M, x.st));
-    else {
-        PDSC_TRY(pdsc_linear(x.featA, C, x.W(PDSC_W_CLS1_W, 0), x.W(PDSC_W_CLS1_B, 0), nullptr, 0, h1, 32, M, C, 32, 1, x.st));
-        PDSC_TRY(pdsc_linear(h1, 32, x.W(PDSC_W_CLS2_W, 0), x.W(PDSC_W_CLS2_B, 0), nullptr, 0, h2, 32, M, 32, 32, 1, x.st));
-    }
-    if (x.normed_pf)
-        PDSC_TRY(launch_normalize_conf_pf(x.featA, h2, x.W(PDSC_W_CLS3_W, 0), x.W(PDSC_W_CLS3_B, 0), x.normed, x.normed_pf, x.conf, c.bs, c.N, x.st));
-    else
-        PDSC_TRY(pdsc_normalize_confidence(x.featA, h2, x.W(PDSC_W_CLS3_W, 0), x.W(PDSC_W_CLS3_B, 0), x.normed, x.conf, M, x.st));
+    if (!tail_finishes_encoder(x)) {
+        if (env_int("PDSC_CLS_FUSED", 1))
+            PDSC_TRY(launch_classifier_hidden(x.featA, x.W(PDSC_W_CLS1_W, 0), x.W(PDSC_W_CLS1_B, 0), x.W(PDSC_W_CLS2_W, 0), x.W(PDSC_W_CLS2_B, 0), h2, M, x.st));
+        else {
+            PDSC_TRY(pdsc_linear(x.featA, C, x.W(PDSC_W_CLS1_W, 0), x.W(PDSC_W_CLS1_B, 0), nullptr, 0, h1, 32, M, C, 32, 1, x.st));
+            PDSC_TRY(pdsc_linear(h1, 32, x.W(PDSC_W_CLS2_W, 0), x.W(PDSC_W_CLS2_B, 0), nullptr, 0, h2, 32, M, 32, 32, 1, x.st));
+        }
+        if (x.normed_pf)
+            PDSC_TRY(launch_normalize_conf_pf(x.featA, h2, x.W(PDSC_W_CLS3_W, 0), x.W(PDSC_W_CLS3_B, 0), x.normed, x.normed_pf, x.conf, c.bs, c.N, x.st));
+        else
+            PDSC_TRY(pdsc_normalize_confidence(x.featA, h2, x.W(PDSC_W_CLS3_W, 0), x.W(PDSC_W_CLS3_B, 0), x.normed, x.conf, M, x.st));
+    }
     if (c.mode == ForwardMode::Testing) {
         PDSC_TRY(launch_nms_keys_grid(c.src, x.conf, c.cfg->nms_radius, x.keys, x.L.at<void>(c.workspace, WS_NMS_WS),
                                       pdsc_nms_workspace_bytes(c.bs, c.N), c.bs, c.N, c.nvalid, x.st));
@@ -703,6 +733,9 @@
     PDSC_TRY(validate_call(call));
     PDSC_TRY(plan_encoder(call.cfg, call.bs, call.N, call.nvalid, call.n_min, &x.plan));
     PDSC_TRY(bind_workspace(x));
+    PDSC_REQUIRE(probe || g_encoder_ends_override < 2 || head_computes_layer0(x) || tail_finishes_encoder(x), "pdsc_encoder_ends_override(%d): "
+                 "this call does not take the point-fragment route (bs=%d N=%d), which alone has the fused forms", g_encoder_ends_override,
+                 call.bs, call.N);
     PDSC_TRY(run_compat_layer0(x));
     PDSC_TRY(x.plan.fused && !probe ? run_encoder_fused(x) : run_encoder_per_conv(x));
     if (probe) return PDSC_OK;
diff --git a/pointdsc_amd/csrc/compat.hip b/pointdsc_amd/csrc/compat.hip
--- a/pointdsc_amd/csrc/compat.hip
+++ b/pointdsc_amd/csrc/compat.hip
@@ -92,14 +92,20 @@
 }
 
 constexpr int CS_T = 128;
+__device__ __forceinline__ void range_sentinel_clear(unsigned int* __restrict__ range_clear, int range_n, bool first_block) {
+    if (range_clear && first_block)
+        for (int i = threadIdx.x; i < range_n; i += 256) range_clear[i] = 0u;
+}
+
 constexpr int CS_STRIP = 32;
 constexpr int CS_LD = CS_T + 4;
 
 template <bool FASTMATH>
 __global__ __launch_bounds__(256) void compat_sym_kernel(const float* __restrict__ src, const float* __restrict__ tgt,
                                                          const float* __restrict__ sigma_spat, float* __restrict__ compat,
-                                                         long long ld, int N) {
+                                                         long long ld, int N, unsigned int* __restrict__ range_clear, int range_n) {
     const int I = blockIdx.y, J = blockIdx.x, b = blockIdx.z;
+    range_sentinel_clear(range_clear, range_n, I == 0 && J == 0 && b == 0);
     if (I > J) return;
     __shared__ __attribute__((aligned(16))) float Ts[CS_STRIP * CS_LD];
     __shared__ __attribute__((aligned(16))) float rows_s[CS_T * 8];
@@ -257,8 +263,10 @@
 template <bool CLAMP>
 __global__ __launch_bounds__(256) void compat_sym_u16_kernel(const float* __restrict__ src, const float* __restrict__ tgt,
                                                              const float* __restrict__ sigma_spat,
-                                                             unsigned short* __restrict__ compat, long long ld, int N, int nt) {
+                                                             unsigned short* __restrict__ compat, long long ld, int N, int nt,
+                                                             unsigned int* __restrict__ range_clear, int range_n) {
     const int idx = blockIdx.x, b = blockIdx.y;
+    range_sentinel_clear(range_clear, range_n, idx == 0 && b == 0);
     int I = (int)(((float)(2 * nt + 1) - __builtin_sqrtf((float)((2 * nt + 1) * (2 * nt + 1) - 8 * idx))) * 0.5f);
     I = max(0, min(I, nt - 1));
     while (I > 0 && I * nt - I * (I - 1) / 2 > idx) --I;
@@ -387,8 +395,9 @@
 
 extern "C" long long pdsc_compat_ld(int N) { return N <= 0 ? -1 : pdsc::round_up(N, 64); }
 
-extern "C" int pdsc_spatial_compat(const float* src, const float* tgt, const float* sigma_spat, float* compat,
-                                   float* src_dist, long long ld, int bs, int N, void* stream) {
+namespace pdsc {
+int launch_spatial_compat(const float* src, const float* tgt, const float* sigma_spat, float* compat, float* src_dist, long long ld, int bs,
+                          int N, unsigned int* range_clear, void* stream) {
     PDSC_REQUIRE(src && tgt && sigma_spat && compat, "pdsc_spatial_compat: null pointer");
     PDSC_REQUIRE(bs > 0 && N > 0, "pdsc_spatial_compat: bs=%d N=%d", bs, N);
     PDSC_REQUIRE(ld >= N && ld % 4 == 0, "pdsc_spatial_compat: ld=%lld must be >= N and a multiple of 4", ld);
@@ -396,6 +405,17 @@
     const dim3 full_grid(pdsc::ceil_div((int)ld, pdsc::CT_COLS), pdsc::ceil_div(N, pdsc::CT_ROWS), bs);
     const int nt = pdsc::ceil_div(N, pdsc::CS_T);
     const dim3 sym_grid(nt, nt, bs);
+    bool own_clear = src_dist == nullptr;
+#ifdef PDSC_EXPERIMENTS
+    {
+        const int variant = pdsc::env_int("PDSC_COMPAT_VARIANT", PDSC_COMPAT_DEFAULT_VARIANT);
+        own_clear = own_clear && (variant < 0 || variant > 2);
+    }
+#endif
+    if (range_clear && !own_clear) {
+        if (const int rc = launch_fill_u32(range_clear, 0u, (size_t)bs, st); rc != PDSC_OK) return rc;
+        range_clear = nullptr;
+    }
     pdsc::profile_mark_begin(PDSC_PROF_COMPAT, st);
     if (src_dist)
         hipLaunchKernelGGL((pdsc::compat_kernel<true, true>), full_grid, dim3(256), 0, st, src, tgt, sigma_spat, compat, src_dist, ld, N);
@@ -407,17 +427,17 @@
         else if (variant == 1)
             hipLaunchKernelGGL((pdsc::compat_kernel<false, true>), full_grid, dim3(256), 0, st, src, tgt, sigma_spat, compat, nullptr, ld, N);
         else if (variant == 2)
-            hipLaunchKernelGGL((pdsc::compat_sym_kernel<false>), sym_grid, dim3(256), 0, st, src, tgt, sigma_spat, compat, ld, N);
+            hipLaunchKernelGGL((pdsc::compat_sym_kernel<false>), sym_grid, dim3(256), 0, st, src, tgt, sigma_spat, compat, ld, N, nullptr, 0);
         else
 #endif
-        hipLaunchKernelGGL((pdsc::compat_sym_kernel<true>), sym_grid, dim3(256), 0, st, src, tgt, sigma_spat, compat, ld, N);
+        hipLaunchKernelGGL((pdsc::compat_sym_kernel<true>), sym_grid, dim3(256), 0, st, src, tgt, sigma_spat, compat, ld, N, range_clear, bs);
     }
     pdsc::profile_mark_end(PDSC_PROF_COMPAT, st);
     return pdsc::check_launch("pdsc_spatial_compat");
 }
 
-extern "C" int pdsc_spatial_compat_u16(const float* src, const float* tgt, const float* sigma_spat, unsigned short* compat_u16,
-                                       long long ld, int bs, int N, void* stream) {
+int launch_spatial_compat_u16(const float* src, const float* tgt, const float* sigma_spat, unsigned short* compat_u16, long long ld, int bs,
+                              int N, unsigned int* range_clear, void* stream) {
     PDSC_REQUIRE(src && tgt && sigma_spat && compat_u16, "pdsc_spatial_compat_u16: null pointer");
     PDSC_REQUIRE(bs > 0 && N > 0, "pdsc_spatial_compat_u16: bs=%d N=%d", bs, N);
     PDSC_REQUIRE(ld >= pdsc::round_up(N, 32) && ld % 32 == 0, "pdsc_spatial_compat_u16: ld=%lld must be a multiple of 32 and >= N", ld);
@@ -425,16 +445,32 @@
     const int nt = pdsc::ceil_div(N, pdsc::CF_T);
     PDSC_REQUIRE(nt <= 1024, "pdsc_spatial_compat_u16: N=%d too large", N);
     const dim3 grid((unsigned)(nt * (nt + 1) / 2), bs);
+#ifdef PDSC_EXPERIMENTS
+    const int variant = pdsc::env_int("PDSC_COMPAT16_VARIANT", 2);
+    if (range_clear && variant == 0) {
+        if (const int rc = launch_fill_u32(range_clear, 0u, (size_t)bs, st); rc != PDSC_OK) return rc;
+        range_clear = nullptr;
+    }
+#endif
     pdsc::profile_mark_begin(PDSC_PROF_COMPAT, st);
 #ifdef PDSC_EXPERIMENTS
-    const int variant = pdsc::env_int("PDSC_COMPAT16_VARIANT", 2);
     if (variant == 0)
         hipLaunchKernelGGL(pdsc::compat_sym_u16_exact_kernel, dim3(nt, nt, bs), dim3(256), 0, st, src, tgt, sigma_spat, compat_u16, ld, N);
     else if (variant == 1)
-        hipLaunchKernelGGL(pdsc::compat_sym_u16_kernel<true>, grid, dim3(256), 0, st, src, tgt, sigma_spat, compat_u16, ld, N, nt);
+        hipLaunchKernelGGL(pdsc::compat_sym_u16_kernel<true>, grid, dim3(256), 0, st, src, tgt, sigma_spat, compat_u16, ld, N, nt, range_clear, bs);
     else
 #endif
-    hipLaunchKernelGGL(pdsc::compat_sym_u16_kernel<false>, grid, dim3(256), 0, st, src, tgt, sigma_spat, compat_u16, ld, N, nt);
+    hipLaunchKernelGGL(pdsc::compat_sym_u16_kernel<false>, grid, dim3(256), 0, st, src, tgt, sigma_spat, compat_u16, ld, N, nt, range_clear, bs);
     pdsc::profile_mark_end(PDSC_PROF_COMPAT, st);
     return pdsc::check_launch("pdsc_spatial_compat_u16");
 }
+}
+
+extern "C" int pdsc_spatial_compat(const float* src, const float* tgt, const float* sigma_spat, float* compat,
+                                   float* src_dist, long long ld, int bs, int N, void* stream) {
+    return pdsc::launch_spatial_compat(src, tgt, sigma_spat, compat, src_dist, ld, bs, N, nullptr, stream);
+}
+extern "C" int pdsc_spatial_compat_u16(const float* src, const float* tgt, const float* sigma_spat, unsigned short* compat_u16,
+                                       long long ld, int bs, int N, void* stream) {
+    return pdsc::launch_spatial_compat_u16(src, tgt, sigma_spat, compat_u16, ld, bs, N, nullptr, stream);
+}
diff --git a/pointdsc_amd/csrc/encoder_finish.h b/pointdsc_amd/csrc/encoder_finish.h
--- /dev/null
+++ b/pointdsc_amd/csrc/encoder_finish.h
@@ -0,0 +1,106 @@
+#pragma once
+#include "pdsc_common.h"
+#include "split_layout.h"
+#include "layer_args.h"
+
+namespace pdsc {
+
+constexpr int EF_HIDDEN = 32;
+
+__device__ __forceinline__ float other_half(float x) { return __shfl_xor(x, 32, 64); }
+
+__device__ __forceinline__ float finish_sum_squares(const f32x4 (&v)[16]) {
+    float u[2];
+#pragma unroll
+    for (int j = 0; j < 2; ++j) {
+        float t[16];
+#pragma unroll
+        for (int q = 0; q < 16; ++q) t[q] = fmaf(v[q][2 * j + 1], v[q][2 * j + 1], v[q][2 * j] * v[q][2 * j]);
+#pragma unroll
+        for (int n = 8; n > 0; n >>= 1)
+#pragma unroll
+            for (int q = 0; q < n; ++q) t[q] = t[q] + t[q + n];
+        u[j] = t[0];
+    }
+    u[0] = u[0] + other_half(u[0]);
+    u[1] = u[1] + other_half(u[1]);
+    return u[0] + u[1];
+}
+
+__device__ __forceinline__ float finish_dot_w3(const f32x4 (&h2)[4], const float* __restrict__ w3, int h) {
+    f32x4 p[4];
+#pragma unroll
+    for (int g = 0; g < 4; ++g) {
+        const f32x4 wv = *reinterpret_cast<const f32x4*>(w3 + 8 * g + 4 * h);
+#pragma unroll
+        for (int e = 0; e < 4; ++e) p[g][e] = h2[g][e] * wv[e] + 0.f;
+    }
+    float s[4];
+#pragma unroll
+    for (int e = 0; e < 4; ++e) {
+        s[e] = (p[0][e] + p[2][e]) + (p[1][e] + p[3][e]);
+        s[e] = s[e] + other_half(s[e]);
+    }
+    return (s[0] + s[2]) + (s[1] + s[3]);
+}
+
+__device__ __forceinline__ void encoder_finish(const LayerArgs& a, const f32x4 (&v)[16], size_t row, size_t gw, int lane, bool live, int qsel,
+                                               bool do_cls) {
+    const int l31 = lane & 31, h = lane >> 5;
+    if (do_cls) {
+        f32x16 acc;
+#pragma unroll
+        for (int r = 0; r < 16; ++r) acc[r] = 0.f;
+        const float* wa = a.cls_w1 + l31 * PDSC_CHANNELS + 4 * h;
+#pragma unroll
+        for (int q = 0; q < PDSC_CHANNELS / 8; ++q) {
+            const f32x4 av = *reinterpret_cast<const f32x4*>(wa + 8 * q);
+#pragma unroll
+            for (int e = 0; e < 4; ++e) acc = __builtin_amdgcn_mfma_f32_32x32x2f32(av[e], v[q][e], acc, 0, 0, 0);
+        }
+        f32x4 h1[4];
+#pragma unroll
+        for (int q = 0; q < 4; ++q) {
+            const f32x4 bv = *reinterpret_cast<const f32x4*>(a.cls_b1 + 8 * q + 4 * h);
+#pragma unroll
+            for (int e = 0; e < 4; ++e) h1[q][e] = fmaxf(acc[4 * q + e] + bv[e], 0.f);
+        }
+        f32x16 acc2;
+#pragma unroll
+        for (int r = 0; r < 16; ++r) acc2[r] = 0.f;
+        const float* wa2 = a.cls_w2 + l31 * EF_HIDDEN + 4 * h;
+#pragma unroll
+        for (int q = 0; q < EF_HIDDEN / 8; ++q) {
+            const f32x4 av = *reinterpret_cast<const f32x4*>(wa2 + 8 * q);
+#pragma unroll
+            for (int e = 0; e < 4; ++e) acc2 = __builtin_amdgcn_mfma_f32_32x32x2f32(av[e], h1[q][e], acc2, 0, 0, 0);
+        }
+        f32x4 h2[4];
+#pragma unroll
+        for (int g = 0; g < 4; ++g) {
+            const f32x4 bv = *reinterpret_cast<const f32x4*>(a.cls_b2 + 8 * g + 4 * h);
+#pragma unroll
+            for (int e = 0; e < 4; ++e) h2[g][e] = fmaxf(acc2[4 * g + e] + bv[e], 0.f);
+        }
+        const float p = finish_dot_w3(h2, a.cls_w3, h);
+        if (h == 0) a.conf[row] = p + a.cls_b3[0];
+    }
+    const float ss = finish_sum_squares(v);
+    const float nrm = fmaxf(sqrtf(ss), 1e-12f);
+    float* pf = a.normed_pf ? a.normed_pf + gw * PF_TILE_FLOATS + lane * 4 : nullptr;
+#pragma unroll
+    for (int q = 0; q < 16; ++q) {
+        if (qsel >= 0 && (q >> 2) != qsel) continue;
+        f32x4 o;
+#pragma unroll
+        for (int e = 0; e < 4; ++e) o[e] = v[q][e] / nrm;
+        *reinterpret_cast<f32x4*>(a.normed + row * PDSC_CHANNELS + 8 * q + 4 * h) = o;
+        if (pf) {
+#pragma unroll
+            for (int e = 0; e < 4; ++e) o[e] = live ? o[e] : 0.f;
+            *reinterpret_cast<f32x4*>(pf + pf_offset_floats(q)) = o;
+        }
+    }
+}
+
+}
diff --git a/pointdsc_amd/csrc/layer.hip b/pointdsc_amd/csrc/layer.hip
--- a/pointdsc_amd/csrc/layer.hip
+++ b/pointdsc_amd/csrc/layer.hip
@@ -319,12 +319,16 @@
                                  a.part_slots, a.nsplit);
         PDSC_REQUIRE(!(io & PDSC_IO_PARTIALS_PF) || (!a.msg && a.Npad % 32 == 0), "%s: PF partials come un-merged (msg NULL), Npad a multiple of 32", who);
     } else {
-        PDSC_REQUIRE(a.feat_in, "%s: head-only needs feat_in", who);
+        PDSC_REQUIRE((a.feat_in != nullptr) != (a.corr_pos != nullptr), "%s: head-only needs feat_in, or corr_pos (layer0 inside the launch), not both", who);
+        PDSC_REQUIRE(!a.corr_pos || (h3 && (io & PDSC_IO_FEATB_PF) && a.w0 && a.b0 && a.in_dim >= 1 && a.in_dim <= 16),
+                     "%s: corr_pos needs the H3 kernel with point-fragment featB, W0, b0 and 1 <= in_dim=%d <= 16", who, a.in_dim);
         PDSC_REQUIRE(!(io & (PDSC_IO_PARTIALS_PF | PDSC_IO_RES_PF)), "%s: head-only takes feat_in in row order", who);
     }
     if (head) PDSC_REQUIRE((a.qkv_out || a.qs) && (frag ? a.wf_head != nullptr : a.wp && a.bp && a.wq && a.bq),
                            "%s: head needs qkv_out or the split streams, and pcn, qkv weights (natural layout or the head stream)", who);
     else PDSC_REQUIRE(a.feat_out && !(io & PDSC_IO_FEATB_PF), "%s: tail-only needs feat_out (row order)", who);
+    PDSC_REQUIRE(!a.normed || (h3 && tail && !head && a.conf && a.cls_w1 && a.cls_b1 && a.cls_w2 && a.cls_b2 && a.cls_w3 && a.cls_b3),
+                 "%s: normed (the encoder finished inside the launch) needs a tail-only launch of the H3 kernel, conf and the classifier weights", who);
     PDSC_REQUIRE((a.qs == nullptr) == (a.kv == nullptr), "%s: q_split and kv_tiles go together", who);
     PDSC_REQUIRE(!h3 || launch_layer_h3_fits(a, tail, head), "%s: output set not served by the H3 kernel (head: the split streams "
                  "only; tail + head: no feat_out; tail only: feat_out)", who);
diff --git a/pointdsc_amd/csrc/layer0_chain.h b/pointdsc_amd/csrc/layer0_chain.h
--- /dev/null
+++ b/pointdsc_amd/csrc/layer0_chain.h
@@ -0,0 +1,40 @@
+#pragma once
+#include "pdsc_common.h"
+
+namespace pdsc {
+
+constexpr int L0_LD = 16;
+constexpr int layer0_kd(int in_dim) { return in_dim <= 8 ? 8 : 16; }
+
+template <int KD>
+__device__ __forceinline__ void layer0_load_row(const float* __restrict__ corr, long long row, int in_dim, float (&x)[KD]) {
+#pragma unroll
+    for (int d = 0; d < KD; ++d) x[d] = d < in_dim ? corr[row * in_dim + d] : 0.f;
+}
+
+template <int KD>
+__device__ __forceinline__ float layer0_channel(const float (&x)[KD], const float (&w)[KD], float bias) {
+    float s = 0.f;
+#pragma unroll
+    for (int d = 0; d < KD; ++d) s = fmaf(x[d], w[d], s);
+    return s + bias;
+}
+
+template <int KD>
+__device__ __forceinline__ f32x4 layer0_piece(const float (&x)[KD], const float* __restrict__ W0, const float* __restrict__ b0, int c0) {
+    f32x4 o;
+#pragma unroll
+    for (int c = 0; c < 4; ++c) {
+        float w[KD];
+#pragma unroll
+        for (int d4 = 0; d4 < KD; d4 += 4) {
+            const f32x4 v = *reinterpret_cast<const f32x4*>(W0 + (c0 + c) * L0_LD + d4);
+#pragma unroll
+            for (int d = 0; d < 4; ++d) w[d4 + d] = v[d];
+        }
+        o[c] = layer0_channel<KD>(x, w, b0[c0 + c]);
+    }
+    return o;
+}
+
+}
diff --git a/pointdsc_amd/csrc/layer_args.h b/pointdsc_amd/csrc/layer_args.h
--- a/pointdsc_amd/csrc/layer_args.h
+++ b/pointdsc_amd/csrc/layer_args.h
@@ -30,6 +30,11 @@
     unsigned int* range_flag;
     int value_fold;
     const int* nvalid;
+    const float* corr_pos;
+    const float *w0, *b0;
+    int in_dim;
+    const float *cls_w1, *cls_b1, *cls_w2, *cls_b2, *cls_w3, *cls_b3;
+    float *normed, *normed_pf, *conf;
 };
 
 enum class LayerKernel { Block, Wave, H3, X3 };
diff --git a/pointdsc_amd/csrc/layer_coop.hip b/pointdsc_amd/csrc/layer_coop.hip
--- a/pointdsc_amd/csrc/layer_coop.hip
+++ b/pointdsc_amd/csrc/layer_coop.hip
@@ -5,6 +5,8 @@
 #include "layer_args.h"
 #include "layer_wave.h"
 #include "ragged.h"
+#include "layer0_chain.h"
+#include "encoder_finish.h"
 
 namespace pdsc {
 
@@ -20,7 +22,7 @@
         for (int e = 0; e < 4; ++e) v[g][e] = QKV ? acc[4 * g + e] : fmaf(cross[4 * g + e], H3_INV, acc[4 * g + e]);
 }
 
-template <bool T, bool H, bool FB_PF, int NB, bool F = false>
+template <bool T, bool H, bool FB_PF, int NB, bool F = false, bool L0 = false, bool FIN = false>
 __global__ __launch_bounds__(64 * LC_WAVES, NB <= 4 ? 2 : 1) void layer_h3_coop_kernel(LayerArgs a) {
     __shared__ __attribute__((aligned(16))) CoopOps ops;
     __shared__ __attribute__((aligned(16))) float Vs_all[LC_WAVES][32 * LW_VLD];
@@ -175,9 +177,35 @@
             for (int e = 0; e < 4; ++e) y3[s][e] = y3[s][e] + v[s][e];
             if constexpr (!H) *reinterpret_cast<f32x4*>(a.feat_out + row * PDSC_CHANNELS + 32 * w + 8 * s + 4 * h) = y3[s];
         }
+        if constexpr (FIN) {
+            static_assert(!H, "the tail-only launch finishes the encoder");
+            f32x4* fin = reinterpret_cast<f32x4*>(&ops.v[1][0][0][0]);
+#pragma unroll
+            for (int s = 0; s < 4; ++s) fin[(4 * w + s) * 64 + lane] = y3[s];
+            __syncthreads();
+            f32x4 full[16];
+#pragma unroll
+            for (int q = 0; q < 16; ++q) full[q] = fin[q * 64 + lane];
+            encoder_finish(a, full, row, (size_t)gw, lane, live, w, w == 0);
+        }
     } else {
-#pragma unroll
-        for (int s = 0; s < 4; ++s) y3[s] = *reinterpret_cast<const f32x4*>(a.feat_in + row * PDSC_CHANNELS + 32 * w + 8 * s + 4 * h);
+        if constexpr (L0) {
+            auto rows = [&](auto kd_c) __attribute__((always_inline)) {
+                constexpr int KD = decltype(kd_c)::value;
+                float x[KD];
+                layer0_load_row<KD>(a.corr_pos, (long long)row, a.in_dim, x);
+#pragma unroll
+                for (int s = 0; s < 4; ++s) {
+                    y3[s] = layer0_piece<KD>(x, a.w0, a.b0, 32 * w + 8 * s + 4 * h);
+                    __builtin_amdgcn_sched_barrier(0);
+                }
+            };
+            if (layer0_kd(a.in_dim) == 8) rows(std::integral_constant<int, 8>{});
+            else rows(std::integral_constant<int, 16>{});
+        } else {
+#pragma unroll
+            for (int s = 0; s < 4; ++s) y3[s] = *reinterpret_cast<const f32x4*>(a.feat_in + row * PDSC_CHANNELS + 32 * w + 8 * s + 4 * h);
+        }
     }
 
     if constexpr (H) {
@@ -289,12 +317,24 @@
     const dim3 grid(a.bs * ceil_div(a.N, 32)), block(64 * LC_WAVES);
     switch (layer_h3_form(a, tail, head)) {
         case H3Form::FoldTailHeadPF: hipLaunchKernelGGL((layer_h3_coop_kernel<true, true, true, 4, true>), grid, block, 0, st, a); break;
-        case H3Form::FoldHeadPF: hipLaunchKernelGGL((layer_h3_coop_kernel<false, true, true, 4, true>), grid, block, 0, st, a); break;
-        case H3Form::FoldTail: hipLaunchKernelGGL((layer_h3_coop_kernel<true, false, false, 4, true>), grid, block, 0, st, a); break;
+        case H3Form::FoldHeadPF:
+            if (a.corr_pos) hipLaunchKernelGGL((layer_h3_coop_kernel<false, true, true, 4, true, true>), grid, block, 0, st, a);
+            else hipLaunchKernelGGL((layer_h3_coop_kernel<false, true, true, 4, true>), grid, block, 0, st, a);
+            break;
+        case H3Form::FoldTail:
+            if (a.normed) hipLaunchKernelGGL((layer_h3_coop_kernel<true, false, false, 4, true, false, true>), grid, block, 0, st, a);
+            else hipLaunchKernelGGL((layer_h3_coop_kernel<true, false, false, 4, true>), grid, block, 0, st, a);
+            break;
         case H3Form::TailHeadPF: hipLaunchKernelGGL((layer_h3_coop_kernel<true, true, true, 4>), grid, block, 0, st, a); break;
-        case H3Form::HeadPF: hipLaunchKernelGGL((layer_h3_coop_kernel<false, true, true, 4>), grid, block, 0, st, a); break;
+        case H3Form::HeadPF:
+            if (a.corr_pos) hipLaunchKernelGGL((layer_h3_coop_kernel<false, true, true, 4, false, true>), grid, block, 0, st, a);
+            else hipLaunchKernelGGL((layer_h3_coop_kernel<false, true, true, 4>), grid, block, 0, st, a);
+            break;
         case H3Form::TailHead: hipLaunchKernelGGL((layer_h3_coop_kernel<true, true, false, 4>), grid, block, 0, st, a); break;
-        case H3Form::Tail: hipLaunchKernelGGL((layer_h3_coop_kernel<true, false, false, 4>), grid, block, 0, st, a); break;
+        case H3Form::Tail:
+            if (a.normed) hipLaunchKernelGGL((layer_h3_coop_kernel<true, false, false, 4, false, false, true>), grid, block, 0, st, a);
+            else hipLaunchKernelGGL((layer_h3_coop_kernel<true, false, false, 4>), grid, block, 0, st, a);
+            break;
         case H3Form::Head: hipLaunchKernelGGL((layer_h3_coop_kernel<false, true, false, 4>), grid, block, 0, st, a); break;
         case H3Form::Unserved: return PDSC_ERR_ARG;
     }
diff --git a/pointdsc_amd/csrc/layer_h3.hip b/pointdsc_amd/csrc/layer_h3.hip
--- a/pointdsc_amd/csrc/layer_h3.hip
+++ b/pointdsc_amd/csrc/layer_h3.hip
@@ -5,6 +5,8 @@
 #include "merge_partials.h"
 #include "layer_args.h"
 #include "layer_wave.h"
+#include "layer0_chain.h"
+#include "encoder_finish.h"
 
 namespace pdsc {
 
@@ -16,7 +18,8 @@
 template <bool F = false>
 constexpr int stage_tiles(int stage) { return stage == ST_FC1 || stage == ST_FC2 ? 2 : stage == ST_FC3 || stage == ST_PCN ? 4 : F ? 10 : 12; }
 
-template <bool T, bool H, bool TRACE = false, int PIPE = 6, int EXP = 0, bool FB_PF = false, int NWV = LW_WAVES, int NBUF = 2, bool F = false>
+template <bool T, bool H, bool TRACE = false, int PIPE = 6, int EXP = 0, bool FB_PF = false, int NWV = LW_WAVES, int NBUF = 2, bool F = false,
+          bool L0 = false, bool FIN = false>
 __global__ __launch_bounds__(64 * NWV, NBUF > 2 ? 1 : 2) void layer_h3_kernel(LayerArgs a) {
     __shared__ __attribute__((aligned(16))) float Vs_all[NWV][32 * LW_VLD];
     const int lane = threadIdx.x & 63;
@@ -110,8 +113,21 @@
             });
         }
     } else {
-#pragma unroll
-        for (int q = 0; q < 16; ++q) y3[q] = *reinterpret_cast<const f32x4*>(a.feat_in + row * PDSC_CHANNELS + 8 * q + 4 * h);
+        static_assert(!L0 || (H && !T), "layer0 is formed by the head-only launch");
+        if constexpr (L0) {
+            auto rows = [&](auto kd_c) __attribute__((always_inline)) {
+                constexpr int KD = decltype(kd_c)::value;
+                float x[KD];
+                layer0_load_row<KD>(a.corr_pos, (long long)row, a.in_dim, x);
+#pragma unroll
+                for (int q = 0; q < 16; ++q) y3[q] = layer0_piece<KD>(x, a.w0, a.b0, 8 * q + 4 * h);
+            };
+            if (layer0_kd(a.in_dim) == 8) rows(std::integral_constant<int, 8>{});
+            else rows(std::integral_constant<int, 16>{});
+        } else {
+#pragma unroll
+            for (int q = 0; q < 16; ++q) y3[q] = *reinterpret_cast<const f32x4*>(a.feat_in + row * PDSC_CHANNELS + 8 * q + 4 * h);
+        }
 #pragma unroll
         for (int kk = 0; kk < 8; ++kk) make_kstep<true>(y3[2 * kk], y3[2 * kk + 1], ayh[kk], ayl[kk], rmax);
     }
@@ -266,6 +282,10 @@
     });
 
     LH_STAMP(63)
+    if constexpr (FIN) {
+        static_assert(T && !H, "the tail-only launch finishes the encoder");
+        encoder_finish(a, y3, row, (size_t)gw, lane, live, -1, true);
+    }
     range_report(a.range_flag, b, rmax);
 }
 
@@ -337,8 +357,14 @@
     } while (0)
     switch (form) {
         case H3Form::FoldTailHeadPF: hipLaunchKernelGGL((layer_h3_kernel<true, true, false, 6, 0, true, LW_WAVES, 2, true>), grid, block, 0, st, a); break;
-        case H3Form::FoldHeadPF: hipLaunchKernelGGL((layer_h3_kernel<false, true, false, 6, 0, true, LW_WAVES, 2, true>), grid, block, 0, st, a); break;
-        case H3Form::FoldTail: hipLaunchKernelGGL((layer_h3_kernel<true, false, false, 6, 0, false, LW_WAVES, 2, true>), grid, block, 0, st, a); break;
+        case H3Form::FoldHeadPF:
+            if (a.corr_pos) hipLaunchKernelGGL((layer_h3_kernel<false, true, false, 6, 0, true, LW_WAVES, 2, true, true>), grid, block, 0, st, a);
+            else hipLaunchKernelGGL((layer_h3_kernel<false, true, false, 6, 0, true, LW_WAVES, 2, true>), grid, block, 0, st, a);
+            break;
+        case H3Form::FoldTail:
+            if (a.normed) hipLaunchKernelGGL((layer_h3_kernel<true, false, false, 6, 0, false, LW_WAVES, 2, true, false, true>), grid, block, 0, st, a);
+            else hipLaunchKernelGGL((layer_h3_kernel<true, false, false, 6, 0, false, LW_WAVES, 2, true>), grid, block, 0, st, a);
+            break;
         case H3Form::TailHeadPF: {
 #ifdef PDSC_LAYER_DIAG
             const int ex = env_int("PDSC_LAYER_H3_EXP", 0);
@@ -355,7 +381,10 @@
             PDSC_H3_LAUNCH(true, true, true);
             break;
         }
-        case H3Form::HeadPF: PDSC_H3_LAUNCH(false, true, true); break;
+        case H3Form::HeadPF:
+            if (a.corr_pos) hipLaunchKernelGGL((layer_h3_kernel<false, true, false, 6, 0, true, LW_WAVES, 2, false, true>), grid, block, 0, st, a);
+            else PDSC_H3_LAUNCH(false, true, true);
+            break;
         case H3Form::TailHead:
 #ifdef PDSC_EXPERIMENTS
             if (a.trace) hipLaunchKernelGGL((layer_h3_kernel<true, true, true>), dim3(ceil_div(waves, LW_WAVES)), dim3(64 * LW_WAVES), 0, st, a);
@@ -363,7 +392,10 @@
 #endif
             PDSC_H3_LAUNCH(true, true, false);
             break;
-        case H3Form::Tail: PDSC_H3_LAUNCH(true, false, false); break;
+        case H3Form::Tail:
+            if (a.normed) hipLaunchKernelGGL((layer_h3_kernel<true, false, false, 6, 0, false, LW_WAVES, 2, false, false, true>), grid, block, 0, st, a);
+            else PDSC_H3_LAUNCH(true, false, false);
+            break;
         case H3Form::Head: PDSC_H3_LAUNCH(false, true, false); break;
         case H3Form::Unserved: break;
     }
diff --git a/pointdsc_amd/csrc/linear.hip b/pointdsc_amd/csrc/linear.hip
--- a/pointdsc_amd/csrc/linear.hip
+++ b/pointdsc_amd/csrc/linear.hip
@@ -1,6 +1,7 @@
 #include "pdsc_common.h"
 #include "gram_tile.h"
 #include "ragged.h"
+#include "layer0_chain.h"
 
 namespace pdsc {
 
@@ -103,7 +104,6 @@
 }
 
 constexpr int L0_MAX_BLOCKS = 2048;
-constexpr int L0_LD = 16;
 template <int KD>
 __global__ __launch_bounds__(256) void layer0_kernel(const float* __restrict__ corr, int in_dim,
                                                      const float* __restrict__ W0, const float* __restrict__ b0,
@@ -124,16 +124,10 @@
     }
     for (long long row = (long long)blockIdx.x * 8 + rl; row < M; row += (long long)gridDim.x * 8) {
         float x[KD];
-#pragma unroll
-        for (int d = 0; d < KD; ++d) x[d] = d < in_dim ? corr[row * in_dim + d] : 0.f;
+        layer0_load_row<KD>(corr, row, in_dim, x);
         f32x4 o;
 #pragma unroll
-        for (int c = 0; c < 4; ++c) {
-            float s = 0.f;
-#pragma unroll
-            for (int d = 0; d < KD; ++d) s = fmaf(x[d], w[c][d], s);
-            o[c] = s + bias[c];
-        }
+        for (int c = 0; c < 4; ++c) o[c] = layer0_channel<KD>(x, w[c], bias[c]);
         *reinterpret_cast<f32x4*>(feat + row * PDSC_CHANNELS + c4) = o;
     }
 }
@@ -383,7 +377,7 @@
     PDSC_REQUIRE(corr_pos && W0 && b0 && feat, "pdsc_layer0: null pointer");
     PDSC_REQUIRE(in_dim >= 1 && in_dim <= 16 && M > 0, "pdsc_layer0: in_dim=%d (1..16) M=%d", in_dim, M);
     const int blocks = ceil_div(M, 8) < L0_MAX_BLOCKS ? ceil_div(M, 8) : L0_MAX_BLOCKS;
-    if (in_dim <= 8)
+    if (layer0_kd(in_dim) == 8)
         hipLaunchKernelGGL(layer0_kernel<8>, dim3((unsigned)blocks), dim3(256), 0, st, corr_pos, in_dim, W0, b0, feat, M, range_flag, bs);
     else
         hipLaunchKernelGGL(layer0_kernel<16>, dim3((unsigned)blocks), dim3(256), 0, st, corr_pos, in_dim, W0, b0, feat, M, range_flag, bs);
diff --git a/pointdsc_amd/csrc/ragged.h b/pointdsc_amd/csrc/ragged.h
--- a/pointdsc_amd/csrc/ragged.h
+++ b/pointdsc_amd/csrc/ragged.h
@@ -33,6 +33,10 @@
                            const unsigned int* range_flag = nullptr);
 int launch_layer0(const float* corr_pos, int in_dim, const float* W0, const float* b0, float* feat, int M, unsigned int* range_flag, int bs,
                   hipStream_t st);
+int launch_spatial_compat(const float* src, const float* tgt, const float* sigma_spat, float* compat, float* src_dist, long long ld, int bs,
+                          int N, unsigned int* range_clear, void* stream);
+int launch_spatial_compat_u16(const float* src, const float* tgt, const float* sigma_spat, unsigned short* compat_u16, long long ld, int bs,
+                              int N, unsigned int* range_clear, void* stream);
 constexpr int PDSC_REFINE_TRACE = 24;
 int launch_attention_split_ex(const void* q_split, const void* kv_tiles, const void* compat, int compat_format, long long ld,
                               float* msg, void* scratch, size_t scratch_bytes, int bs, int N, int nsplit, int partial_layout,
```
